# eigenvivek/DiffDRR

Hardware: AMD Instinct MI355X
Metric: DRRs/sec fwd+bwd, 512^3 vol -> 256^2 det, batched poses (higher is better)
Workload: dtype f32; 1 GPU; 512^3 fp32 noise volume -> 256x256 detector, Siddon forward + backward w.r.t. 6-DoF pose (euler ZXY) through NCC, 32 perturbed poses per GPU per step; volume=512x512x512 f32 (512 MiB, replicated per GPU), detector=256x256, batch_per_gpu=32, global_batch=32, parallelism=single GPU, brick_storage_fallbacks=0, bricks=2048, brick_storage=q16p, step=DRR.ncc, fused (at most 32 poses per call): ddrr_pose_ray...

## Files before the change

### diffdrr_amd/_lib.py

```python
from __future__ import annotations

import ctypes
import os
import re
from ctypes import c_char_p, c_double, c_float, c_int, c_long, c_void_p
from typing import NamedTuple

_HERE = os.path.dirname(os.path.abspath(__file__))
_INCLUDE = os.path.join(os.path.dirname(_HERE), "include")
LIB_PATH = os.path.join(_HERE, "csrc", "libdiffdrr_hip.so")
ABI_VERSION = 33
MI_ABI_VERSION = 1
RECON_ABI_VERSION = 1
FBP_ABI_VERSION = 1
LM_ABI_VERSION = 1
WARP_ABI_VERSION = 1
BSPLINE_ABI_VERSION = 1
POLYRIGID_ABI_VERSION = 1
JACOBIAN_ABI_VERSION = 1
PROX_ABI_VERSION = 1

_P, _I, _F, _L, _D = c_void_p, c_int, c_float, c_long, c_double
_ARGTYPES = {"int": c_int, "long": c_long, "float": c_float, "double": c_double}
_RESTYPES_OF = {"int": c_int, "long": c_long, "const char *": c_char_p}
_DECLARATION = re.compile(r"(.*?)\b(ddrr_\w+)\s*\((.*)\)", re.S)
_POINTER = re.compile(r"[\w\s]+\*[\s*]*\w+")
_SCALAR = re.compile(r"(\w+)\s+\w+")


def parse_header(text: str):
    code = re.sub(r"/\*.*?\*/", " ", text, flags=re.S)
    code = re.sub(r"//[^\n]*", "", code)
    defines = {k: int(v) for k, v in re.findall(r"^[ \t]*#[ \t]*define[ \t]+(DDRR_\w+)[ \t]+(\d+)[ \t]*$",
                                                code, re.M)}
    code = re.sub(r"^[ \t]*#[^\n]*", "", code, flags=re.M)
    signatures, restypes = {}, {}
    for stmt in re.split(r"[;{}]", code):
        if not re.search(r"\bddrr_\w+\s*\(", stmt):
            continue
        m = _DECLARATION.fullmatch(" ".join(stmt.split()))
        name = m.group(2) if m else re.search(r"\bddrr_\w+", stmt).group(0)
        ret = re.sub(r"\s*\*\s*", " *", m.group(1)).strip() if m else None
        if ret not in _RESTYPES_OF:
            raise ValueError(f"{name}: cannot bind the declaration {' '.join(stmt.split())!r} "
                             "(return type int, long or const char * expected)")
        params = m.group(3).strip()
        argtypes = []
        for param in ([] if params == "void" else params.split(",")):
            param = param.strip()
            scalar = _SCALAR.fullmatch(param)
            if _POINTER.fullmatch(param):
                argtypes.append(c_void_p)
            elif scalar and scalar.group(1) in _ARGTYPES:
                argtypes.append(_ARGTYPES[scalar.group(1)])
            else:
                raise ValueError(f"{name}: cannot bind the parameter {param!r} (a pointer, int, long, float "
                                 "or double expected)")
        if name in signatures:
            raise ValueError(f"{name}: declared twice")
        signatures[name], restypes[name] = argtypes, _RESTYPES_OF[ret]
    return signatures, restypes, defines


class Header(NamedTuple):
    path: str
    prefix: str
    version: int
    argtypes: dict
    restypes: dict
    defines: dict

    @classmethod
    def read(cls, name: str, prefix: str, version: int) -> "Header":
        path = os.path.join(_INCLUDE, name)
        with open(path) as f:
            argtypes, restypes, defines = parse_header(f.read())
        macro = f"{prefix.upper()}_ABI_VERSION"
        if defines.get(macro) != version:
            raise RuntimeError(f"{path}: {macro} is {defines.get(macro)}, the binding is written against {version}")
        return cls(path, prefix, version, argtypes, restypes, defines)

    def tables(self):
        own = (f"{self.prefix}_abi_version", f"{self.prefix}_last_error")
        signatures = {n: a for n, a in self.argtypes.items() if n not in own}
        return signatures, {n: self.restypes[n] for n in signatures if self.restypes[n] is not c_int}, \
            list(self.argtypes)

    def constants(self, *names):
        return [self.defines[f"{self.prefix.upper()}_{n}"] for n in names]


HEADER = Header.read("diffdrr_hip.h", "ddrr", ABI_VERSION)
_SIGNATURES, _RESTYPES, EXPORTS = HEADER.tables()

REDUCE_SUM, REDUCE_MAX = HEADER.constants("REDUCE_SUM", "REDUCE_MAX")
LOOKUP_STEP, LOOKUP_MID_NEAREST, LOOKUP_MID_TRILINEAR = HEADER.constants(
    "LOOKUP_STEP", "LOOKUP_MID_NEAREST", "LOOKUP_MID_TRILINEAR")
SIDDON_AUX, = HEADER.constants("SIDDON_AUX")
AUX_INTERLEAVED, AUX_BLOCKED, AUX_PACKED = HEADER.constants("AUX_INTERLEAVED", "AUX_BLOCKED", "AUX_PACKED")
REC_BLOCK_RAYS, REC_BLOCK_FLOATS = HEADER.constants("REC_BLOCK_RAYS", "REC_BLOCK_FLOATS")
BRICKS_F32, BRICKS_Q16, BRICKS_Q16_PACKED, BRICKS_CLEARED = HEADER.constants(
    "BRICKS_F32", "BRICKS_Q16", "BRICKS_Q16_PACKED", "BRICKS_CLEARED")
PACKED_AUX_PLANES, TRI_AUX_PLANES = HEADER.constants("PACKED_AUX_PLANES", "TRI_AUX_PLANES")


class DdrrLibrary:

    def __init__(self, path: str, header: Header = HEADER):
        self.path = path
        self.cdll = ctypes.CDLL(path)
        for name in header.argtypes:
            if not hasattr(self.cdll, name):
                raise RuntimeError(f"{path} does not export {name}")
            fn = getattr(self.cdll, name)
            fn.argtypes, fn.restype = header.argtypes[name], header.restypes[name]
        got = getattr(self.cdll, f"{header.prefix}_abi_version")()
        if got != header.version:
            raise RuntimeError(f"{path}: ABI version {got}, expected {header.version}")
        self._last_error = getattr(self.cdll, f"{header.prefix}_last_error")

    def query(self, name: str, *args):
        return getattr(self.cdll, name)(*args)

    def call(self, name: str, *args):
        rc = getattr(self.cdll, name)(*args)
        if rc != 0:
            msg = self._last_error().decode(errors="replace")
            raise RuntimeError(f"{name} failed (code {rc}): {msg}")


_lib: DdrrLibrary | None = None


def get_lib() -> DdrrLibrary:
    global _lib
    if _lib is None:
        import torch

        if not os.path.exists(LIB_PATH):
            raise RuntimeError(
                f"{LIB_PATH} is missing: the MI355X renderers have not been built. Run "
                "`python -c 'import __graft_entry__ as g; g.build()'` (needs hipcc); "
                "diffdrr_amd has no CPU fallback."
            )
        _lib = DdrrLibrary(LIB_PATH)
    return _lib


MI_LIB_PATH = os.path.join(_HERE, "csrc", "libdiffdrr_mi_hip.so")
MI_HEADER = Header.read("diffdrr_mi_hip.h", "ddrr_mi", MI_ABI_VERSION)
_MI_SIGNATURES, _MI_RESTYPES, MI_EXPORTS = MI_HEADER.tables()
MI_MAX_BINS, = MI_HEADER.constants("MAX_BINS")


def mi_library(path: str) -> DdrrLibrary:
    return DdrrLibrary(path, MI_HEADER)


_mi_lib: DdrrLibrary | None = None


def get_mi_lib() -> DdrrLibrary:
    global _mi_lib
    if _mi_lib is None:
        import torch

        if not os.path.exists(MI_LIB_PATH):
            raise RuntimeError(
                f"{MI_LIB_PATH} is missing: the MutualInformation kernels have not been built. Run "
                "`python -c 'import __graft_entry__ as g; g.build()'` (needs hipcc).")
        _mi_lib = mi_library(MI_LIB_PATH)
    return _mi_lib


RECON_LIB_PATH = os.path.join(_HERE, "csrc", "libdiffdrr_recon_hip.so")
RECON_HEADER = Header.read("diffdrr_recon_hip.h", "ddrr_recon", RECON_ABI_VERSION)
_RECON_SIGNATURES, _RECON_RESTYPES, RECON_EXPORTS = RECON_HEADER.tables()
RECON_TV_ISOTROPIC, RECON_TV_ANISOTROPIC, RECON_MAX_DIM = RECON_HEADER.constants(
    "TV_ISOTROPIC", "TV_ANISOTROPIC", "MAX_DIM")


def recon_library(path: str) -> DdrrLibrary:
    return DdrrLibrary(path, RECON_HEADER)


_recon_lib: DdrrLibrary | None = None


def get_recon_lib() -> DdrrLibrary:
    global _recon_lib
    if _recon_lib is None:
        import torch

        if not os.path.exists(RECON_LIB_PATH):
            raise RuntimeError(
                f"{RECON_LIB_PATH} is missing: the reconstruction kernels have not been built. Run "
                "`python -c 'import __graft_entry__ as g; g.build()'` (needs hipcc).")
        _recon_lib = recon_library(RECON_LIB_PATH)
    return _recon_lib


FBP_LIB_PATH = os.path.join(_HERE, "csrc", "libdiffdrr_fbp_hip.so")
FBP_HEADER = Header.read("diffdrr_fbp_hip.h", "ddrr_fbp", FBP_ABI_VERSION)
_FBP_SIGNATURES, _FBP_RESTYPES, FBP_EXPORTS = FBP_HEADER.tables()
FBP_MAX_IMAGE_DIM, FBP_MAX_VIEWS, FBP_MAX_DIM, FBP_VIEW_FLOATS = FBP_HEADER.constants(
    "MAX_IMAGE_DIM", "MAX_VIEWS", "MAX_DIM", "VIEW_FLOATS")


def fbp_library(path: str) -> DdrrLibrary:
    return DdrrLibrary(path, FBP_HEADER)


_fbp_lib: DdrrLibrary | None = None


def get_fbp_lib() -> DdrrLibrary:
    global _fbp_lib
    if _fbp_lib is None:
        import torch

        if not os.path.exists(FBP_LIB_PATH):
            raise RuntimeError(
                f"{FBP_LIB_PATH} is missing: the FDK kernels have not been built. Run "
                "`python -c 'import __graft_entry__ as g; g.build()'` (needs hipcc).")
        _fbp_lib = fbp_library(FBP_LIB_PATH)
    return _fbp_lib


LM_LIB_PATH = os.path.join(_HERE, "csrc", "libdiffdrr_lm_hip.so")
LM_HEADER = Header.read("diffdrr_lm_hip.h", "ddrr_lm", LM_ABI_VERSION)
_LM_SIGNATURES, _LM_RESTYPES, LM_EXPORTS = LM_HEADER.tables()
LM_SUMS, LM_GROUP_RAYS, LM_STATE_DOUBLES, LM_MAX_POSES = LM_HEADER.constants(
    "SUMS", "GROUP_RAYS", "STATE_DOUBLES", "MAX_POSES")


def lm_library(path: str) -> DdrrLibrary:
    return DdrrLibrary(path, LM_HEADER)


_lm_lib: DdrrLibrary | None = None


def get_lm_lib() -> DdrrLibrary:
    global _lm_lib
    if _lm_lib is None:
        import torch

        if not os.path.exists(LM_LIB_PATH):
            raise RuntimeError(
                f"{LM_LIB_PATH} is missing: the Levenberg-Marquardt kernels have not been built. Run "
                "`python -c 'import __graft_entry__ as g; g.build()'` (needs hipcc).")
        _lm_lib = lm_library(LM_LIB_PATH)
    return _lm_lib


# ... 138 lines not shown
```

### diffdrr_amd/csrc/brick_shared.h

```cpp
#pragma once

#include <mutex>

#include "runtime.h"
#include "brick_core.h"
#include "brick_walk.h"
#include "record_layout.h"

namespace ddrr_brick {

using namespace ddrr;

constexpr int kQueueCap = 128;
constexpr int kBuckets = 3;
#if defined(DDRR_EXPERIMENTS) && defined(DDRR_RECORD_GROUP)
constexpr int kRecordGroup = DDRR_RECORD_GROUP;
#else
constexpr int kRecordGroup = 4;
#endif
#if defined(DDRR_EXPERIMENTS) && defined(DDRR_RECORD_ALIGN)
constexpr int kRecordAlign = DDRR_RECORD_ALIGN;
#else
constexpr int kRecordAlign = 4;
#endif
static_assert(kRecordGroup == 8 || kRecordGroup == 4 || kRecordGroup == 2 || kRecordGroup == 1, "DPP maxima");
static_assert(kRecordAlign == 8 || kRecordAlign == 4 || kRecordAlign == 2 || kRecordAlign == 1, "a power of two, at most a run of the record");

struct BrickArgs {
    const float *vol;
    Dims D;
    const float *source;
    const float *target;
    const float *img;
    int B, det_h, det_w;
    float shift, eps;
    BrickLayout lay;
    unsigned aux_plane;
    float rec_q;
    int pix_bits;
    float t1, t2;
    int dbg;
    int *work;
    const float *grad_out;
    float *g_volume;
    int n_points;
    const float *amin, *amax;
    unsigned long long *prof;
    const unsigned char *labels;
    int n_channels;
    const float *ranges;
    const int *fallback;
    int *ws_header;
    int ranges_valid;
    const unsigned char *packed;
    const unsigned *pix_mask;
    const unsigned *fingerprint;
    int vec;
    const int *order;
    int *order_ws;
    int order_cap;
    float *clear;
    long clear_n;
    unsigned *brick_times;
    int split_t, split_s;
};

#if defined(DDRR_BRICK_PROFILE)
struct BrickProf {
    unsigned long long t[16];
    unsigned long long last, born;
    __device__ __forceinline__ void start() {
#pragma unroll
        for (int i = 0; i < 16; ++i) t[i] = 0;
        last = __builtin_amdgcn_s_memtime();
        born = __builtin_amdgcn_s_memrealtime();
    }
    __device__ __forceinline__ void mark(int i) {
        const unsigned long long now = __builtin_amdgcn_s_memtime();
        t[i] += now - last;
        last = now;
    }
    __device__ __forceinline__ void count(int i, unsigned long long n) { t[i] += n; }
};
#if defined(DDRR_TRACE_ONLY)
#define DDRR_PROF(i)
#define DDRR_PROF_COUNT(i, n)
#define DDRR_PROF_WAIT_VMEM()
#else
#define DDRR_PROF(i) prof.mark(i)
#define DDRR_PROF_COUNT(i, n) prof.count(i, n)
#define DDRR_PROF_WAIT_VMEM() asm volatile("s_waitcnt vmcnt(0)" ::: "memory")
#endif
#else
struct BrickProf {};
#define DDRR_PROF(i)
#define DDRR_PROF_COUNT(i, n)
#define DDRR_PROF_WAIT_VMEM()
#endif
enum {
    PROF_STAGE = 0,
    PROF_PULL = 1,
    PROF_PHASE_A = 2,
    PROF_POP = 3,
    PROF_LOADS = 4,
    PROF_SETUP = 5,
    PROF_WALK = 6,
    PROF_DELIVER = 7,
    PROF_BARRIER = 8,
    PROF_N_BATCH = 9, PROF_N_STEPS = 10, PROF_N_UNITS = 11, PROF_N_HITS = 12,
    PROF_CLAIM = 13,
    PROF_ROWS = 14,
    PROF_STORE = 15,
};

constexpr int BRICK_FWD = 0;
constexpr int BRICK_FWD_AUX = 1;
constexpr int BRICK_VOLGRAD = 2;
constexpr int BRICK_TRI_FWD = 3;
constexpr int BRICK_TRI_VOLGRAD = 4;
constexpr int BRICK_TRI_FWD_AUX = 5;
constexpr int BRICK_CHANNELS = 6;
constexpr int BRICK_TRI_CHANNELS = 7;
constexpr int BRICK_CHANNELS_AUX = 8;
constexpr int BRICK_TRI_CHANNELS_AUX = 9;
constexpr int BRICK_CHANNELS_VOLGRAD = 10;
constexpr int BRICK_CHANNELS_WORDS = 12;
constexpr int BRICK_TRI_CHANNELS_VOLGRAD = 11;


#if defined(__HIPCC__)
__device__ __forceinline__ void halfwave_swap(unsigned a, unsigned b, unsigned &x, unsigned &y) {
    const auto s = __builtin_amdgcn_permlane32_swap(a, b, false, false);
    x = s[0];
    y = s[1];
}

__device__ __forceinline__ void deliver_record_blocked(float *__restrict__ aux, bool ok,
                                                       unsigned r, const float v[5]) {
    const unsigned lo = rec_off01(r) | (ok ? 0u : 0x80000000u);
    unsigned xu, yu, x01u, y01u, x23u, y23u;
    halfwave_swap(lo, lo + 8u, xu, yu);
    halfwave_swap(__float_as_uint(v[0]), __float_as_uint(v[1]), x01u, y01u);
    halfwave_swap(__float_as_uint(v[2]), __float_as_uint(v[3]), x23u, y23u);
    const int xo = (int)xu, yo = (int)yu;
    const float x01 = __uint_as_float(x01u), y01 = __uint_as_float(y01u);
    const float x23 = __uint_as_float(x23u), y23 = __uint_as_float(y23u);
    if (xo >= 0) {
        unsafeAtomicAdd(aux + xo, x01);
        unsafeAtomicAdd(aux + xo + 16, x23);
    }
    if (yo >= 0) {
        unsafeAtomicAdd(aux + yo, y01);
        unsafeAtomicAdd(aux + yo + 16, y23);
    }
    if (ok) unsafeAtomicAdd(aux + rec_off4(r), v[4]);
}

typedef unsigned int quad_u32x4 __attribute__((ext_vector_type(4)));
typedef unsigned int quad_u32x4_a4 __attribute__((ext_vector_type(4), aligned(4)));
template <bool LABELS>
__device__ __forceinline__ void quad_load(const float *__restrict__ vol,
                                          const unsigned char *__restrict__ label_map, const Dims &D,
                                          long at, quad_u32x4 &v, unsigned &labels) {
    const long a = quad_clamped_at(D, at);
    v = *reinterpret_cast<const quad_u32x4_a4 *>(vol + a);
    if (LABELS) __builtin_memcpy(&labels, label_map + a, 4);
}
__device__ __forceinline__ void quad_fix(const Dims &D, int x, int y, int z, quad_u32x4 &v,
                                         unsigned &labels) {
    const int shift = quad_shift(D, x, y, z);
    if (shift > 0) {
        if (shift >= 2) v = quad_u32x4{v.z, v.w, 0u, 0u};
        if (shift & 1) v = quad_u32x4{v.y, v.z, v.w, 0u};
        labels = shift < 4 ? labels >> (8 * shift) : 0u;
    }
}

__device__ __forceinline__ int lane_rank(unsigned long long mask) {
    return (int)__builtin_amdgcn_mbcnt_hi((unsigned)(mask >> 32),
                                          __builtin_amdgcn_mbcnt_lo((unsigned)mask, 0u));
}

__device__ __forceinline__ int uni(int v) { return __builtin_amdgcn_readfirstlane(v); }

__device__ __forceinline__ void wave_fence() {
    __builtin_amdgcn_fence(__ATOMIC_SEQ_CST, "wavefront");
    __builtin_amdgcn_wave_barrier();
}

#endif

struct BrickLaunch {
    const float *volume;
    int dx, dy, dz;
    const float *source, *target, *img;
    int B, det_h, det_w;
    float shift, eps;
    hipStream_t st;
    void *launch_ws;
    const char *who;
    const float *grad_out = nullptr;
    float *out = nullptr, *aux = nullptr, *g_volume = nullptr;
    int n_points = 0;
    const float *amin = nullptr, *amax = nullptr;
    float rec_q = 0.f;
    const unsigned char *labels = nullptr;
    int n_channels = 0;
    const unsigned *pix_mask = nullptr;
};

struct FwdStorage {
    int variant, packed;
    float *brick_ranges;
    int ranges_valid;
    float *clear;
    long clear_n;
};

int brick_args(const BrickLaunch &l, BrickArgs &p);

long brick_launch_workspace_bytes(int dx, int dy, int dz);
int brick_launch_resources(const BrickLaunch &l, BrickArgs &p, int &dev, int &n_cu, bool zero_work = true);

constexpr int kMaxDev = 64;
int current_device(int &dev);
struct OncePerDevice {
    std::mutex mu;
    bool done[kMaxDev] = {false};
};
template <class F>
int once_per_device(OncePerDevice &once, int dev, F f) {
    std::lock_guard<std::mutex> lock(once.mu);
    if (once.done[dev]) return 0;
    if (int rc = f()) return rc;
    once.done[dev] = true;
    return 0;
}
template <class K>
int raise_lds_limit(K *kernel, int bytes) {
    const hipError_t e = hipFuncSetAttribute(reinterpret_cast<const void *>(kernel),
                                             hipFuncAttributeMaxDynamicSharedMemorySize, bytes);
    return e == hipSuccess ? 0 : ddrr_rt::fail_hip(e, "hipFuncSetAttribute");
}

bool order_bricks(BrickArgs &q, int BX, int BY, int BZ, int nby, int nbz, int n_bricks, int slots,
                  hipStream_t st, bool zero_counter = false, int min_poses = 8);
int launch_bricks(int mode, const BrickLaunch &l);

long brick_workspace_bytes(int dx, int dy, int dz, int brick_storage);
int launch_fwd_bricks(const BrickLaunch &l, const FwdStorage &s);

#if defined(DDRR_EXPERIMENTS) || defined(DDRR_BRICK_PROFILE)
extern float g_brick_t1, g_brick_t2;
extern int g_brick_dbg;
extern int g_brick_variant;
extern const int *g_brick_order;
extern unsigned *g_brick_times;
extern int g_brick_split_t, g_brick_split_s;
#else
constexpr float g_brick_t1 = 18.f, g_brick_t2 = 40.f;
constexpr int g_brick_dbg = 0;
#endif
#if defined(DDRR_BRICK_PROFILE)
extern unsigned long long *g_brick_prof;
#endif

}
```

### diffdrr_amd/csrc/bricks.hip

```cpp
#include "runtime.h"

#include "siddon_core.h"
#include "brick_core.h"
#include "brick_walk.h"
#include "brick_step.h"
#include "record_pack.h"
#include "record_layout.h"
#include "tri_brick.h"
#include "brick_shared.h"
#include "trilinear_core.h"

using namespace ddrr;
using namespace ddrr_rt;
using namespace ddrr_brick;

namespace {


constexpr int kBrickThreads = 1024;
constexpr int kBrickWaves = kBrickThreads / 64;
constexpr int kPoseChunk = 32;

inline size_t brick_lds_bytes(const BrickLayout &lay) {
    return (size_t)brick_floats(lay) * 4 + (size_t)kBrickWaves * kBuckets * kQueueCap * 4 +
// ... 964 lines not shown
    p.prof = g_brick_prof;
#endif
    return 0;
}

namespace {

struct BrickMode {
    int mode;
    void (*kernel)(BrickArgs, float *, float *);
    bool marcher;
    bool tri_grid;
    int prepare;
    int order_min_poses;
};
template <int MODE>
constexpr BrickMode brick_mode(bool marcher, bool tri_grid, int prepare, int order_min_poses) {
    return {MODE, &siddon_brick_kernel<MODE>, marcher, tri_grid, prepare, order_min_poses};
}
constexpr BrickMode kBrickModes[] = {
    brick_mode<BRICK_CHANNELS_WORDS>(false, false, 0, 8),
    brick_mode<BRICK_TRI_CHANNELS_VOLGRAD>(true, false, 2, 0),
    brick_mode<BRICK_CHANNELS_VOLGRAD>(false, false, 2, 8),
    brick_mode<BRICK_TRI_CHANNELS_AUX>(true, true, 0, 0),
    brick_mode<BRICK_CHANNELS_AUX>(false, false, 0, 8),
    brick_mode<BRICK_TRI_CHANNELS>(true, true, 0, 0),
    brick_mode<BRICK_CHANNELS>(false, false, 0, 8),
    brick_mode<BRICK_TRI_FWD_AUX>(true, true, 0, 0),
    brick_mode<BRICK_FWD>(false, false, 0, 8),
    brick_mode<BRICK_FWD_AUX>(false, false, 0, 8),
    brick_mode<BRICK_VOLGRAD>(false, false, 1, 8),
    brick_mode<BRICK_TRI_FWD>(true, true, 0, 0),
    brick_mode<BRICK_TRI_VOLGRAD>(true, false, 1, 1),
};

}

int launch_bricks(int mode, const BrickLaunch &l) {
    const BrickMode *m = nullptr;
    for (const BrickMode &row : kBrickModes)
        if (row.mode == mode) m = &row;
    if (!m) return fail(-1, "unknown brick mode");
    BrickArgs p;
    if (int rc = brick_args(l, p)) return rc;
    p.lay = g_brick_layout;
    if (m->marcher) {
        p.t1 = g_tri_t1;
        p.t2 = g_tri_t2;
    }
    const size_t lds = brick_lds_bytes(p.lay);
    int dev = 0, n_cu = 0;
    if (int rc = brick_launch_resources(l, p, dev, n_cu)) return rc;
    static OncePerDevice lds_limit;
    if (int rc = once_per_device(lds_limit, dev, [] {
            for (const BrickMode &row : kBrickModes)
                if (int r = raise_lds_limit(row.kernel, 160 * 1024)) return r;
            return 0;
        }))
        return rc;
    if (m->prepare) {
        const int N = l.det_h * l.det_w;
        int bx = (N + kBlock - 1) / kBlock;
        bx = bx > 64 ? 64 : bx;
        hipLaunchKernelGGL(volgrad_prepare_kernel, dim3(bx, l.B), dim3(kBlock), 0, l.st, (int)m->marcher,
                           l.source, l.target, l.img, l.grad_out, N, l.det_w, p.D, l.shift, l.eps,
                           l.n_points, l.amin, l.amax, p.work, m->prepare == 2 ? l.n_channels : 0);
    }
    const BrickGrid bg = m->tri_grid ? tri_brick_grid(p.D) : brick_grid(p.D);
    const int n_bricks = bg.nx * bg.ny * bg.nz;
    if (m->order_min_poses)
        order_bricks(p, BRICK, BRICK, BRICK, bg.ny, bg.nz, n_bricks, n_cu, l.st, false, m->order_min_poses);
    const dim3 grid(n_bricks < n_cu ? n_bricks : n_cu), block(kBrickThreads);
    hipLaunchKernelGGL(m->kernel, grid, block, lds, l.st, p, l.out, l.aux);
    return finish(l.who);
}

}

extern "C" {

#if defined(DDRR_EXPERIMENTS) || defined(DDRR_BRICK_PROFILE)
int ddrr_set_brick_layout(int sy, int sx) {
    if (sy < BRICK || sx < BRICK * sy) return -1;
    BrickLayout lay = {sy, sx};
    if (brick_lds_bytes(lay) > 160 * 1024) return -1;
    g_brick_layout = lay;
    return 0;
}
int ddrr_set_brick_debug(int flags) {
    g_brick_dbg = flags;
    return 0;
}
int ddrr_set_brick_classes(float t1, float t2) {
    g_brick_t1 = t1;
    g_brick_t2 = t2;
    return 0;
}
#endif
#if defined(DDRR_BRICK_PROFILE)
int ddrr_brick_profile_reset() {
    if (!g_brick_prof && hipMalloc(reinterpret_cast<void **>(&g_brick_prof), 20 * 8) != hipSuccess)
        return -1;
    return hipMemset(g_brick_prof, 0, 20 * 8) == hipSuccess ? 0 : -1;
}
int ddrr_brick_profile_read20(unsigned long long *host20) {
    if (!g_brick_prof) return -1;
    return hipMemcpy(host20, g_brick_prof, 20 * 8, hipMemcpyDeviceToHost) == hipSuccess ? 0 : -1;
}
int ddrr_brick_profile_read(unsigned long long *host16) {
    if (!g_brick_prof) return -1;
    return hipMemcpy(host16, g_brick_prof, 16 * 8, hipMemcpyDeviceToHost) == hipSuccess ? 0 : -1;
}
#endif

static int check_detector(int det_h, int det_w) {
    if (det_h < 2 || det_w < 2) return fail(-1, "the brick path needs a detector of at least 2x2");
    return 0;
}
static int check_channel_cap(int B, int C, int N, const char *per_ray_entry) {
    if ((long)B * C * N < (1L << 30) && N < (1 << 22)) return 0;
    char msg[256];
    snprintf(msg, sizeof(msg), "B * C * N must stay below 2^30 (and N below 2^22) for one channel launch "
                               "on the bricks: split the pose batch or use %s", per_ray_entry);
    return fail(-1, msg);
}
static int check_n_points(int n_points) {
    if (n_points < 2) return fail(-1, "n_points must be >= 2");
    return 0;
}
static int check_alpha_range(const float *alphamin, const float *alphamax) {
    if (!alphamin || !alphamax) return fail(-1, "null alphamin / alphamax");
    return 0;
}
static int zero_floats(float *buf, size_t n, hipStream_t st) {
    const hipError_t e = hipMemsetAsync(buf, 0, sizeof(float) * n, st);
    return e == hipSuccess ? 0 : fail_hip(e, "hipMemsetAsync");
}
static int zero_volume_gradient(float *g_volume, int dx, int dy, int dz, hipStream_t st) {
    return zero_floats(g_volume, (size_t)dx * dy * dz, st);
}

static int siddon_forward_bricks_impl(const float *volume, int dx, int dy, int dz, const float *source,
                                      const float *target, const float *img, int B, int det_h,
                                      int det_w, float voxel_shift, float eps, float *out, float *aux,
                                      float record_vmax, int brick_storage, float *brick_ranges,
                                      int ranges_valid, void *launch_ws, const unsigned *pixel_mask,
                                      void *stream) {
    const int N = det_h * det_w;
    if (int rc = check_common(volume, dx, dy, dz, source, 1, target, B, N, nullptr)) return rc;
    if (!out && !aux) return fail(-1, "null out pointer");
    if (int rc = check_detector(det_h, det_w)) return rc;
    if (!(record_vmax >= 0.f)) return fail(-1, "record_vmax must be >= 0");
    if (brick_storage != DDRR_BRICKS_F32 && brick_storage != DDRR_BRICKS_Q16 &&
        brick_storage != DDRR_BRICKS_Q16_PACKED)
        return fail(-1, "brick_storage must be DDRR_BRICKS_F32, DDRR_BRICKS_Q16 or DDRR_BRICKS_Q16_PACKED");
    if (brick_storage != DDRR_BRICKS_F32 && !brick_ranges)
        return fail(-1, "DDRR_BRICKS_Q16 needs the brick_ranges workspace");
    if (B == 0) return 0;
    hipStream_t st = (hipStream_t)stream;
    const long R = (long)B * N;
    const bool cleared = (ranges_valid & DDRR_BRICKS_CLEARED) != 0;
    const bool packed = aux && record_vmax > 0.f;
    const size_t fill = !aux ? (size_t)R : (packed ? (size_t)R * 5 : (size_t)rec_blocked_floats(R));
    BrickLaunch l{volume, dx, dy, dz, source, target, img, B, det_h, det_w, voxel_shift, eps, st, launch_ws,
                  "ddrr_siddon_forward_bricks"};
    l.out = out;
    l.aux = aux;
    l.pix_mask = pixel_mask;
    if (packed) {
        if (!cleared)
            if (int rc = zero_floats(aux, fill, st)) return rc;
        l.rec_q = record_scale(record_vmax, Dims{dx, dy, dz});
        hipLaunchKernelGGL(record_prepare_kernel, dim3((unsigned)((R + kBlock - 1) / kBlock)),
                           dim3(kBlock), 0, st, source, target, R, N, Dims{dx, dy, dz}, voxel_shift,
                           eps, l.rec_q, aux);
    }
    FwdStorage fs;
    fs.packed = brick_storage == DDRR_BRICKS_Q16_PACKED;
    fs.variant = fs.packed ? DDRR_BRICKS_Q16 : brick_storage;
    fs.brick_ranges = brick_ranges;
    fs.ranges_valid = ranges_valid & 1;
    fs.clear = packed || cleared ? nullptr : (aux ? aux : out);
    fs.clear_n = cleared ? -1 : (packed ? 0 : (long)fill);
    if (int rc = launch_fwd_bricks(l, fs)) return rc;
    if (!aux) return 0;
    if (out)
        hipLaunchKernelGGL(siddon_out_from_record_kernel, dim3((unsigned)((R + kBlock - 1) / kBlock)),
                           dim3(kBlock), 0, st, aux + (packed ? 4 * R : 0), packed ? 0 : 1, img, R, out);
    return finish("ddrr_siddon_forward_bricks");
}

int ddrr_siddon_forward_bricks(const float *volume, int dx, int dy, int dz, const float *source,
                               const float *target, const float *img, int B, int det_h,
                               int det_w, float voxel_shift, float eps, float *out, float *aux,
                               float record_vmax, int brick_storage, float *brick_ranges,
                               int ranges_valid, void *launch_ws, void *stream) {
    return siddon_forward_bricks_impl(volume, dx, dy, dz, source, target, img, B, det_h, det_w, voxel_shift,
                                      eps, out, aux, record_vmax, brick_storage, brick_ranges, ranges_valid,
                                      launch_ws, nullptr, stream);
}

int ddrr_siddon_forward_bricks_masked(const float *volume, int dx, int dy, int dz, const float *source,
                                      const float *target, const float *img, int B, int det_h,
                                      int det_w, float voxel_shift, float eps, float *out, float *aux,
                                      float record_vmax, int brick_storage, float *brick_ranges,
                                      int ranges_valid, void *launch_ws, const unsigned *pixel_mask,
                                      void *stream) {
    if (pixel_mask && (reinterpret_cast<uintptr_t>(pixel_mask) & 3) != 0)
        return fail(-1, "pixel_mask must be 4-byte aligned");
    return siddon_forward_bricks_impl(volume, dx, dy, dz, source, target, img, B, det_h, det_w, voxel_shift,
                                      eps, out, aux, record_vmax, brick_storage, brick_ranges, ranges_valid,
                                      launch_ws, pixel_mask, stream);
}

long ddrr_brick_workspace_bytes(int dx, int dy, int dz, int brick_storage) {
    if (dx < 1 || dy < 1 || dz < 1) return 0;
    return brick_workspace_bytes(dx, dy, dz, brick_storage);
}

long ddrr_brick_launch_workspace_bytes(int dx, int dy, int dz) {
    if (dx < 1 || dy < 1 || dz < 1) return 0;
    return brick_launch_workspace_bytes(dx, dy, dz);
}

int ddrr_siddon_forward_channels_bricks(const float *volume, const unsigned char *labels, int dx,
                                        int dy, int dz, const float *source, const float *target,
                                        const float *img, int B, int det_h, int det_w, int C,
                                        float voxel_shift, float eps, float *out, void *launch_ws,
                                        void *stream) {
    const int N = det_h * det_w;
    if (int rc = check_common(volume, dx, dy, dz, source, 1, target, B, N,
                              "ddrr_siddon_forward_channels_bricks (mask_to_channels)"))
        return rc;
    if (!labels || !out || C < 1) return fail(-1, "null labels/out or C < 1");
    if (int rc = check_detector(det_h, det_w)) return rc;
    if (int rc = check_channel_cap(B, C, N, "ddrr_siddon_forward_channels")) return rc;
    if (B == 0) return 0;
    hipStream_t st = (hipStream_t)stream;
    if (int rc = zero_floats(out, (size_t)B * C * N, st)) return rc;
    BrickLaunch l{volume, dx, dy, dz, source, target, img, B, det_h, det_w, voxel_shift, eps, st, launch_ws,
                  "ddrr_siddon_forward_channels_bricks"};
    l.out = out;
    l.labels = labels;
    l.n_channels = C;
    return launch_bricks(BRICK_CHANNELS, l);
}

constexpr int kChannelWordsStateWords = 2 + 2 * kFingerprintWords;

__global__ __launch_bounds__(1024) void channel_words_check_kernel(const float *__restrict__ vol,
                                                                   const unsigned char *__restrict__ labels,
                                                                   long n, int *__restrict__ state, int force) {
    unsigned *fp = reinterpret_cast<unsigned *>(state + 2);
    int bad = force;
    unsigned v = 0u, l = 0u;
    if (threadIdx.x < kFingerprintWords) {
        const long at = fingerprint_index(threadIdx.x, n);
        v = __float_as_uint(vol[at]);
        l = (unsigned)labels[at];
        bad |= (v != fp[threadIdx.x]) | (l != fp[kFingerprintWords + threadIdx.x]);
    }
    const bool stale = __syncthreads_or(bad) != 0;
    if (stale && threadIdx.x < kFingerprintWords) {
        fp[threadIdx.x] = v;
        fp[kFingerprintWords + threadIdx.x] = l;
    }
    if (threadIdx.x == 0) {
        state[0] = stale ? 1 : 0;
        if (stale) state[1] += 1;
    }
}

__global__ __launch_bounds__(1024) void channel_words_kernel(const float *__restrict__ vol,
                                                             const unsigned char *__restrict__ labels, long n,
                                                             unsigned n_channels, float *__restrict__ words,
                                                             const int *__restrict__ state) {
    if (state[0] == 0) return;
    const long stride = (long)gridDim.x * 1024;
    for (long i = (long)blockIdx.x * 1024 + threadIdx.x; i < n; i += stride)
        words[i] = pack_voxel_label_below(vol[i], labels[i], n_channels);
}

long ddrr_channel_words_state_bytes(void) { return (long)kChannelWordsStateWords * 4; }

int ddrr_channel_words(const float *volume, const unsigned char *labels, long n_voxels, int C, float *words,
                       void *state, int force, void *stream) {
    if (!volume || !labels || !words || !state || C < 1 || n_voxels < 0)
        return fail(-1, "null pointer or C < 1");
    if (n_voxels == 0) return 0;
    static_assert(kFingerprintWords <= 1024, "one sample per thread of the check");
    const long blocks = (n_voxels + 4095) / 4096;
    hipLaunchKernelGGL(channel_words_check_kernel, dim3(1), dim3(1024), 0, (hipStream_t)stream, volume, labels,
                       n_voxels, reinterpret_cast<int *>(state), force ? 1 : 0);
    hipLaunchKernelGGL(channel_words_kernel, dim3((unsigned)(blocks > 512 ? 512 : blocks)), dim3(1024), 0,
                       (hipStream_t)stream, volume, labels, n_voxels, (unsigned)C, words,
                       reinterpret_cast<const int *>(state));
    return finish("ddrr_channel_words");
}

int ddrr_siddon_forward_channels_bricks_words(const float *words, int dx, int dy, int dz, const float *source,
                                              const float *target, const float *img, int B, int det_h,
                                              int det_w, int C, float voxel_shift, float eps, float *out,
                                              void *launch_ws, void *stream) {
    const int N = det_h * det_w;
    if (int rc = check_common(words, dx, dy, dz, source, 1, target, B, N,
                              "ddrr_siddon_forward_channels_bricks_words (mask_to_channels)"))
        return rc;
    if (!out || C < 1) return fail(-1, "null out or C < 1");
    if (int rc = check_detector(det_h, det_w)) return rc;
    if (int rc = check_channel_cap(B, C, N, "ddrr_siddon_forward_channels")) return rc;
    if (B == 0) return 0;
    hipStream_t st = (hipStream_t)stream;
    if (int rc = zero_floats(out, (size_t)B * C * N, st)) return rc;
    BrickLaunch l{words, dx, dy, dz, source, target, img, B, det_h, det_w, voxel_shift, eps, st, launch_ws,
                  "ddrr_siddon_forward_channels_bricks_words"};
    l.out = out;
    l.n_channels = C;
    return launch_bricks(BRICK_CHANNELS_WORDS, l);
}

int ddrr_siddon_backward_channels_bricks(const float *volume, const unsigned char *labels, int dx,
                                         int dy, int dz, const float *source, const float *target,
                                         const float *grad_out, int B, int det_h, int det_w, int C,
                                         float voxel_shift, float eps, float *aux, void *launch_ws,
                                         void *stream) {
    const int N = det_h * det_w;
    if (int rc = check_common(volume, dx, dy, dz, source, 1, target, B, N,
                              "ddrr_siddon_backward_channels_bricks (mask_to_channels)"))
        return rc;
    if (!labels || !grad_out || !aux || C < 1) return fail(-1, "null labels/grad_out/aux or C < 1");
    if (int rc = check_detector(det_h, det_w)) return rc;
    if (int rc = check_channel_cap(B, C, N, "ddrr_siddon_backward_channels")) return rc;
// ... 217 lines not shown
```

### diffdrr_amd/csrc/bricks_fwd.hip

```cpp
#include "runtime.h"

#include "siddon_core.h"
#include "brick_core.h"
#include "brick_walk.h"
#include "brick_step.h"
#include "record_pack.h"
#include "record_layout.h"
#include "brick_shared.h"

using namespace ddrr;
using namespace ddrr_rt;
using namespace ddrr_brick;

namespace {

template <int BX_, int BY_, int BZ_, int THREADS_, bool Q16_, int ROWPAD_ = -1>
struct FwdCfg {
    static constexpr int BX = BX_, BY = BY_, BZ = BZ_, THREADS = THREADS_, WAVES = THREADS_ / 64;
    static constexpr bool Q16 = Q16_;
    static constexpr int ES = Q16 ? 2 : 4;
    static constexpr int ROWPAD = ROWPAD_ < 0 ? ES : ROWPAD_;
    static constexpr int SY = BZ * ES + ROWPAD;
    static constexpr int SX = BY * SY + ES;
    static constexpr int BRICK_BYTES = (BX * SX + 15) / 16 * 16;
    static constexpr int WGS_PER_CU = 1024 / THREADS;
    static constexpr int LDS_BUDGET = 160 * 1024 / WGS_PER_CU;
    static constexpr int QUEUE_BYTES = WAVES * kBuckets * kQueueCap * 4;
    static constexpr int HZ = BZ / 2;
    static constexpr int FSY = HZ * 4 + 4, FSX = BY * FSY + 4;
    static constexpr int FALLBACK_BYTES = (BX * FSX + 15) / 16 * 16;
    static constexpr bool MIXED =
        Q16 && HZ % 4 == 0 && (BX * BY * (HZ / 4)) % THREADS == 0 &&
        FALLBACK_BYTES + QUEUE_BYTES + 16 + 8 * 20 * 4 <= LDS_BUDGET;
    using Half = FwdCfg<BX_, BY_, BZ_ / 2, THREADS_, false>;
    static constexpr int LDS_BRICK = MIXED && FALLBACK_BYTES > BRICK_BYTES ? FALLBACK_BYTES : BRICK_BYTES;
    static constexpr int ROW_ROOM = (LDS_BUDGET - LDS_BRICK - QUEUE_BYTES - 48) / (20 * 4);
    static constexpr int CHUNK = ROW_ROOM >= 32 ? 32 : ROW_ROOM;
    static constexpr int LDS_MIN = LDS_BRICK + QUEUE_BYTES + CHUNK * 20 * 4 + 16 + 32;
    static constexpr int POOL_BYTES = WAVES * kBuckets * 4;
    static constexpr bool POOL = LDS_MIN + POOL_BYTES <= LDS_BUDGET && WAVES * kBuckets <= 64;
    static constexpr int LDS = LDS_MIN + (POOL ? POOL_BYTES : 0);
    static constexpr int MAXSTEPS = BX + BY + BZ + 4;
    static_assert(CHUNK >= 8, "no room for the row table");
    static_assert(BZ % 4 == 0 && (BX * BY * (BZ / 4)) % THREADS == 0, "staging");
};

struct FwdRow {
    float D0[3], ei[3], ej[3], P0[3], P1[3];
    float inv_w;
    int i0, j0, w, count;
};
static_assert(sizeof(FwdRow) == 80, "FwdRow");

__device__ __forceinline__ FwdRow fwd_row(const BrickRow &r) {
    FwdRow f;
#pragma unroll
    for (int a = 0; a < 3; ++a) {
        f.D0[a] = r.D0[a];
        f.ei[a] = r.ei[a];
        f.ej[a] = r.ej[a];
        f.P0[a] = r.P0[a];
        f.P1[a] = r.P1[a];
    }
    f.inv_w = r.inv_w;
    f.i0 = r.i0;
    f.j0 = r.j0;
    f.w = r.w;
    f.count = r.count;
    return f;
}

__device__ __forceinline__ BrickRow brick_row_of(const FwdRow &f) {
    BrickRow r;
#pragma unroll
    for (int a = 0; a < 3; ++a) {
        r.D0[a] = f.D0[a];
        r.ei[a] = f.ei[a];
        r.ej[a] = f.ej[a];
        r.P0[a] = f.P0[a];
        r.P1[a] = f.P1[a];
    }
    r.inv_w = f.inv_w;
    r.nscale = 0.f;
    r.i0 = f.i0;
    r.j0 = f.j0;
    r.w = f.w;
    r.count = f.count;
    r.perm_k = 1;
    return r;
}

struct LdsAbsFetch16 {
    __device__ __forceinline__ float operator()(unsigned addr) const {
#if defined(__HIP_DEVICE_COMPILE__)
        const unsigned q =
            *(const __attribute__((address_space(3))) unsigned short *)(unsigned long long)addr;
        return __uint_as_float(q);
#else
        (void)addr;
        return 0.f;
#endif
    }
};

template <class C>
__device__ __forceinline__ Box cfg_brick_box(const Dims D, int nby, int nbz, int id) {
    const int bz = id % nbz, by = (id / nbz) % nby, bx = id / (nbz * nby);
    Box b;
    b.lo[0] = bx * C::BX;
    b.lo[1] = by * C::BY;
    b.lo[2] = bz * C::BZ;
    b.hi[0] = b.lo[0] + C::BX < D.x ? b.lo[0] + C::BX : D.x;
    b.hi[1] = b.lo[1] + C::BY < D.y ? b.lo[1] + C::BY : D.y;
    b.hi[2] = b.lo[2] + C::BZ < D.z ? b.lo[2] + C::BZ : D.z;
    return b;
}

template <bool AUX, class C>
__device__ __forceinline__ void fwd_item(const BrickArgs &p, unsigned lds_base,
                                         const StepGeom &SG, const Q16Range &range, bool active,
                                         unsigned b, unsigned pix, float *__restrict__ out,
                                         float *__restrict__ aux, BrickProf &prof,
                                         const FwdRow *rows = nullptr, int b0 = 0,
                                         bool f32_brick = !C::Q16) {
    const bool q16 = C::Q16 && !f32_brick;
    const unsigned r = b * (unsigned)(p.det_h * p.det_w) + pix;
    float v[5] = {0.f, 0.f, 0.f, 0.f, 0.f};
    bool ok = false;
    if (active) {
        const float *sp = p.source + b * 3u, *tp = p.target + r * 3u;
        float s[3], t[3], L = 1.f;
#if defined(DDRR_EXPERIMENTS) || defined(DDRR_BRICK_PROFILE)
        if ((p.dbg & 256) && rows) {
            const FwdRow &w = rows[b - b0];
            const float fi = floorf(((float)pix + 0.5f) / (float)p.det_w);
            const float fj = (float)pix - fi * (float)p.det_w;
#pragma unroll
            for (int a = 0; a < 3; ++a) {
                s[a] = (float)(a == 0 ? SG.lof[0] : (a == 1 ? SG.lof[1] : SG.lof[2])) - 0.01f - p.shift -
                       w.P0[a];
                t[a] = s[a] + (fmaf(fj, w.ej[a], fmaf(fi, w.ei[a], w.D0[a])) - p.eps);
            }
            L = sqrtf((t[0] - s[0]) * (t[0] - s[0]) + (t[1] - s[1]) * (t[1] - s[1]) +
                      (t[2] - s[2]) * (t[2] - s[2]));
        } else
#endif
        {
#pragma unroll
            for (int a = 0; a < 3; ++a) {
                s[a] = sp[a];
                t[a] = tp[a];
            }
            L = (!AUX && p.img) ? p.img[r] : 1.f;
        }
        DDRR_PROF_WAIT_VMEM();
        DDRR_PROF(PROF_LOADS);
        StepEntry E = step_enter(SG, s, t, p.shift, p.eps, lds_base);
        if (q16) q16_scale_entry(E);
        DDRR_PROF(PROF_SETUP);
        int steps = 0;
        float ex[2] = {0.f, 0.f};
        if (E.hit) {
            if (!AUX) {
                float a_end;
                if (q16) {
                    steps = step_walk_fwd<C::MAXSTEPS>(LdsAbsFetch16{}, SG, E, v[0], a_end);
                    v[0] = q16_finish_fwd(range, E, v[0], a_end);
                } else {
                    steps = step_walk_fwd<C::MAXSTEPS>(LdsAbsFetch{}, SG, E, v[0], a_end);
                }
            } else if (q16) {
                steps = step_walk<AUX, C::MAXSTEPS>(LdsAbsFetch16{}, SG, E, v[0], v + 1, ex);
                q16_finish<AUX>(range, E, ex, v[0], v + 1);
            } else {
                steps = step_walk<AUX, C::MAXSTEPS>(LdsAbsFetch{}, SG, E, v[0], v + 1);
            }
        }
        DDRR_PROF(PROF_WALK);
        DDRR_PROF_COUNT(PROF_N_STEPS, (unsigned long long)__builtin_amdgcn_readfirstlane(steps));
        (void)steps;
        ok = E.hit;
        if (!AUX && ok) unsafeAtomicAdd(out + r, L * v[0]);
    }
    if (AUX) {
        if (p.rec_q > 0.f) {
            if (ok) {
                const float qa = p.rec_q / aux[5u * p.aux_plane + r];
// ... 179 lines not shown
        store1<3>(v3, dst, tid), store1<4>(v4, dst, tid), store1<5>(v5, dst, tid);
        store1<6>(v6, dst, tid), store1<7>(v7, dst, tid), store1<8>(v8, dst, tid);
    }
};

template <class C>
__global__ __launch_bounds__(C::THREADS) void brick_pack_kernel(BrickArgs p, int nby, int nbz,
                                                                unsigned char *__restrict__ packed) {
    extern __shared__ __align__(16) unsigned char smem_raw[];
    __shared__ int counter[4];
    const int tid = threadIdx.x, brick_id = blockIdx.x;
    if (p.fallback && p.fallback[brick_id]) return;
    constexpr int NV = C::BRICK_BYTES / 16;
    uint4 *lds = reinterpret_cast<uint4 *>(smem_raw);
    for (int k = tid; k < NV; k += C::THREADS) lds[k] = make_uint4(0u, 0u, 0u, 0u);
    __syncthreads();
    const Box box = cfg_brick_box<C>(p.D, nby, nbz, brick_id);
    Q16Range range = {0.f, 0.f, 0.f};
    bool empty = false;
    fwd_stage_brick<C>(p, smem_raw, box, brick_id, tid, range, empty, counter);
    __syncthreads();
    uint4 *dst = reinterpret_cast<uint4 *>(packed + (size_t)brick_id * C::BRICK_BYTES);
    for (int k = tid; k < NV; k += C::THREADS) dst[k] = lds[k];
}

#if defined(DDRR_BRICK_PROFILE)
#define DDRR_TRACE(k, how)                                                                      \
    if (p.brick_times && lane == 0) {                                                           \
        const unsigned dt_ = (unsigned)__builtin_amdgcn_s_memrealtime() - (unsigned)ahead[6];   \
        unsigned *slot_ = p.brick_times + n_bricks + 16 * brick_id + (k);                        \
        if (how) atomicMax(slot_, dt_);                                                         \
        else if (wave == 0) *slot_ = dt_;                                                       \
    }
#else
#define DDRR_TRACE(k, how) {}
#endif

template <bool AUX, class C, bool PRE = false, bool SUB = false>
__global__ __launch_bounds__(C::THREADS) __attribute__((amdgpu_waves_per_eu(4, 4))) void
siddon_fwd_brick_kernel(BrickArgs p, float *__restrict__ out, float *__restrict__ aux) {
    extern __shared__ __align__(16) unsigned char smem_raw[];
    unsigned char *brick = smem_raw;
    unsigned *queue = reinterpret_cast<unsigned *>(smem_raw + C::LDS_BRICK);
    FwdRow *rows = reinterpret_cast<FwdRow *>(queue + C::WAVES * kBuckets * kQueueCap);
    int *counter = reinterpret_cast<int *>(rows + C::CHUNK);
    volatile int *ahead = counter + 4;
    int *pool = counter + 12;

    const int tid = threadIdx.x, wave = tid >> 6, lane = tid & 63;
    const int nbx = (p.D.x + C::BX - 1) / C::BX, nby = (p.D.y + C::BY - 1) / C::BY;
    const int nbz = (p.D.z + C::BZ - 1) / C::BZ;
    const int n_bricks = nbx * nby * nbz;
    const int N = p.det_h * p.det_w;
    unsigned *myq = queue + wave * kBuckets * kQueueCap;
    const unsigned pix_mask = (1u << p.pix_bits) - 1u;
    const unsigned lds_base = LdsAbsFetch::base_of(reinterpret_cast<const float *>(brick));
    const bool GROUPED = AUX && p.rec_q == 0.f && !(p.dbg & 8);
    const bool POOLED = C::POOL && !(p.dbg & 2048);

    BrickProf prof;
#if defined(DDRR_BRICK_PROFILE)
    prof.start();
#endif
    int brick_id = 0, sub = 0, n_sub = 1, pose_lo = 0, pose_hi = p.B;
    bool f32_brick = !C::Q16;
    constexpr int kLookRounds = 3;
    constexpr int kLaStage = 1 << 30;
    const bool LOOK = C::Q16 && PackedPrefetch<C>::FITS && p.packed != nullptr && p.B <= C::CHUNK && !(p.dbg & 4096)
#if defined(DDRR_EXPERIMENTS) || defined(DDRR_BRICK_PROFILE)
                      && p.split_t == 0
#endif
        ;
    const int n_wg = (int)gridDim.x;
    PackedPrefetch<C> pf;
    pf.clear();
    int la_item = -1, la_brick = 0, la_after = -1;
    float la_lo = 0.f, la_hi = 0.f;
    bool la_f32 = false;
    bool stale = false;
    if constexpr (C::MIXED) {
        if (p.fingerprint != nullptr && p.ranges_valid) {
            static_assert(kFingerprintWords <= C::THREADS, "one sample per thread");
            int bad = 0;
            if (tid < kFingerprintWords)
                bad = __float_as_uint(p.vol[fingerprint_index(tid, (long)p.D.x * p.D.y * p.D.z)]) != p.fingerprint[tid];
            if constexpr (PRE) {
                if (tid == 0) {
                    const int it = atomicAdd(p.work, 1);
                    int b = 0, fb = 0;
                    float lo = 0.f, hi = 0.f;
                    if (it < n_bricks) {
                        b = p.order ? p.order[it] : it;
                        fb = p.fallback ? p.fallback[b] : 0;
                        lo = p.ranges[2 * b];
                        hi = p.ranges[2 * b + 1];
                    }
                    ahead[0] = it;
                    ahead[1] = b | (fb ? kLaStage : 0);
                    ahead[2] = __float_as_int(lo);
                    ahead[3] = __float_as_int(hi);
                }
            }
            stale = __syncthreads_or(bad) != 0;
            if constexpr (PRE) {
                la_item = uni(ahead[0]);
                const int b = uni(ahead[1]);
                la_brick = b & ~kLaStage;
                la_f32 = stale || (b & kLaStage) != 0;
                la_lo = __int_as_float(uni(ahead[2]));
                la_hi = __int_as_float(uni(ahead[3]));
            }
            if (stale && blockIdx.x == 0 && tid == 0) atomicAdd(p.ws_header + 2, 1);
        }
    }
    int pf_kind = 0;
    int item = 0;
    for (;;) {
        __syncthreads();
        DDRR_PROF(PROF_BARRIER);
        const bool next_half = sub + 1 < n_sub;
        const bool known = !next_half && la_item >= 0;
        const bool loaded = pf_kind != 0;
        if (tid == 0) {
            if (!next_half && !known) counter[1] = atomicAdd(p.work, 1);
            counter[2] = 0;
            counter[3] = 0;
        }
        if (!loaded) __syncthreads();
        float cur_lo = 0.f, cur_hi = 0.f;
        if (next_half) {
            ++sub;
        } else {
            item = known ? la_item : counter[1];
#if defined(DDRR_EXPERIMENTS) || defined(DDRR_BRICK_PROFILE)
            const int n_full = n_bricks - p.split_t;
            if (item >= n_full + p.split_t * p.split_s) break;
            const int kth = item < n_full ? item : n_full + (item - n_full) / p.split_s;
            const int part = item < n_full ? 0 : (item - n_full) % p.split_s;
            const int parts = item < n_full ? 1 : p.split_s;
            pose_lo = (int)((long)p.B * part / parts);
            pose_hi = (int)((long)p.B * (part + 1) / parts);
#else
            if (item >= n_bricks) break;
            const int kth = item;
#endif
            brick_id = known ? la_brick : (p.order ? p.order[kth] : kth);
            cur_lo = la_lo;
            cur_hi = la_hi;
            la_item = -1;
            sub = 0;
            n_sub = 1;
            if (C::MIXED) {
                f32_brick = stale || (known ? la_f32 : (p.fallback && p.fallback[brick_id] != 0));
                const int z0 = (brick_id % nbz) * C::BZ;
                n_sub = f32_brick && p.D.z - z0 > C::HZ ? 2 : 1;
            }
        }
        const bool last_part = sub + 1 >= n_sub;
        const bool look = LOOK && last_part;
#if defined(DDRR_EXPERIMENTS) || defined(DDRR_BRICK_PROFILE)
        const int look_rounds = (p.dbg >> 13) & 3 ? 1 + ((p.dbg >> 13) & 3) : kLookRounds;
#else
        constexpr int look_rounds = kLookRounds;
#endif
        const bool claim = look && item + look_rounds * n_wg < n_bricks;
        int nx_item = la_after;
        int req_item = -1, req_brick = 0, req_fb = 0;
        float req_lo = 0.f, req_hi = 0.f;
        if (tid == 64 && look) {
            if (nx_item < 0 && claim) nx_item = atomicAdd(p.work, 1);
            if (claim) req_item = atomicAdd(p.work, 1);
            if (nx_item >= 0 && nx_item < n_bricks) {
                req_brick = p.order ? p.order[nx_item] : nx_item;
                req_fb = stale ? 1 : (C::MIXED && p.fallback ? p.fallback[req_brick] : 0);
                req_lo = p.ranges[2 * req_brick];
                req_hi = p.ranges[2 * req_brick + 1];
            }
        }
#if defined(DDRR_BRICK_PROFILE)
        const unsigned long long brick_t0 = __builtin_amdgcn_s_memrealtime();
        if (tid == 0) ahead[6] = (int)(unsigned)brick_t0;
#endif
        const int n_chunks = (pose_hi - pose_lo + C::CHUNK - 1) / C::CHUNK;
        const int chunk = n_chunks ? (pose_hi - pose_lo + n_chunks - 1) / n_chunks : 0;
        DDRR_PROF(PROF_CLAIM);
        Box box = cfg_brick_box<C>(p.D, nby, nbz, brick_id);
        if (C::MIXED && f32_brick) {
            box.lo[2] += sub * C::HZ;
            box.hi[2] = box.lo[2] + C::HZ < box.hi[2] ? box.lo[2] + C::HZ : box.hi[2];
        }
        const BoxF cells = boxf(box);
        StepGeom SG;
#pragma unroll
        for (int a = 0; a < 3; ++a) {
            SG.lof[a] = (float)box.lo[a];
            SG.hif[a] = (float)box.hi[a];
        }
        const bool half = C::MIXED && f32_brick;
        SG.strideb[0] = bits_as_float((unsigned)(half ? C::FSX : C::SX));
        SG.strideb[1] = bits_as_float((unsigned)(half ? C::FSY : C::SY));
        SG.strideb[2] = bits_as_float((unsigned)(half ? 4 : C::ES));
        int qn0 = 0, qn1 = 0, qn2 = 0;
        bool brick_empty = false, pool_open = false;
        Q16Range range = {0.f, 0.f, 0.f};
        int tid_pf = tid;
        asm volatile("" : "+v"(tid_pf));
        if (pf_kind == 1) {
            range = q16_range(cur_lo, cur_hi);
            brick_empty = cur_lo == 0.f && cur_hi == 0.f;
            if (!brick_empty) pf.store(brick, tid_pf);
        }
        if constexpr (C::MIXED) {
            if (pf_kind == 2) pf.template half<typename C::Half>(p, brick, box, tid_pf, false);
        }
        DDRR_TRACE(8, 0)
        DDRR_TRACE(10, 1)

        for (int ch = 0; ch < n_chunks; ++ch) {
            const int b0 = pose_lo + ch * chunk;
            const int nb = pose_hi - b0 < chunk ? pose_hi - b0 : chunk;
            const bool last_chunk = ch == n_chunks - 1;
            if (ch > 0) __syncthreads();
            int det_h = p.det_h, det_w = p.det_w, tid_here = tid;
            asm volatile("" : "+s"(det_h), "+s"(det_w), "+v"(tid_here));
            if (tid < nb) {
                const PoseGrid pg = pose_grid(p.source + (long)(b0 + tid) * 3,
                                              p.target + (long)(b0 + tid) * N * 3, det_h, det_w);
                PixBox pb = project_brick_grid(pg, det_h, det_w, cells, p.shift);
                if (GROUPED && kRecordAlign > 1 && !(p.dbg & 1024)) pb = align_pixbox_rows(pb, det_w, kRecordAlign);
                rows[tid] = fwd_row(brick_row(pg, pb, cells, p.shift, p.eps, 0.f));
            }
            if (tid == 0) counter[0] = 0;
            DDRR_PROF(PROF_ROWS);
            if (ch == 0) DDRR_TRACE(9, 0)
            if (ch == 0 && !loaded) {
                if constexpr (C::MIXED) {
                    if (f32_brick)
                        fwd_stage_brick<typename C::Half>(p, brick, box, brick_id, tid_here, range,
                                                          brick_empty, counter);
                    else if (p.packed)
                        fwd_stage_packed<C>(p, brick, brick_id, tid_here, range, brick_empty);
                    else
                        fwd_stage_brick<C>(p, brick, box, brick_id, tid_here, range, brick_empty, counter);
                } else if (C::Q16 && p.packed) {
                    fwd_stage_packed<C>(p, brick, brick_id, tid_here, range, brick_empty);
                } else {
                    fwd_stage_brick<C>(p, brick, box, brick_id, tid_here, range, brick_empty, counter);
                }
            }
            if (ch == 0 && look && tid == 64) {
                ahead[0] = nx_item;
                ahead[1] = req_brick | (req_fb ? kLaStage : 0);
                ahead[2] = __float_as_int(req_lo);
                ahead[3] = __float_as_int(req_hi);
                ahead[4] = req_item;
            }
            DDRR_PROF(PROF_STORE);
            if (ch == 0) DDRR_TRACE(4, 0)
            if (ch == 0) DDRR_TRACE(7, 1)
            __syncthreads();
            if (ch == 0) DDRR_TRACE(0, 0)
            if ((!C::Q16 || f32_brick) && ch == 0 && !loaded) brick_empty = counter[2] == 0;
            int incl = lane < nb ? (rows[lane].count + 63) >> 6 : 0;
#pragma unroll
            for (int o = 1; o < 32; o <<= 1) {
                const int up = __shfl_up(incl, o, 64);
                incl += lane >= o ? up : 0;
            }
            const int units = brick_empty ? 0 : __builtin_amdgcn_readlane(incl, 31);
            int cur = 0, cur_lo = 0, cur_hi = __builtin_amdgcn_readlane(incl, 0);
            DDRR_PROF(PROF_STAGE);
            for (;;) {
                int u = 0;
                if (lane == 0) u = atomicAdd(&counter[0], 1);
                u = uni(u);
                const bool drain = u >= units;
                if (drain && !last_chunk) break;
                if (!drain) {
                    while (u >= cur_hi) {
                        ++cur;
                        cur_lo = cur_hi;
                        cur_hi = __builtin_amdgcn_readlane(incl, uni(cur));
                    }
                    const BrickRow r = brick_row_of(rows[cur]);
                    DDRR_PROF(PROF_PULL);
                    DDRR_PROF_COUNT(PROF_N_UNITS, 1);
                    const int local = (u - cur_lo) * 64 + lane;
                    const bool valid = local < uni(r.count);
                    int pix = 0;
                    float n_est = 0.f;
                    bool hit = valid && brick_candidate(r, local, p.det_w, pix, n_est);
                    if constexpr (SUB) hit = hit && ((p.pix_mask[pix >> 5] >> (pix & 31)) & 1u) != 0u;
                    float n_grp = hit ? n_est : 0.f;
                    if (GROUPED) {
                        if constexpr (kRecordGroup >= 2)
                            n_grp = fmaxf(n_grp, __builtin_bit_cast(float, __builtin_amdgcn_update_dpp(
                                0, __builtin_bit_cast(int, n_grp), 0xB1, 0xf, 0xf, true)));
                        if constexpr (kRecordGroup >= 4)
                            n_grp = fmaxf(n_grp, __builtin_bit_cast(float, __builtin_amdgcn_update_dpp(
                                0, __builtin_bit_cast(int, n_grp), 0x4E, 0xf, 0xf, true)));
                        if constexpr (kRecordGroup >= 8)
                            n_grp = fmaxf(n_grp, __builtin_bit_cast(float, __builtin_amdgcn_update_dpp(
                                0, __builtin_bit_cast(int, n_grp), 0x141, 0xf, 0xf, true)));
                    }
                    const bool c0 = n_grp < p.t1, c1 = !c0 && n_grp < p.t2;
                    const unsigned long long m0 = __ballot(hit && c0);
                    const unsigned long long m1 = __ballot(hit && c1);
                    const unsigned long long m2 = __ballot(hit && !c0 && !c1);
                    if (hit) {
                        const int r0 = lane_rank(m0), r1 = lane_rank(m1), r2 = lane_rank(m2);
                        const int slot = c0 ? qn0 + r0 : (c1 ? kQueueCap + qn1 + r1
                                                             : 2 * kQueueCap + qn2 + r2);
                        myq[slot] = ((unsigned)(b0 + cur) << p.pix_bits) | (unsigned)pix;
                    }
                    qn0 = uni(qn0 + (int)__popcll(m0));
                    qn1 = uni(qn1 + (int)__popcll(m1));
                    qn2 = uni(qn2 + (int)__popcll(m2));
                    wave_fence();
                    DDRR_PROF_COUNT(PROF_N_HITS, __popcll(m0) + __popcll(m1) + __popcll(m2));
                    DDRR_PROF(PROF_PHASE_A);
                }
                for (;;) {
                    int n = 0;
                    unsigned e = 0;
                    if (!pool_open) {
                        int k = -1;
                        if (qn0 >= 64) k = 0;
                        else if (qn1 >= 64) k = 1;
                        else if (qn2 >= 64) k = 2;
                        if (k >= 0) {
                            const int base = (k == 0 ? qn0 : (k == 1 ? qn1 : qn2)) - 64;
                            qn0 -= k == 0 ? 64 : 0;
                            qn1 -= k == 1 ? 64 : 0;
                            qn2 -= k == 2 ? 64 : 0;
                            e = myq[k * kQueueCap + base + lane];
                            n = 64;
                        } else if (drain && POOLED) {
                            if (lane < kBuckets)
                                pool[wave * kBuckets + lane] = lane == 0 ? qn0 : (lane == 1 ? qn1 : qn2);
                            DDRR_TRACE(1, 0)
                            __syncthreads();
                            DDRR_TRACE(2, 0)
                            DDRR_PROF(PROF_BARRIER);
                            pool_open = true;
                            continue;
                        } else if (drain && qn0 + qn1 + qn2 > 0) {
                            const int tot = qn0 + qn1 + qn2;
                            n = tot < 64 ? tot : 64;
                            const int i2 = lane, i1 = lane - qn2, i0 = lane - qn2 - qn1;
                            if (lane < n)
                                e = i2 < qn2 ? myq[2 * kQueueCap + qn2 - 1 - i2]
                                             : (i1 < qn1 ? myq[kQueueCap + qn1 - 1 - i1]
                                                         : myq[qn0 - 1 - i0]);
                            const int t2 = qn2 < n ? qn2 : n;
                            const int t1 = qn1 < n - t2 ? qn1 : n - t2;
                            qn2 -= t2;
                            qn1 -= t1;
                            qn0 -= n - t2 - t1;
                        } else {
                            break;
                        }
                    } else {
                        constexpr int NSEG = C::WAVES * kBuckets;
                        int j = 0;
                        if (lane == 0) j = atomicAdd(&counter[3], 1);
                        j = uni(j) * 64;
                        int end = lane < NSEG ? pool[(lane % C::WAVES) * kBuckets + kBuckets - 1 - lane / C::WAVES] : 0;
#pragma unroll
                        for (int o = 1; o < 64; o <<= 1) {
                            const int up = __shfl_up(end, o, 64);
                            end += lane >= o ? up : 0;
                        }
                        const int total = __builtin_amdgcn_readlane(end, 63);
                        if (j >= total) break;
                        const int kf = (int)__popcll(__ballot(lane < NSEG && end <= j));
                        const int kl = (int)__popcll(__ballot(lane < NSEG && end <= j + 63));
                        const int g = j + lane;
                        int seg = kf, base = kf ? __builtin_amdgcn_readlane(end, uni(kf - 1)) : 0;
                        for (int k = kf; k < kl; ++k) {
                            const int ek = __builtin_amdgcn_readlane(end, uni(k));
                            if (ek <= g) seg = k + 1, base = ek;
                        }
                        n = total - j < 64 ? total - j : 64;
                        if (lane < n)
                            e = queue[((seg % C::WAVES) * kBuckets + kBuckets - 1 - seg / C::WAVES) * kQueueCap + (g - base)];
                    }
                    DDRR_PROF(PROF_POP);
                    DDRR_PROF_COUNT(PROF_N_BATCH, 1);
                    fwd_item<AUX, C>(p, lds_base, SG, range, lane < n, e >> p.pix_bits,
                                     e & pix_mask, out, aux, prof, rows, b0, f32_brick);
                    wave_fence();
                }
                if (drain) break;
            }
        }
        DDRR_TRACE(3, 0)
        DDRR_TRACE(6, 1)
        pf_kind = 0;
        int half_of = -1, half_sub = 0;
        if (C::MIXED && LOOK && !last_part) {
            half_of = brick_id;
            half_sub = sub + 1;
        } else if (look) {
            la_item = uni(ahead[0]);
            la_after = uni(ahead[4]);
            const int b = uni(ahead[1]);
            la_brick = b & ~kLaStage;
            la_lo = __int_as_float(uni(ahead[2]));
            la_hi = __int_as_float(uni(ahead[3]));
            la_f32 = (b & kLaStage) != 0;
            if (la_item >= 0 && la_item < n_bricks) {
                if (la_f32) half_of = la_brick;
                else pf_kind = 1;
            }
        }
        int tid_ld = tid;
        asm volatile("" : "+v"(tid_ld));
        if (pf_kind == 1 && !(la_lo == 0.f && la_hi == 0.f)) {
            pf.load(p, la_brick, tid_ld);
        } else if (C::MIXED && half_of >= 0) {
            if constexpr (C::MIXED) {
                Box nbox = cfg_brick_box<C>(p.D, nby, nbz, half_of);
                nbox.lo[2] += half_sub * C::HZ;
                nbox.hi[2] = nbox.lo[2] + C::HZ < nbox.hi[2] ? nbox.lo[2] + C::HZ : nbox.hi[2];
                pf.clear();
                pf.template half<typename C::Half>(p, brick, nbox, tid_ld, true);
                pf_kind = 2;
            }
        } else {
            pf.clear();
        }
        DDRR_TRACE(5, 1)
#if defined(DDRR_BRICK_PROFILE)
        __syncthreads();
        if (tid == 0 && p.brick_times)
            p.brick_times[brick_id] = (unsigned)(__builtin_amdgcn_s_memrealtime() - brick_t0);
#endif
    }
#if defined(DDRR_BRICK_PROFILE)
    DDRR_PROF(PROF_BARRIER);
    if (lane == 0 && p.prof) {
        for (int i = 0; i < 16; ++i) atomicAdd(p.prof + i, prof.t[i]);
        const unsigned long long died = __builtin_amdgcn_s_memrealtime();
        atomicAdd(p.prof + 16, prof.born);
        atomicAdd(p.prof + 17, died);
        atomicMax(p.prof + 18, ~prof.born);
        atomicMax(p.prof + 19, died);
    }
#endif
}

constexpr int kSubBlocks = 1024;
__global__ __launch_bounds__(256) void brick_range_kernel(const float *__restrict__ vol, Dims D,
                                                          int BX, int BY, int BZ, int nby, int nbz,
                                                          float *__restrict__ ranges,
                                                          int *__restrict__ fallback, int vec) {
    __shared__ float red[3][4];
    __shared__ float sub_sum[kSubBlocks];
    __shared__ int sub_nnz[kSubBlocks];
    const int id = blockIdx.x;
    const int bz = id % nbz, by = (id / nbz) % nby, bx = id / (nbz * nby);
    const int x0 = bx * BX, y0 = by * BY, z0 = bz * BZ;
    const int nx = min(BX, D.x - x0), ny = min(BY, D.y - y0), nz = min(BZ, D.z - z0);
    const int QZ = BZ / 4, quads = nx * ny * QZ;
    const int SBY = (BY + 3) / 4, n_sub = ((BX + 3) / 4) * SBY * QZ;
    for (int k = threadIdx.x; k < kSubBlocks; k += 256) {
        sub_sum[k] = 0.f;
        sub_nnz[k] = 0;
    }
    __syncthreads();
    float tmin = INFINITY, tmax = -INFINITY;
    bool bad = false;
    for (int k = threadIdx.x; k < quads; k += 256) {
        const int qz = k % QZ, row = k / QZ, ly = row % ny, lx = row / ny;
        if (qz * 4 >= nz) continue;
        const float *g = vol + ((long)(x0 + lx) * D.y + (y0 + ly)) * D.z + z0 + qz * 4;
        const int nv = nz - qz * 4;
        float4 v;
        if (vec) {
            v = *reinterpret_cast<const float4 *>(g);
        } else {
            v.x = g[0];
            v.y = nv > 1 ? g[1] : v.x;
            v.z = nv > 2 ? g[2] : v.x;
            v.w = nv > 3 ? g[3] : v.x;
        }
        tmin = fminf(fminf(fminf(tmin, v.x), fminf(v.y, v.z)), v.w);
        tmax = fmaxf(fmaxf(fmaxf(tmax, v.x), fmaxf(v.y, v.z)), v.w);
        const float sum = (fabsf(v.x) + (nv > 1 ? fabsf(v.y) : 0.f)) +
                          ((nv > 2 ? fabsf(v.z) : 0.f) + (nv > 3 ? fabsf(v.w) : 0.f));
        bad = bad || !(sum < INFINITY);
        const int sb = ((lx >> 2) * SBY + (ly >> 2)) * QZ + qz;
        if (n_sub <= kSubBlocks) {
            atomicAdd(&sub_sum[sb], sum);
            atomicAdd(&sub_nnz[sb], (v.x != 0.f) + (nv > 1 && v.y != 0.f) + (nv > 2 && v.z != 0.f) +
                                        (nv > 3 && v.w != 0.f));
        }
    }
#pragma unroll
    for (int o = 32; o > 0; o >>= 1) {
        tmin = fminf(tmin, __shfl_xor(tmin, o, 64));
        tmax = fmaxf(tmax, __shfl_xor(tmax, o, 64));
    }
    bad = __ballot(bad) != 0ull;
    const int wave = threadIdx.x >> 6;
    if ((threadIdx.x & 63) == 0) {
        red[0][wave] = tmin;
        red[1][wave] = bad ? NAN : tmax;
    }
    __syncthreads();
    float lo = INFINITY, hi = -INFINITY;
    bool nan = false;
    for (int w = 0; w < 4; ++w) {
        lo = fminf(lo, red[0][w]);
        hi = fmaxf(hi, red[1][w]);
        nan = nan || red[1][w] != red[1][w];
    }
    if (!(lo <= hi)) lo = hi = 0.f;
    float level = INFINITY;
    for (int k = threadIdx.x; k < n_sub && n_sub <= kSubBlocks; k += 256) {
        const int qz = k % QZ, sy = (k / QZ) % SBY, sx = k / (QZ * SBY);
        const int cx = min(4, nx - 4 * sx), cy = min(4, ny - 4 * sy), cz = min(4, nz - 4 * qz);
        if (cx <= 0 || cy <= 0 || cz <= 0) continue;
        const int n_eff = lo == 0.f ? sub_nnz[k] : cx * cy * cz;
        if (n_eff > 0) level = fminf(level, sub_sum[k] / (float)n_eff);
    }
#pragma unroll
    for (int o = 32; o > 0; o >>= 1) level = fminf(level, __shfl_xor(level, o, 64));
    if ((threadIdx.x & 63) == 0) red[2][wave] = level;
    __syncthreads();
    if (threadIdx.x == 0) {
        level = fminf(fminf(red[2][0], red[2][1]), fminf(red[2][2], red[2][3]));
        if (n_sub > kSubBlocks) level = 0.f;
        const float vmax = nan ? NAN : hi;
        ranges[2 * id] = lo;
        ranges[2 * id + 1] = vmax;
        fallback[id] = q16_usable(lo, vmax, level) ? 0 : 1;
    }
}

__global__ __launch_bounds__(256) void brick_fallback_count_kernel(const int *__restrict__ fallback,
                                                                   int n_bricks, int *__restrict__ header) {
    __shared__ int total;
    if (threadIdx.x == 0) total = 0;
    __syncthreads();
    int n = 0;
    for (int k = threadIdx.x; k < n_bricks; k += 256) n += fallback[k] != 0;
    atomicAdd(&total, n);
    __syncthreads();
    if (threadIdx.x == 0) {
        header[0] = total;
        header[1] = n_bricks;
        header[2] = 0;
    }
}

__global__ __launch_bounds__(1024) void brick_fingerprint_kernel(const float *__restrict__ vol, long n_vox,
                                                                 unsigned *__restrict__ fp) {
    const int i = blockIdx.x * 1024 + threadIdx.x;
    if (i < kFingerprintWords) fp[i] = __float_as_uint(vol[fingerprint_index(i, n_vox)]);
}

__global__ __launch_bounds__(256) void brick_weight_kernel(BrickArgs p, int BX, int BY, int BZ,
                                                           int nby, int nbz, int n_bricks,
                                                           float *__restrict__ weight) {
    const int brick = blockIdx.x * 4 + (threadIdx.x >> 6), lane = threadIdx.x & 63;
    if (brick >= n_bricks) return;
    const int bz = brick % nbz, by = (brick / nbz) % nby, bx = brick / (nbz * nby);
    BoxF cells;
    cells.lo[0] = (float)(bx * BX), cells.lo[1] = (float)(by * BY), cells.lo[2] = (float)(bz * BZ);
    cells.hi[0] = (float)min(bx * BX + BX, p.D.x), cells.hi[1] = (float)min(by * BY + BY, p.D.y);
    cells.hi[2] = (float)min(bz * BZ + BZ, p.D.z);
    const int N = p.det_h * p.det_w;
    float w = 0.f;
    for (int b = lane; b < p.B; b += 64) {
        const PoseGrid pg = pose_grid(p.source + (long)b * 3, p.target + (long)b * N * 3, p.det_h, p.det_w);
        w += (float)pixbox_count(project_brick_grid(pg, p.det_h, p.det_w, cells, p.shift));
    }
#pragma unroll
    for (int o = 32; o > 0; o >>= 1) w += __shfl_xor(w, o, 64);
    if (lane == 0) weight[brick] = p.fallback && p.fallback[brick] ? 2.f * w : w;
}

constexpr int kOrderClasses = 1024;
__global__ __launch_bounds__(1024) void brick_order_kernel(const float *__restrict__ weight,
                                                           int n_bricks, int *__restrict__ order,
                                                           int *__restrict__ zero4) {
    if (zero4 && threadIdx.x < 4) zero4[threadIdx.x] = 0;
    __shared__ int hist[kOrderClasses];
    __shared__ float wmax_s[16];
    const int tid = threadIdx.x;
    float wmax = 0.f;
    for (int i = tid; i < n_bricks; i += 1024) wmax = fmaxf(wmax, weight[i]);
#pragma unroll
    for (int o = 32; o > 0; o >>= 1) wmax = fmaxf(wmax, __shfl_xor(wmax, o, 64));
    if ((tid & 63) == 0) wmax_s[tid >> 6] = wmax;
    hist[tid] = 0;
    __syncthreads();
    wmax = 0.f;
    for (int k = 0; k < 16; ++k) wmax = fmaxf(wmax, wmax_s[k]);
    const float scale = wmax > 0.f ? (float)(kOrderClasses - 1) / wmax : 0.f;
    for (int i = tid; i < n_bricks; i += 1024)
        atomicAdd(&hist[kOrderClasses - 1 - (int)(weight[i] * scale)], 1);
    __syncthreads();
    int v = hist[tid];
    for (int o = 1; o < kOrderClasses; o <<= 1) {
        __syncthreads();
        const int add = tid >= o ? hist[tid - o] : 0;
        __syncthreads();
        hist[tid] += add;
    }
    __syncthreads();
    const int excl = hist[tid] - v;
    __syncthreads();
    hist[tid] = excl;
    __syncthreads();
    for (int i = tid; i < n_bricks; i += 1024)
        order[atomicAdd(&hist[kOrderClasses - 1 - (int)(weight[i] * scale)], 1)] = i;
}

__global__ __launch_bounds__(256) void brick_clear_kernel(float *__restrict__ buf, long n, int *__restrict__ work) {
    if (work && blockIdx.x == 0 && threadIdx.x < 4) work[threadIdx.x] = 0;
    const long stride = (long)gridDim.x * 256, n4 = n >> 2;
    float4 *b4 = reinterpret_cast<float4 *>(buf);
    for (long i = (long)blockIdx.x * 256 + threadIdx.x; i < n4; i += stride) b4[i] = make_float4(0.f, 0.f, 0.f, 0.f);
    if (blockIdx.x == 0 && threadIdx.x < (n & 3)) buf[(n4 << 2) + threadIdx.x] = 0.f;
}

template <bool AUX, class C, bool PRE = false, bool SUB = false>
int launch_cfg(const BrickArgs &p, int dev, int n_cu, float *out, float *aux, hipStream_t st) {
    static_assert(C::LDS <= C::LDS_BUDGET, "LDS budget");
    static OncePerDevice lds_limit;
    if (int rc = once_per_device(lds_limit, dev, [] {
            return raise_lds_limit(&siddon_fwd_brick_kernel<AUX, C, PRE, SUB>, C::LDS);
        }))
        return rc;
    hipError_t e;
    const int nbx = (p.D.x + C::BX - 1) / C::BX, nby = (p.D.y + C::BY - 1) / C::BY;
    const int nbz = (p.D.z + C::BZ - 1) / C::BZ;
    const int n_bricks = nbx * nby * nbz, slots = n_cu * C::WGS_PER_CU;
    if constexpr (C::Q16) {
        if (!p.ranges) return fail(-1, "DDRR_BRICKS_Q16 needs the brick_ranges workspace");
        if (!p.ranges_valid) {
            hipLaunchKernelGGL(brick_range_kernel, dim3(n_bricks), dim3(256), 0, st, p.vol, p.D, C::BX,
                               C::BY, C::BZ, nby, nbz, const_cast<float *>(p.ranges),
                               const_cast<int *>(p.fallback), p.vec);
            hipLaunchKernelGGL(brick_fallback_count_kernel, dim3(1), dim3(256), 0, st, p.fallback,
                               n_bricks, p.ws_header);
            hipLaunchKernelGGL(brick_fingerprint_kernel, dim3((kFingerprintWords + 1023) / 1024), dim3(1024), 0, st,
                               p.vol, (long)p.D.x * p.D.y * p.D.z, const_cast<unsigned *>(p.fingerprint));
            if (p.packed) {
                static OncePerDevice pack_lds_limit;
                if (int rc = once_per_device(pack_lds_limit, dev, [] {
                        return raise_lds_limit(&brick_pack_kernel<C>, C::BRICK_BYTES);
                    }))
                    return rc;
                hipLaunchKernelGGL(brick_pack_kernel<C>, dim3(n_bricks), dim3(C::THREADS),
                                   C::BRICK_BYTES, st, p, nby, nbz,
                                   const_cast<unsigned char *>(p.packed));
            }
        }
    } else if (p.packed) {
        return fail(-1, "packed bricks are 16-bit bricks");
    }
    BrickArgs q = p;
    const bool ordered = order_bricks(q, C::BX, C::BY, C::BZ, nby, nbz, n_bricks, slots, st, true);
    const bool clear_here = p.clear && p.clear_n > 0;
    if (p.clear_n < 0) {
    } else if (clear_here && (reinterpret_cast<uintptr_t>(p.clear) & 15) == 0) {
        const long blocks = (p.clear_n / 4 + 255) / 256;
        hipLaunchKernelGGL(brick_clear_kernel, dim3((unsigned)(blocks < 1 ? 1 : (blocks > 4096 ? 4096 : blocks))),
                           dim3(256), 0, st, p.clear, p.clear_n, ordered ? nullptr : q.work);
    } else {
        if (clear_here && (e = hipMemsetAsync(p.clear, 0, sizeof(float) * (size_t)p.clear_n, st)) != hipSuccess)
            return fail_hip(e, "hipMemsetAsync");
        if (!ordered && (e = hipMemsetAsync(q.work, 0, 4 * sizeof(int), st)) != hipSuccess)
            return fail_hip(e, "hipMemsetAsync");
    }
    const dim3 grid(n_bricks < slots ? n_bricks : slots), block(C::THREADS);
    hipLaunchKernelGGL((siddon_fwd_brick_kernel<AUX, C, PRE, SUB>), grid, block, C::LDS, st, q, out, aux);
    return 0;
}

using CfgF32 = FwdCfg<32, 32, 32, 1024, false>;
using CfgQ16Z64 = FwdCfg<32, 32, 64, 1024, true>;
#if defined(DDRR_EXPERIMENTS) || defined(DDRR_BRICK_PROFILE)
using CfgQ16x2 = FwdCfg<32, 32, 32, 512, true>;
using CfgQ16x1 = FwdCfg<32, 32, 32, 1024, true>;
using CfgF32Half = FwdCfg<32, 32, 16, 512, false, 0>;
using CfgQ16X64 = FwdCfg<64, 32, 32, 1024, true>;
using CfgQ16Y64 = FwdCfg<32, 64, 32, 1024, true>;
using CfgF32Y64 = FwdCfg<16, 64, 32, 1024, false>;
using CfgF32X64 = FwdCfg<64, 16, 32, 1024, false>;
using CfgF32Z64 = FwdCfg<16, 32, 64, 1024, false>;
#endif

}

namespace ddrr_brick {

bool order_bricks(BrickArgs &q, int BX, int BY, int BZ, int nby, int nbz, int n_bricks, int slots,
                  hipStream_t st, bool zero_counter, int min_poses) {
    if (!(q.order_ws && n_bricks <= q.order_cap && n_bricks > slots && !q.order && q.B >= min_poses)) return false;
    float *weight = reinterpret_cast<float *>(q.order_ws);
    int *order = q.order_ws + q.order_cap;
    hipLaunchKernelGGL(brick_weight_kernel, dim3((n_bricks + 3) / 4), dim3(256), 0, st, q, BX, BY,
                       BZ, nby, nbz, n_bricks, weight);
    hipLaunchKernelGGL(brick_order_kernel, dim3(1), dim3(1024), 0, st, weight, n_bricks, order,
                       zero_counter ? q.work : nullptr);
    q.order = order;
    return true;
}

constexpr long kWsHeaderBytes = 256;
static long n32_bricks(int dx, int dy, int dz) {
    return (long)((dx + 31) / 32) * ((dy + 31) / 32) * ((dz + 31) / 32);
}
constexpr long kFingerprintBytes = kFingerprintWords * (long)sizeof(unsigned);
static long ranges_bytes(int dx, int dy, int dz) {
    return kWsHeaderBytes + (n32_bricks(dx, dy, dz) * 3 * (long)sizeof(float) + 255) / 256 * 256 + kFingerprintBytes;
}

long brick_workspace_bytes(int dx, int dy, int dz, int brick_storage) {
    if (brick_storage == DDRR_BRICKS_F32) return 0;
    long n = ranges_bytes(dx, dy, dz);
    if (brick_storage == DDRR_BRICKS_Q16_PACKED)
        n += (long)((dx + CfgQ16Z64::BX - 1) / CfgQ16Z64::BX) * ((dy + CfgQ16Z64::BY - 1) / CfgQ16Z64::BY) *
             ((dz + CfgQ16Z64::BZ - 1) / CfgQ16Z64::BZ) * CfgQ16Z64::BRICK_BYTES;
    return n;
}

template <class C, bool PRE = false>
static int launch_variant(const BrickLaunch &l, const BrickArgs &p, int dev, int n_cu) {
    if (p.pix_mask)
        return l.aux ? launch_cfg<true, C, PRE, true>(p, dev, n_cu, l.out, l.aux, l.st)
                     : launch_cfg<false, C, PRE, true>(p, dev, n_cu, l.out, l.aux, l.st);
    return l.aux ? launch_cfg<true, C, PRE, false>(p, dev, n_cu, l.out, l.aux, l.st)
                 : launch_cfg<false, C, PRE, false>(p, dev, n_cu, l.out, l.aux, l.st);
}

int launch_fwd_bricks(const BrickLaunch &l, const FwdStorage &s) {
    int variant = s.variant, ranges_valid = s.ranges_valid;
    const bool vec_ok = (l.dz & 3) == 0 && (reinterpret_cast<uintptr_t>(l.volume) & 15) == 0;
    const bool quads_ok = l.dz >= 4 && (long)l.dx * l.dy * l.dz >= 4 && (reinterpret_cast<uintptr_t>(l.volume) & 3) == 0;
    bool few_f32 = variant == DDRR_BRICKS_F32 && l.B < 8;
#if defined(DDRR_EXPERIMENTS) || defined(DDRR_BRICK_PROFILE)
    if (g_brick_variant != -2) {
        static int last_variant = -100;
        variant = g_brick_variant;
        if (variant != last_variant) ranges_valid = 0;
        last_variant = variant;
        few_f32 = false;
    }
#endif
    if (!quads_ok || variant < 0 || few_f32) {
        if (s.clear && s.clear_n > 0 &&
            hipMemsetAsync(s.clear, 0, sizeof(float) * (size_t)s.clear_n, l.st) != hipSuccess)
            return fail(-1, "hipMemsetAsync");
        return launch_bricks(l.aux ? BRICK_FWD_AUX : BRICK_FWD, l);
    }
    BrickArgs p;
    if (int rc = brick_args(l, p)) return rc;
    p.vec = vec_ok ? 1 : 0;
    float *const ws = s.brick_ranges;
    p.ws_header = reinterpret_cast<int *>(ws);
    p.ranges = ws ? ws + kWsHeaderBytes / sizeof(float) : nullptr;
    p.fallback = ws ? reinterpret_cast<const int *>(p.ranges + 2 * n32_bricks(l.dx, l.dy, l.dz)) : nullptr;
    p.ranges_valid = ranges_valid;
    p.packed = s.packed && ws ? reinterpret_cast<const unsigned char *>(ws) + ranges_bytes(l.dx, l.dy, l.dz)
                              : nullptr;
    p.fingerprint = ws ? reinterpret_cast<const unsigned *>(reinterpret_cast<const unsigned char *>(ws) +
                                                            ranges_bytes(l.dx, l.dy, l.dz) - kFingerprintBytes)
                       : nullptr;
    p.clear = s.clear;
    p.clear_n = s.clear_n;
#if defined(DDRR_EXPERIMENTS) || defined(DDRR_BRICK_PROFILE)
    p.order = g_brick_order;
    p.split_t = g_brick_split_t;
    p.split_s = g_brick_split_s;
#endif
    if (variant == DDRR_BRICKS_Q16 || variant == 5) {
        p.t1 = g_brick_t1 * (22.f / 18.f);
        p.t2 = g_brick_t2 * (48.f / 40.f);
    }
    int dev = 0, n_cu = 0;
    if (int rc = brick_launch_resources(l, p, dev, n_cu, false)) return rc;
    int rc = 0;
    switch (variant) {
        case DDRR_BRICKS_F32: rc = launch_variant<CfgF32>(l, p, dev, n_cu); break;
        case DDRR_BRICKS_Q16:
            rc = l.B <= 8 ? launch_variant<CfgQ16Z64, true>(l, p, dev, n_cu)
                          : launch_variant<CfgQ16Z64>(l, p, dev, n_cu);
            break;
#if defined(DDRR_EXPERIMENTS) || defined(DDRR_BRICK_PROFILE)
        case 2: rc = launch_variant<CfgQ16x1>(l, p, dev, n_cu); break;
        case 10: rc = launch_variant<CfgQ16x2>(l, p, dev, n_cu); break;
        case 3: rc = launch_variant<CfgF32Half>(l, p, dev, n_cu); break;
        case 4: rc = launch_variant<CfgQ16X64>(l, p, dev, n_cu); break;
        case 5: rc = launch_variant<CfgQ16Z64>(l, p, dev, n_cu); break;
        case 6: rc = launch_variant<CfgQ16Y64>(l, p, dev, n_cu); break;
        case 7: rc = launch_variant<CfgF32Y64>(l, p, dev, n_cu); break;
        case 8: rc = launch_variant<CfgF32X64>(l, p, dev, n_cu); break;
        case 9: rc = launch_variant<CfgF32Z64>(l, p, dev, n_cu); break;
#endif
        default: return fail(-1, "unknown brick variant");
    }
    if (rc) return rc;
    return finish(l.who);
}

}

#if defined(DDRR_EXPERIMENTS) || defined(DDRR_BRICK_PROFILE)
extern "C" int ddrr_set_brick_variant(int v) {
    ddrr_brick::g_brick_variant = v;
    return 0;
}
extern "C" int ddrr_set_brick_times(unsigned *device_times) {
    ddrr_brick::g_brick_times = device_times;
    return 0;
}
extern "C" int ddrr_set_brick_order(const int *device_order) {
    ddrr_brick::g_brick_order = device_order;
    return 0;
}
extern "C" int ddrr_set_brick_split(int t, int s) {
    ddrr_brick::g_brick_split_t = t;
    ddrr_brick::g_brick_split_s = s < 1 ? 1 : s;
    return 0;
}
#endif
```

### diffdrr_amd/drr.py

```python
from __future__ import annotations

import math

import torch
import torch.nn as nn
from torch.utils.checkpoint import checkpoint

from . import ops
from .detector import Detector
from .pose import RigidTransform, convert, euler_world_pose
from .renderers import Siddon, Trilinear


class DRR(nn.Module):

    def __init__(
        self,
        subject,
        sdd: float,
        height: int,
        delx: float,
        width: int | None = None,
        dely: float | None = None,
        x0: float = 0.0,
        y0: float = 0.0,
        p_subsample: float | None = None,
        reshape: bool = True,
        reverse_x_axis: bool = True,
        patch_size: int | None = None,
        renderer: str = "siddon",
        voxel_shift: float = 0.5,
        persistent: bool = True,
        compile_renderer: bool = False,
        checkpoint_gradients: bool = False,
        **renderer_kwargs,
    ):
        super().__init__()
        width = height if width is None else width
        dely = delx if dely is None else dely
        n_subsample = int(height * width * p_subsample) if p_subsample is not None else None
        self.detector = Detector(sdd, height, width, delx, dely, x0, y0, subject.reorient,
                                 reverse_x_axis=reverse_x_axis, n_subsample=n_subsample)

        self.subject = subject
        affine = torch.as_tensor(subject.volume.affine, dtype=torch.float32).unsqueeze(0)
        self.register_buffer("_affine", affine, persistent=persistent)
        self.register_buffer("_affine_inverse", torch.linalg.inv(affine).contiguous(),
                             persistent=persistent)
        density = subject.density.data.squeeze().to(torch.float32).contiguous()
        self.register_buffer("density", density, persistent=persistent)
        if subject.mask is not None:
            self.register_buffer("mask", subject.mask.data.to(torch.float32).squeeze(),
                                 persistent=persistent)

        if renderer == "siddon":
            self.renderer = Siddon(voxel_shift, **renderer_kwargs)
        elif renderer == "trilinear":
            self.renderer = Trilinear(voxel_shift, **renderer_kwargs)
        else:
            raise ValueError(f"renderer must be 'siddon' or 'trilinear', not {renderer}")
        self.compile_renderer = compile_renderer
        self.reshape = reshape
        self.patch_size = patch_size
        self.checkpoint_gradients = checkpoint_gradients

    @property
    def affine(self):
        return RigidTransform(self._affine)

    @property
    def affine_inverse(self):
        return RigidTransform(self._affine_inverse)

    @property
    def n_patches(self):
        return (self.detector.height * self.detector.width) // (self.patch_size**2)

    @property
    def device(self):
        return self.density.device

    @property
    def dtype(self):
        return self.density.dtype

    def reshape_transform(self, img, batch_size):
        if self.reshape:
            if self.detector.n_subsample is None:
                img = img.view(batch_size, -1, self.detector.height, self.detector.width)
            else:
                img = reshape_subsampled_drr(img, self.detector, batch_size)
        return img

    def volume_changed(self):
        ops.invalidate_brick_workspace(self.density)

    def forward(self, *args, parameterization: str = None, convention: str = None,
                calibration: RigidTransform = None, mask_to_channels: bool = False,
                degrees: bool = False, **kwargs):
        fused = self._fused_ok(mask_to_channels, kwargs, calibration)
        if (fused and parameterization == "euler_angles" and len(args) == 2
                and all(torch.is_tensor(a) and a.dim() == 2 and a.shape[-1] == 3
                        and a.dtype == torch.float32 and ops.on_device(a) for a in args)):
            if (not mask_to_channels and calibration is None and not kwargs
                    and not (torch.is_grad_enabled() and (args[0].requires_grad or args[1].requires_grad
                                                          or self.density.requires_grad))):
                img = self._render_euler_inference(args[0], args[1], convention, degrees)
                if img is not None:
                    return self._reshape_fused(img, len(args[0]))
            if not mask_to_channels and calibration is None and not kwargs:
                img = self._render_euler_differentiable(args[0], args[1], convention, degrees)
                if img is not None:
                    return self._reshape_fused(img, len(args[0]))
            Mw = euler_world_pose(args[0], args[1], convention, self.detector._reorient,
                                  degrees=degrees)
            return self._reshape_fused(self._render_fused_Mw(Mw, calibration, mask_to_channels, **kwargs),
                                       len(Mw))
        if parameterization is None:
            pose = args[0]
        else:
            pose = convert(*args, parameterization=parameterization, convention=convention,
                           degrees=degrees)
        if fused:
            return self._reshape_fused(self._render_fused(pose, calibration, mask_to_channels, **kwargs),
                                       len(pose))
        source, target = self.detector(pose, calibration)
        self._rays_from_detector = True
        try:
            if self.checkpoint_gradients:
                img = checkpoint(self.render, self.density, source, target, mask_to_channels,
                                 **kwargs, use_reentrant=False)
            else:
                img = self.render(self.density, source, target, mask_to_channels, **kwargs)
        finally:
            self._rays_from_detector = False
        return self.reshape_transform(img, batch_size=len(pose))

    def _reshape_fused(self, img, batch_size):
        if isinstance(img, _ScatteredGrid):
            det = self.detector
            if self.reshape:
                return img.dense.view(batch_size, -1, det.height, det.width)
            return img.dense.index_select(-1, det.subsample_index())
        return self.reshape_transform(img, batch_size=batch_size)

    fuse_ray_generation = True
    _rays_from_detector = False

    def _fused_ok(self, mask_to_channels, kwargs, cal=None, dense_only=False):
        r = self.renderer
        if dense_only and self.detector.n_subsample is not None:
            return False
        if cal is not None and getattr(getattr(cal, "matrix", None), "requires_grad", False):
            return False
        kw_ok = not kwargs or (isinstance(r, Trilinear)
                               and set(kwargs) <= {"n_points", "alphamin", "alphamax"})
        return (self.fuse_ray_generation and isinstance(r, (Siddon, Trilinear))
                and r.supports_pose_entry()
                and ops.on_device(self.density) and self.density.dtype == torch.float32
                and (not mask_to_channels or getattr(self, "mask", None) is not None)
                and kw_ok and not self.checkpoint_gradients
                and (self.patch_size is None or self.n_patches >= 1)
                and min(self.detector.height, self.detector.width) >= 2)

    def _render_fused(self, pose, calibration, mask_to_channels=False, **kwargs):
        Mw = (pose.matrix @ self.detector._reorient)[:, :3, :]
        return self._render_fused_Mw(Mw, calibration, mask_to_channels, **kwargs)

    def _calibrated_points(self, calibration=None):
        det = self.detector
        grid = det.full_target()
        if calibration is not None:
            return calibration(grid)[0].detach()
        key = getattr(self, "_P_key", None)
        if key is None or key[0] is not det._calibration or key[1] != det._calibration._version \
                or key[2] is not grid or key[3] != grid._version:
            self._P_cache = det.calibration(grid)[0].detach()
            self._P_key = (det._calibration, det._calibration._version, grid, grid._version)
        return self._P_cache

    def _render_fused_Mw(self, Mw, calibration, mask_to_channels=False, **kwargs):
        det = self.detector
        P = self._calibrated_points(calibration)
        Ainv = self._affine_inverse[0, :3, :] if self._affine_inverse.dim() == 3 \
            else self._affine_inverse[:3, :]
        if self.patch_size is not None or det.n_subsample is not None:
            return self._render_sparse(Mw, P, Ainv, self.mask if mask_to_channels else None, **kwargs)
        self.renderer.detector_shape = (det.height, det.width)
        self.renderer.trust_detector_shape = True
        try:
            return self.renderer.render_poses(self.density, Mw, P, Ainv,
                                              mask=self.mask if mask_to_channels else None,
                                              **kwargs)
        finally:
            self.renderer.trust_detector_shape = False

    def _sparse_plan(self):
        det = self.detector
        H, W = det.height, det.width
        key = (H, W, self.patch_size, None if det.n_subsample is None else len(det.subsamples))
        plan = getattr(det, "_sparse_plan_cache", None)
        if plan is not None and plan[0] == key and plan[2] == det.target.device:
            return plan[1]
        idx = det.subsample_index()
        n = H * W if idx is None else int(idx.numel())
        if self.patch_size is not None:
            k = self.n_patches
            size = -(-n // k)
            bounds = [(a, min(a + size, n)) for a in range(0, n, size)]
        else:
            bounds = [(0, n)]
        host = None if idx is None else idx.cpu()
        chunks = []
        for a, b in bounds:
            if host is None:
                r0, r1 = a // W, (b - 1) // W
            else:
                r0, r1 = int(host[a:b].min()) // W, int(host[a:b].max()) // W
            if r1 == r0:
                r0, r1 = (r0, r0 + 1) if r0 + 1 < H else (r0 - 1, r0)
            whole = host is None and a == r0 * W and b == (r1 + 1) * W
            local = None if whole else (
                torch.arange(a - r0 * W, b - r0 * W, device=det.target.device) if host is None
                else idx[a:b] - r0 * W)
            chunks.append((r0, r1 - r0 + 1, local, None if host is None else idx[a:b], (a, b)))
        det._sparse_plan_cache = (key, chunks, det.target.device)
        return chunks

    def _render_sparse(self, Mw, P, Ainv, mask, **kwargs):
        from .renderers import _RaygenFn, get_alpha_minmax

        det, r = self.detector, self.renderer
        H, W = det.height, det.width
        idx = det.subsample_index()
        if isinstance(r, Siddon):
            pm = det.subsample_mask() if (idx is not None and mask is None and r.grid_path == "bricks") else None
            r.detector_shape, r.trust_detector_shape = (H, W), True
            try:
                dense = r.render_poses(self.density, Mw, P, Ainv, mask=mask, pixel_mask=pm)
            finally:
                r.trust_detector_shape = False
            if pm is not None:
                return _ScatteredGrid(dense)
            return dense if idx is None else dense.index_select(-1, idx)
        source, target, img = _RaygenFn.apply(Mw, P, Ainv)
        given = kwargs.get("alphamin") is not None and kwargs.get("alphamax") is not None
        need_grad = torch.is_grad_enabled() and (source.requires_grad or target.requires_grad)
        outs = []
        for r0, rows, local, pix, (a, b) in self._sparse_plan():
            kw = dict(kwargs)
            t_rows = target[:, r0 * W:(r0 + rows) * W]
            i_rows = img[:, r0 * W:(r0 + rows) * W]
            if not given:
                t_c = t_rows if local is None else t_rows.index_select(1, local)
                if need_grad:
                    lo, hi = get_alpha_minmax(source, t_c, r.dims(self.density), r.voxel_shift, r.eps)
                    kw["alphamin"], kw["alphamax"] = lo.min(), hi.max()
                else:
                    kw["alphamin"], kw["alphamax"] = ops.trilinear_alpha_range(
                        source.detach(), t_c.detach().contiguous(), self.density.shape,
                        voxel_shift=r.voxel_shift, eps=r.eps)
            r.detector_shape, r.trust_detector_shape = (rows, W), True
            try:
                out = r(self.density, source, t_rows.contiguous(), i_rows.contiguous(), mask=mask, **kw)
            finally:
                r.trust_detector_shape = False
            outs.append(out if local is None else out.index_select(-1, local))
        return outs[0] if len(outs) == 1 else torch.cat(outs, dim=-1)

    def _render_euler_inference(self, rot, xyz, convention, degrees):
        from .pose import _AXIS, _check_convention
        from .renderers import _brick_storage

        r, det = self.renderer, self.detector
        B = rot.shape[0]
        if not (isinstance(r, Siddon) and r.grid_path == "bricks" and not r.packed_record and B > 0
                and rot.shape == xyz.shape and rot.device == self.density.device == xyz.device):
            return None
        _check_convention(convention)
        if degrees:
            rot = rot / 180 * math.pi
        axes = tuple(_AXIS[c] for c in convention)
        P = self._calibrated_points()
        Ainv = self._affine_inverse[0, :3, :] if self._affine_inverse.dim() == 3 \
            else self._affine_inverse[:3, :]
        cfg = r._cfg(False, det=(det.height, det.width))
        with torch.no_grad():
            out = torch.empty(B, P.shape[0], dtype=torch.float32, device=rot.device)
            launch_ws = ops.launch_workspace(self.density.shape, self.density.device)
            _, source, target, img = ops.pose_raygen_forward(
                rot.detach(), xyz.detach(), axes, det._reorient[:3, :].contiguous(), Ainv, P, clear=out,
                clear_launch_ws=launch_ws)
            ops.siddon_forward_bricks(self.density, source, target, img, cfg["det"],
                                      voxel_shift=cfg["voxel_shift"], eps=cfg["eps"],
                                      storage=_brick_storage(self.density, cfg, B), out=out, launch_ws=launch_ws,
                                      cleared=True, pixel_mask=det.subsample_mask())
        if det.n_subsample is not None:
            return _ScatteredGrid(out.unsqueeze(1))
        return out.unsqueeze(1)

    def _render_euler_differentiable(self, rot, xyz, convention, degrees):
        from .pose import _AXIS, _check_convention
        from .renderers import _EulerSiddonImageFn

        r, det = self.renderer, self.detector
        B = rot.shape[0]
        if not (torch.is_grad_enabled() and (rot.requires_grad or xyz.requires_grad)
                and not self.density.requires_grad and isinstance(r, Siddon) and r.grid_path == "bricks"
                and not r.packed_record and 0 < B <= self.FUSED_NCC_MAX_POSES and rot.shape == xyz.shape
                and rot.device == self.density.device == xyz.device
                and self.patch_size is None and det.n_subsample is None and self.fuse_ray_generation):
            return None
        _check_convention(convention)
        if degrees:
            rot = rot / 180 * math.pi
        axes = tuple(_AXIS[c] for c in convention)
        P = self._calibrated_points()
        Ainv = self._affine_inverse[0, :3, :] if self._affine_inverse.dim() == 3 \
            else self._affine_inverse[:3, :]
        cfg = r._cfg(False, det=(det.height, det.width))
        out = _EulerSiddonImageFn.apply(rot, xyz, self.density, det._reorient[:3, :].contiguous(), P, Ainv,
                                        axes, cfg)
        return out.unsqueeze(1)

    FUSED_NCC_MAX_POSES = 32

    def ncc(self, fixed: torch.Tensor, rot: torch.Tensor, xyz: torch.Tensor, *,
            convention: str = "ZXY", degrees: bool = False, eps: float = 1e-5,
            reduction: str = "none") -> torch.Tensor:
        from .metrics import NormalizedCrossCorrelation2d
        from .pose import _AXIS, _check_convention
        from .renderers import _EulerSiddonNccFn

        B = rot.shape[0]
        r, det = self.renderer, self.detector
        ok = (torch.is_grad_enabled() and (rot.requires_grad or xyz.requires_grad)
              and B <= self.FUSED_NCC_MAX_POSES
              and self._fused_ok(False, {}, None, dense_only=True) and isinstance(r, Siddon)
              and r.grid_path == "bricks" and not r.packed_record and not self.density.requires_grad
              and all(torch.is_tensor(a) and a.dim() == 2 and a.shape == (B, 3)
                      and a.dtype == torch.float32 and ops.on_device(a) for a in (rot, xyz))
              and torch.is_tensor(fixed) and fixed.dim() == 4 and fixed.shape[0] in (1, B)
              and fixed.shape[1:] == (1, det.height, det.width) and fixed.dtype == torch.float32
              and fixed.device == rot.device and not fixed.requires_grad and B > 0)
        if reduction not in ("none", "sum"):
            raise ValueError(f"reduction must be 'none' or 'sum', not {reduction}")
        if not ok:
            img = self(rot, xyz, parameterization="euler_angles", convention=convention, degrees=degrees)
            if img.dim() == 3 and det.n_subsample is None:
                img = img.view(B, -1, det.height, det.width)
            vals = NormalizedCrossCorrelation2d(eps=eps)(fixed.expand(B, -1, -1, -1), img)
            if reduction == "sum":
                self.ncc_per_pose = vals.detach()
                return vals.sum()
            return vals
        _check_convention(convention)
        if degrees:
            rot = rot / 180 * math.pi
        axes = tuple(_AXIS[c] for c in convention)
        self._calibrated_points()
        Ainv = self._affine_inverse[0, :3, :] if self._affine_inverse.dim() == 3 \
            else self._affine_inverse[:3, :]
        cfg = r._cfg(False, det=(det.height, det.width))
        x1 = fixed.reshape(fixed.shape[0], det.height * det.width)
        res = _EulerSiddonNccFn.apply(rot, xyz, self.density, det._reorient[:3, :].contiguous(),
                                      self._P_cache, Ainv, x1, axes, cfg, float(eps), reduction == "sum")
        if reduction == "sum":
            total, self.ncc_per_pose = res
            return total
        return res

    @torch.no_grad()
    def marching_range(self, *args, parameterization: str = None, convention: str = None,
                       calibration: RigidTransform = None, degrees: bool = False):
        pose = args[0] if parameterization is None else convert(
            *args, parameterization=parameterization, convention=convention, degrees=degrees)
        source, target = self.detector(pose, calibration)
        source, target = self.affine_inverse(source), self.affine_inverse(target)
        r = self.renderer
        if ops.on_device(target) and target.dtype == torch.float32:
            return ops.trilinear_alpha_range(source, target, self.density.shape,
                                             voxel_shift=r.voxel_shift, eps=r.eps)
        from .renderers import get_alpha_minmax
        lo, hi = get_alpha_minmax(source, target, r.dims(self.density), r.voxel_shift, r.eps)
        return lo.min(), hi.max()

    def render(self, density: torch.Tensor, source: torch.Tensor, target: torch.Tensor,
               mask_to_channels: bool = False, **kwargs):
        img = (target - source).norm(dim=-1).unsqueeze(1)
        source = self.affine_inverse(source)
        target = self.affine_inverse(target)

        kwargs["mask"] = self.mask if mask_to_channels else None
        r = self.renderer
        unpatched = self.patch_size is None or (
            isinstance(r, Siddon) and r.supports_pose_entry() and r.grid_path == "bricks"
            and ops.on_device(density) and density.dtype == torch.float32
            and not kwargs.get("align_corners", False) and self.n_patches >= 1)
        full_grid = (self.detector.n_subsample is None and unpatched and
                     target.shape[1] == self.detector.height * self.detector.width)
        if full_grid and not self._rays_from_detector and ops.on_device(target):
            full_grid = ops.rays_form_detector_grid(source, target, self.detector.height,
                                                    self.detector.width)
        self.renderer.detector_shape = \
            (self.detector.height, self.detector.width) if full_grid else None
        self.renderer.trust_detector_shape = True
        try:
            if unpatched and (self.patch_size is None or full_grid):
                return self.renderer(density, source, target, img, **kwargs)
            partials = [
                self.renderer(density, source, t, i, **kwargs)
                for t, i in zip(target.chunk(self.n_patches, dim=1),
                                img.chunk(self.n_patches, dim=-1))
            ]
            return torch.cat(partials, dim=-1)
        finally:
            self.renderer.trust_detector_shape = False

    def set_intrinsics_(self, sdd: float = None, height: int = None, width: int = None,
                        delx: float = None, dely: float = None, x0: float = None,
                        y0: float = None, n_subsample: int = None, reverse_x_axis: bool = None):
        d = self.detector
        self.detector = Detector(
            sdd if sdd is not None else d.sdd,
            height if height is not None else d.height,
            width if width is not None else d.width,
            delx if delx is not None else d.delx,
            dely if dely is not None else d.dely,
            x0 if x0 is not None else -d.x0,
            y0 if y0 is not None else -d.y0,
            self.subject.reorient,
            n_subsample if n_subsample is not None else d.n_subsample,
            reverse_x_axis if reverse_x_axis is not None else d.reverse_x_axis,
        ).to(self.density)

    def rescale_detector_(self, scale: float):
        self.set_intrinsics_(
            height=int(self.detector.height * scale),
            width=int(self.detector.width * scale),
            delx=float(self.detector.delx / scale),
            dely=float(self.detector.dely / scale),
        )

    def perspective_projection(self, pose: RigidTransform, pts: torch.Tensor):
        extrinsic = (self.detector.reorient.compose(pose)).inverse()
        x = extrinsic(pts)
        x = torch.einsum("ij,bnj->bni", self.detector.intrinsic, x)
        x = x / x[..., -1:].clone()
# ... 29 lines not shown
```

### diffdrr_amd/ops.py

```python
from __future__ import annotations

import ctypes
import os
import weakref

import torch

from . import _lib
from ._lib import REDUCE_MAX, REDUCE_SUM, SIDDON_AUX, TRI_AUX_PLANES

_REDUCE = {"sum": REDUCE_SUM, "max": REDUCE_MAX}
_LOOKUP = {"step": _lib.LOOKUP_STEP, "mid_nearest": _lib.LOOKUP_MID_NEAREST,
           "mid_trilinear": _lib.LOOKUP_MID_TRILINEAR}


def reduce_code(reducefn) -> int:
    if isinstance(reducefn, str) and reducefn in _REDUCE:
        return _REDUCE[reducefn]
    if callable(reducefn):
        raise NotImplementedError(
            "the fused kernels reduce with 'sum' or 'max'; a callable reducefn is served by the "
            "renderer modules through the materialised per-segment / per-sample tensors "
            "(ops.siddon_segments, ops.trilinear_samples)")
    raise ValueError(f"Only supports reducefn 'sum' or 'max', not {reducefn}")
# ... 77 lines not shown

    def __init__(self, source, target, img):
        self.B, self.N, _ = target.shape
        self.source, self.target = source.contiguous(), target.contiguous()
        self.img = None if img is None else img.contiguous()
        self._held = []

    def ptr(self, t):
        if t is None:
            return None
        t = t.contiguous()
        self._held.append(t)
        return t.data_ptr()

    def vol(self, volume):
        return (self.ptr(volume), *volume.shape)

    def rays(self):
        return self.source.data_ptr(), self.source.shape[1], self.target.data_ptr(), _ptr(self.img)

    def grid(self):
        return self.source.data_ptr(), self.target.data_ptr(), _ptr(self.img)


def _rays(volume, source, target, img, dtype=torch.float32) -> _Rays:
    _check_rays(volume, source, target, img, dtype)
    return _Rays(source, target, img)


def _grid(det, N, source):
    H, W = int(det[0]), int(det[1])
    if H * W != N or source.shape[1] != 1 or min(H, W) < 2:
        raise ValueError("the brick path needs one source per pose and an H*W >= 2x2 ray grid")
    return H, W


def _channels(grad_out, B, N):
    C = grad_out.shape[1]
    if grad_out.shape != (B, C, N):
        raise ValueError(f"grad_out must be (B, C, N) = ({B}, C, {N}), got {tuple(grad_out.shape)}")
    return C


def _check_labels(labels_u8, volume=None):
    if volume is None:
        if labels_u8.dtype != torch.uint8 or labels_u8.dim() != 3:
            raise ValueError("labels must be a 3-D uint8 tensor")
    elif labels_u8.dtype != torch.uint8 or labels_u8.shape != volume.shape:
        raise ValueError("labels must be a uint8 tensor of the volume's shape")


def _grad_buffers(B, N, dtype, device, *, rays, img, alpha=None, volume_shape=None, new=torch.empty):
    def buf(want, *shape):
        return new(*shape, dtype=dtype, device=device) if want else None

    g = {"g_source": buf(rays, B, N, 3), "g_target": buf(rays, B, N, 3), "g_img": buf(img, B, N)}
    if alpha is not None:
        g["g_alpha"] = buf(alpha, B, N, 2)
    g["g_volume"] = None if volume_shape is None else \
        torch.zeros(tuple(volume_shape), dtype=dtype, device=device)
    return g


def _batch_grad(g_out, B):
    if g_out.dim() == 0 or (g_out.dim() == 1 and B > 1 and g_out.stride(0) == 0):
        return g_out, 0
    return g_out.contiguous(), 1


def _empty(B, N):
    return B == 0 or N == 0


def rays_form_detector_grid(source, target, det_h, det_w, tol=2e-3) -> bool:
    B, N, _ = target.shape
    if N != det_h * det_w or min(det_h, det_w) < 2 or source.shape[1] != 1:
        return False
    if target.numel() == 0:
        return False
    t = target.detach().reshape(B, det_h, det_w, 3)
    t00 = t[:, :1, :1]
    ei = (t[:, -1:, :1] - t00) / (det_h - 1)
    ej = (t[:, :1, -1:] - t00) / (det_w - 1)
    i = torch.arange(det_h, device=t.device, dtype=t.dtype).view(1, det_h, 1, 1)
    j = torch.arange(det_w, device=t.device, dtype=t.dtype).view(1, 1, det_w, 1)
    dev = (t00 + i * ei + j * ej - t).abs().amax()
    area = torch.linalg.cross(ei.reshape(B, 3), ej.reshape(B, 3)).norm(dim=-1).amin()
    return bool(((dev <= tol) & (area > tol * tol)).item())


def _hints(det, tile, N):
    if det is None or det[0] * det[1] != N:
        return 0, 0, 1, 64
    th, tw = default_tile() if tile is None else tile
    return int(det[0]), int(det[1]), int(th), int(tw)


def siddon_forward(volume, source, target, img, *, voxel_shift=0.5, eps=1e-8, reducefn="sum",
                   lookup="step", align_corners=False, want_aux=False, count_voxels=False,
                   det=None, tile=None):
    r = _rays(volume, source, target, img)
    B, N = r.B, r.N
    out = torch.empty(B, N, dtype=torch.float32, device=volume.device)
    aux = torch.empty(B, N, SIDDON_AUX, dtype=torch.float32, device=volume.device) \
        if want_aux else None
    nvox = torch.empty(B, N, dtype=torch.int32, device=volume.device) if count_voxels else None
    hints = _hints(det, tile, N)
    if _empty(B, N):
        return out, aux, nvox
    _launch(
        "ddrr_siddon_forward", volume.device, *r.vol(volume), *r.rays(), B, N, float(voxel_shift), float(eps),
        reduce_code(reducefn), _LOOKUP[lookup], int(bool(align_corners)), *hints,
        out.data_ptr(), _ptr(aux), _ptr(nvox))
    return out, aux, nvox


_vmax_cache = {}


def volume_absmax(volume) -> float:
    ent = _vmax_cache.get(id(volume))
    if ent is not None and ent[0]() is volume and ent[1] == volume._version:
        return ent[2]
    value = float(volume.detach().abs().max().item())
    key = id(volume)
    _vmax_cache[key] = (weakref.ref(volume, lambda _, k=key: _vmax_cache.pop(k, None)),
                        volume._version, value)
    return value


def record_blocks(B, N) -> int:
    return -(-(B * N) // _lib.REC_BLOCK_RAYS)


def _aux_layout(aux, B, N):
    if aux.shape == (B, N, SIDDON_AUX):
        return _lib.AUX_INTERLEAVED
    if aux.shape == (record_blocks(B, N), _lib.REC_BLOCK_FLOATS):
        return _lib.AUX_BLOCKED
    if aux.shape == (_lib.PACKED_AUX_PLANES, B, N):
        return _lib.AUX_PACKED
    raise ValueError(f"aux has shape {tuple(aux.shape)}: neither (B,N,8), the blocked record "
                     f"(ceil(B N / 16), 80) nor the packed one (7,B,N)")


def record_planes(aux, B, N):
    R = B * N
    blk = aux.reshape(-1, 5, 16)
    pairs = blk[:, :4].reshape(-1, 2, 2, 2, 8)
    p03 = pairs.permute(2, 3, 0, 1, 4).reshape(4, -1)
    return torch.cat([p03, blk[:, 4].reshape(1, -1)])[:, :R].reshape(5, B, N)


_BRICK_STORAGE = {"f32": _lib.BRICKS_F32, "q16": _lib.BRICKS_Q16, "q16p": _lib.BRICKS_Q16_PACKED}
_range_cache = {}


class _Workspace:
    __slots__ = ("ref", "buf", "built_version", "built_ptr", "churn", "event", "stream")

    def __init__(self, ref, buf):
        self.ref, self.buf = ref, buf
        self.built_version = None
        self.built_ptr = None
        self.churn = 0
        self.event = self.stream = None


def _workspace_entry(volume, storage):
    ent = _range_cache.get((id(volume), storage))
    if ent is not None and ent.ref() is volume and ent.buf.device == volume.device:
        return ent
    return None


def brick_workspace(volume, storage="q16"):
    key = (id(volume), storage)
    ent = _workspace_entry(volume, storage)
    n = (int(_query("ddrr_brick_workspace_bytes", *(int(d) for d in volume.shape),
                    _BRICK_STORAGE[storage])) + 3) // 4
    if ent is None or ent.buf.numel() != n:
        ent = _Workspace(weakref.ref(volume, lambda _, k=key: _range_cache.pop(k, None)),
                         torch.empty(n, dtype=torch.float32, device=volume.device))
        _range_cache[key] = ent
    valid = int(ent.built_version is not None and ent.built_version == volume._version
                and ent.built_ptr == volume.data_ptr())
    if valid and ent.event is not None and not torch.cuda.is_current_stream_capturing():
        if ent.event.query():
            ent.event = ent.stream = None
        elif torch.cuda.current_stream(volume.device) != ent.stream:
            torch.cuda.current_stream(volume.device).wait_event(ent.event)
    return ent.buf, valid


def brick_workspace_commit(volume, storage):
    ent = _workspace_entry(volume, storage)
    if ent is None or (ent.built_version == volume._version and ent.built_ptr == volume.data_ptr()):
        return
    if volume.device.type == "cuda" and torch.cuda.is_current_stream_capturing():
        return
    if ent.built_version is not None:
        ent.churn += 1
    ent.built_version = volume._version
    ent.built_ptr = volume.data_ptr()
    ent.event = ent.stream = None
    if volume.device.type == "cuda":
        ent.stream = torch.cuda.current_stream(volume.device)
        ent.event = torch.cuda.Event()
        ent.event.record(ent.stream)


def invalidate_brick_workspace(volume):
    for storage in ("q16", "q16p"):
        ent = _workspace_entry(volume, storage)
        if ent is not None:
            ent.built_version = ent.built_ptr = None


def brick_workspace_stale(volume, storage):
    ent = _workspace_entry(volume, storage)
    if ent is None or ent.built_version is None:
        return None
    return int(ent.buf[2:3].view(torch.int32).item())


def workspace_churn(volume, storage):
    ent = _workspace_entry(volume, storage)
    return ent.churn if ent is not None else 0


def brick_fallbacks(volume, storage):
    ent = _workspace_entry(volume, storage)
    if ent is None or ent.built_version is None:
        return None
    head = ent.buf[:2].view(torch.int32).tolist()
    return head[0], head[1]


def brick_storage_applies(volume) -> bool:
    return volume.dim() == 3 and volume.is_contiguous() and volume.numel() >= 4


def brick_ranges(volume):
    return brick_workspace(volume, "q16")


def brick_record_buffer(B, N, device):
    return torch.empty(record_blocks(B, N), _lib.REC_BLOCK_FLOATS, dtype=torch.float32, device=device)


def siddon_forward_bricks(volume, source, target, img, det, *, voxel_shift=0.5, eps=1e-8,
                          want_aux=False, record_vmax=0.0, storage="f32", want_image=True,
                          aux=None, out=None, launch_ws=None, cleared=False, pixel_mask=None):
    r = _rays(volume, source, target, img)
    B, N = r.B, r.N
    H, W = _grid(det, N, source)
    if storage != "f32" and not brick_storage_applies(volume):
        storage = "f32"
    need_out = want_image or not want_aux
    if out is not None and (not need_out or out.shape != (B, N) or out.dtype != torch.float32
                            or not out.is_contiguous() or out.device != volume.device):
        raise ValueError("out: a contiguous float32 (B, N) image on the volume's device, where one is written")
    if need_out and out is None:
        out = torch.empty(B, N, dtype=torch.float32, device=volume.device)
    ranges, valid = brick_workspace(volume, storage) if storage != "f32" else (None, 0)
    packed = bool(want_aux and record_vmax and record_vmax > 0.0)
    if cleared and (launch_ws is None or packed or (want_aux and aux is None)):
        raise ValueError("cleared=True: the float record (an image with it is formed from the record afterwards) "
                         "or the image, and the launch workspace, as the caller cleared them")
    if want_aux and aux is None:
        shape = (_lib.PACKED_AUX_PLANES, B, N) if packed else \
            (record_blocks(B, N), _lib.REC_BLOCK_FLOATS)
        aux = torch.empty(*shape, dtype=torch.float32, device=volume.device)
    elif not want_aux:
        aux = None
    if _empty(B, N):
        return out, aux
    if launch_ws is None:
        launch_ws = launch_workspace(volume.shape, volume.device)
    if pixel_mask is not None and (pixel_mask.dtype != torch.int32 or pixel_mask.numel() != (N + 31) // 32
                                   or not pixel_mask.is_contiguous() or pixel_mask.device != volume.device):
        raise ValueError("pixel_mask: a contiguous int32 tensor of ceil(N / 32) words on the volume's device")
    _launch(
        "ddrr_siddon_forward_bricks" if pixel_mask is None else "ddrr_siddon_forward_bricks_masked",
        volume.device, *r.vol(volume), *r.grid(), B, H, W, float(voxel_shift), float(eps),
        _ptr(out), _ptr(aux), float(record_vmax) if packed else 0.0,
        _BRICK_STORAGE[storage], _ptr(ranges), int(valid) | (_lib.BRICKS_CLEARED if cleared else 0),
        launch_ws.data_ptr(), *(() if pixel_mask is None else (pixel_mask.data_ptr(),)))
    if storage != "f32" and not valid:
        brick_workspace_commit(volume, storage)
    return out, aux


def pixel_mask_of(index, n_pixels):
    words = torch.zeros((n_pixels + 31) // 32 * 32, dtype=torch.bool, device=index.device)
    words[index] = True
    weights = (1 << torch.arange(32, dtype=torch.int64, device=index.device))
    packed = (words.view(-1, 32).to(torch.int64) * weights).sum(dim=1)
    return (packed - ((packed >> 31) << 32)).to(torch.int32).contiguous()


def siddon_backward_rays(aux, grad_out, source, target, img, *, eps=1e-8, reducefn="sum",
                         want_img_grad=True):
    B, N, _ = target.shape
    layout = _aux_layout(aux, B, N)
    g_source = torch.empty(B, N, 3, dtype=torch.float32, device=target.device)
    g_target = torch.empty(B, N, 3, dtype=torch.float32, device=target.device)
    g_img = torch.empty(B, N, dtype=torch.float32, device=target.device) if want_img_grad else None
    if not _empty(B, N):
        r = _Rays(source, target, img)
        _launch(
            "ddrr_siddon_backward_rays", target.device, aux.data_ptr(), layout, r.ptr(grad_out), *r.rays(), B, N,
            float(eps), reduce_code(reducefn), g_source.data_ptr(), g_target.data_ptr(), _ptr(g_img))
    return g_source, g_target, g_img


def pose_euler_forward(rot, xyz, axes, reorient34):
    _require_gpu(rot)
    B = rot.shape[0]
    rot, xyz, reorient34 = rot.contiguous(), xyz.contiguous(), reorient34.contiguous()
    Mw = torch.empty(B, 3, 4, dtype=torch.float32, device=rot.device)
    if B:
        _launch("ddrr_pose_euler_forward", rot.device, rot.data_ptr(), xyz.data_ptr(), *axes,
                reorient34.data_ptr(), B, Mw.data_ptr())
    return Mw


def pose_euler_backward(rot, xyz, axes, reorient34, gMw):
    B = rot.shape[0]
    rot, xyz, reorient34, gMw = (t.contiguous() for t in (rot, xyz, reorient34, gMw))
    g_rot, g_xyz = torch.empty_like(rot), torch.empty_like(xyz)
    if B:
        _launch("ddrr_pose_euler_backward", rot.device, rot.data_ptr(), xyz.data_ptr(), *axes,
                reorient34.data_ptr(), gMw.data_ptr(), B, g_rot.data_ptr(), g_xyz.data_ptr())
    return g_rot, g_xyz


def ncc_forward(x1, x2, eps):
    _require_gpu(x2)
    B, N = x2.shape
    shared = x1.shape[0] == 1 and B != 1
    x1, x2 = x1.contiguous(), x2.contiguous()
    out = torch.empty(B, dtype=torch.float32, device=x2.device)
    stats = torch.empty(B, 5, dtype=torch.float32, device=x2.device)
    if B:
        _launch("ddrr_ncc_forward", x2.device, x1.data_ptr(), 0 if shared else N, x2.data_ptr(), B,
                N, float(eps), out.data_ptr(), stats.data_ptr())
    return out, stats


def ncc_backward(x1, x2, stats, g_out, want_x1, want_x2):
    B, N = x2.shape
    shared = x1.shape[0] == 1 and B != 1
    x1, x2 = x1.contiguous(), x2.contiguous()
    g_out, g_stride = _batch_grad(g_out, B)
    g_x2 = torch.empty_like(x2) if want_x2 else None
    g_x1 = torch.empty_like(x2) if (want_x1 and not shared) else None
    if B:
        _launch("ddrr_ncc_backward", x2.device, x1.data_ptr(), 0 if shared else N, x2.data_ptr(),
                stats.data_ptr(), g_out.data_ptr(), g_stride, B, N, _ptr(g_x1), _ptr(g_x2))
    return g_x1, g_x2


def ncc_patch_forward(x1, x2, p, eps, want_coef=True):
    _require_gpu(x2)
    B, H, W = x2.shape
    shared = x1.shape[0] == 1 and B != 1
    x1, x2 = x1.contiguous(), x2.contiguous()
    out = torch.empty(B, dtype=torch.float32, device=x2.device)
    coef = torch.empty(B, H - p + 1, W - p + 1, 4, dtype=torch.float32, device=x2.device) if want_coef else None
    if B:
        _launch("ddrr_ncc_patch_forward", x2.device, x1.data_ptr(), 0 if shared else H * W, x2.data_ptr(), B,
                H, W, int(p), float(eps), out.data_ptr(), _ptr(coef))
    return out, coef


def ncc_patch_backward(x1, x2, coef, g_out, p):
    B, H, W = x2.shape
    shared = x1.shape[0] == 1 and B != 1
    x1, x2 = x1.contiguous(), x2.contiguous()
    g_out, g_stride = _batch_grad(g_out, B)
    g_x2 = torch.empty_like(x2)
    if B:
        _launch("ddrr_ncc_patch_backward", x2.device, x1.data_ptr(), 0 if shared else H * W, x2.data_ptr(),
                coef.data_ptr(), g_out.data_ptr(), g_stride, B, H, W, int(p), g_x2.data_ptr())
    return g_x2


def sobel_forward(img):
    _require_gpu(img)
    B, H, W = img.shape
    img = img.contiguous()
    out = torch.empty(B, 2, H, W, dtype=torch.float32, device=img.device)
    if B:
        _launch("ddrr_sobel_forward", img.device, img.data_ptr(), B, H, W, out.data_ptr())
    return out


def sobel_backward(g_out):
    B, _, H, W = g_out.shape
    g_out = g_out.contiguous()
    g_img = torch.empty(B, H, W, dtype=torch.float32, device=g_out.device)
    if B:
        _launch("ddrr_sobel_backward", g_out.device, g_out.data_ptr(), B, H, W, g_img.data_ptr())
    return g_img


def blur_sobel_forward(img, taps):
    _require_gpu(img)
    B, H, W = img.shape
    shared = B > 1 and img.stride(0) == 0
    if shared:
        img = img[:1]
    img = img.contiguous()
    out = torch.empty(B, 2, H, W, dtype=torch.float32, device=img.device)
    if B:
        _launch("ddrr_blur_sobel_forward", img.device, img.data_ptr(), 0 if shared else H * W, B, H, W,
                taps.data_ptr(), int(taps.numel()), out.data_ptr())
    return out


def blur_sobel_backward(g_out, taps):
    B, _, H, W = g_out.shape
    g_out = g_out.contiguous()
    g_img = torch.empty(B, H, W, dtype=torch.float32, device=g_out.device)
    if B:
        _launch("ddrr_blur_sobel_backward", g_out.device, g_out.data_ptr(), B, H, W, taps.data_ptr(),
                int(taps.numel()), g_img.data_ptr())
    return g_img


def raygen_forward(Mw, Ainv, P):
    _require_gpu(Mw)
    B, N = Mw.shape[0], P.shape[0]
    if Mw.shape[1:] != (3, 4) or Ainv.shape != (3, 4) or P.shape != (N, 3):
        raise ValueError("raygen_forward: Mw (B,3,4), Ainv (3,4), P (N,3) expected")
    for t in (Mw, Ainv, P):
        if t.dtype != torch.float32 or t.device != Mw.device:
            raise NotImplementedError("raygen_forward needs float32 tensors on one device")
    Mw, Ainv, P = Mw.contiguous(), Ainv.contiguous(), P.contiguous()
    dev = Mw.device
    source = torch.empty(B, 1, 3, dtype=torch.float32, device=dev)
    target = torch.empty(B, N, 3, dtype=torch.float32, device=dev)
# ... 1251 lines not shown
```

### diffdrr_amd/registration.py

```python
from __future__ import annotations

import torch
import torch.nn as nn

from .pose import convert


class Registration(nn.Module):
    def __init__(self, drr, rotation: torch.Tensor, translation: torch.Tensor,
                 parameterization: str, convention: str | None = None):
        super().__init__()
        self.drr = drr
        self._rotation = nn.Parameter(rotation)
        self._translation = nn.Parameter(translation)
        self.parameterization = parameterization
        self.convention = convention

    def forward(self, **kwargs):
        return self.drr(self._rotation, self._translation,
                        parameterization=self.parameterization, convention=self.convention,
                        **kwargs)

    @property
    def pose(self):
# ... 75 lines not shown

        from .metrics import NormalizedCrossCorrelation2d
        fused = (type(criterion) is NormalizedCrossCorrelation2d and criterion.patch_size is None
                 and reg.parameterization == "euler_angles" and not render_kwargs
                 and hasattr(reg.drr, "ncc") and fused_similarity)
        self.fused_similarity = bool(fused)

        one = torch.ones((), dtype=reg._rotation.dtype, device=reg._rotation.device)

        def iteration():
            optimizer.zero_grad(set_to_none=True)
            if fused:
                values = reg.drr.ncc(target, reg._rotation, reg._translation, convention=reg.convention,
                                     eps=criterion.eps)
            else:
                values = criterion(target, reg(**render_kwargs))
            loss = values.reshape(()) if values.numel() == 1 else values.sum()
            loss.backward(gradient=one)
            optimizer.step()
            return loss.detach()

        try:
            side = torch.cuda.Stream()
            side.wait_stream(torch.cuda.current_stream())
            with torch.cuda.stream(side):
                for _ in range(warmup):
                    iteration()
            torch.cuda.current_stream().wait_stream(side)
            self.graph = torch.cuda.CUDAGraph()
            cap = torch.cuda.Stream()
            cap.wait_stream(torch.cuda.current_stream())
            if fused:
                from . import ops
                with torch.cuda.stream(cap):
                    ops.siddon_ncc_workspace(reg._rotation.shape[0], reg._rotation.device)
                cap.synchronize()
            with torch.cuda.graph(self.graph, stream=cap):
                self.loss = iteration()
        finally:
            if had_static is not None:
                renderer.static_volume = had_static
        with torch.no_grad():
            for p, v in zip(params, saved_params):
                p.copy_(v)
                p.grad = None
                for name, val in optimizer.state.get(p, {}).items():
                    if torch.is_tensor(val):
                        old = saved_state[p].get(name)
                        val.copy_(old) if old is not None else val.zero_()

        self._captured_hyper = self._host_hyper()

    def _host_hyper(self):
        return [tuple(sorted((k, v) for k, v in g.items()
                             if k != "params" and isinstance(v, (bool, int, float, tuple, type(None)))))
                for g in self.optimizer.param_groups]

    def __call__(self) -> torch.Tensor:
        if self._host_hyper() != self._captured_hyper:
            raise RuntimeError(
                "GraphedIteration: the optimizer's hyper-parameters changed after capture "
                f"({self._captured_hyper} -> {self._host_hyper()}); they are baked into the graph -- "
                "build a new GraphedIteration (or use tensor-valued learning rates)")
        self.graph.replay()
        self.iterations_done += 1
        return self.loss


def normal_equations_reference(J: torch.Tensor, x: torch.Tensor, f: torch.Tensor, eps: float = 1e-5):
    J, x, f = J.double(), x.double(), f.double()
    N = x.shape[-1]
    mx, mf = x.mean(-1, keepdim=True), f.mean(-1, keepdim=True)
    vx, vf = ((x - mx) ** 2).mean(-1, keepdim=True), ((f - mf) ** 2).mean(-1, keepdim=True)
    sx, sf = (vx + eps).sqrt(), (vf + eps).sqrt()
    zx, zf = (x - mx) / sx, (f - mf) / sf
    Jc = J - J.mean(-2, keepdim=True)
    zJ = (zx.unsqueeze(-1) * J).sum(-2, keepdim=True)
    Jr = Jc / sx.unsqueeze(-1) - zx.unsqueeze(-1) * zJ / (N * sx.unsqueeze(-1))
    r = zx - zf
    return (zx * zf).mean(-1), Jr.transpose(-1, -2) @ Jr, (Jr * r.unsqueeze(-1)).sum(-2)


class LevenbergMarquardt:

    def __init__(self, reg: Registration, fixed: torch.Tensor, damping: float = 1.0, up: float = 4.0,
                 down: float = 1.0 / 3.0, damping_min: float = 1e-7, damping_max: float = 1e6, eps: float = 1e-5,
                 graph: bool = False):
        from . import ops
        from .pose import _AXIS, _check_convention
        from .renderers import Siddon

        if graph:
            raise NotImplementedError("LevenbergMarquardt: graph=True (the step as one captured HIP graph) is not "
                                      "built; run the eager step, which does not synchronise with the host either")
        self.reg = reg
        self.up, self.down, self.damping_min, self.damping_max, self.eps = (
            float(up), float(down), float(damping_min), float(damping_max), float(eps))
        if not (self.up > 1.0 and 0.0 < self.down < 1.0 and 0.0 < self.damping_min <= self.damping_max < float("inf")
                and self.damping_min <= float(damping) <= self.damping_max and self.eps >= 0.0):
            raise ValueError("LevenbergMarquardt: up > 1, 0 < down < 1, 0 < damping_min <= damping <= damping_max "
                             "< inf and eps >= 0 expected")
        drr = reg.drr
        r, det = getattr(drr, "renderer", None), getattr(drr, "detector", None)
        rot, xyz = reg._rotation, reg._translation

        def refuse(what):
            raise ValueError(f"LevenbergMarquardt: {what}")

        if reg.parameterization != "euler_angles":
            refuse(f"parameterization must be 'euler_angles', not {reg.parameterization!r}")
        _check_convention(reg.convention)
        if not isinstance(r, Siddon):
            refuse("the renderer must be Siddon")
        if r.grid_path != "bricks":
            refuse("the Siddon renderer must take the brick kernel (grid_path == 'bricks')")
        if r.packed_record:
            refuse("the packed backward record (packed_record=True) is not read; use the float record")
        if drr.density.requires_grad:
            refuse("the volume must not require a gradient")
        if drr.patch_size is not None:
            refuse("patch_size must be None")
        if det.n_subsample is not None:
            refuse("p_subsample must be None (a dense detector)")
        if not drr.fuse_ray_generation:
            refuse("fuse_ray_generation must be on")
        for name, t in (("rotation", rot), ("translation", xyz)):
            if t.dim() != 2 or t.shape[1] != 3 or t.dtype != torch.float32 or not t.is_contiguous():
                refuse(f"{name} must be a contiguous float32 (B, 3) parameter, got {tuple(t.shape)} {t.dtype}")
            if t.device != drr.density.device or not ops.on_device(t):
                refuse(f"{name} must live on the volume's device ({drr.density.device}), got {t.device}")
        B = rot.shape[0]
        if rot.shape != xyz.shape:
            refuse(f"rotation {tuple(rot.shape)} and translation {tuple(xyz.shape)} must have one shape")
        if not 0 < B <= drr.FUSED_NCC_MAX_POSES:
            refuse(f"1 ... {drr.FUSED_NCC_MAX_POSES} poses expected, got {B}")
        H, W = det.height, det.width
        if not (torch.is_tensor(fixed) and fixed.dim() == 4 and fixed.shape[0] in (1, B)
                and tuple(fixed.shape[1:]) == (1, H, W) and fixed.dtype == torch.float32):
            refuse(f"fixed must be a float32 ((1 | {B}), 1, {H}, {W}) tensor")
        if fixed.device != rot.device:
            refuse(f"fixed must live on the parameters' device ({rot.device}), got {fixed.device}")
        self.B, self.N = B, H * W
        self.axes = tuple(_AXIS[c] for c in reg.convention)
        self.fixed = fixed.detach().reshape(fixed.shape[0], H * W).contiguous()
        dev = rot.device
        self._state = ops.lm_state(B, damping, dev)
        self._ws = ops.lm_workspace(B, self.N, dev)
        self._aux = ops.brick_record_buffer(B, self.N, dev)
        self._ncc = torch.zeros(B, dtype=torch.float32, device=dev)
        self.steps_done = 0

    def _render(self):
        from . import ops
        from .renderers import _brick_storage

        drr, reg = self.reg.drr, self.reg
        r, det = drr.renderer, drr.detector
        P = drr._calibrated_points()
        Ainv = drr._affine_inverse[0, :3, :] if drr._affine_inverse.dim() == 3 else drr._affine_inverse[:3, :]
        cfg = r._cfg(False, det=(det.height, det.width))
        reorient34 = det._reorient[:3, :].contiguous()
        rot, xyz = reg._rotation.detach(), reg._translation.detach()
        launch_ws = ops.launch_workspace(drr.density.shape, drr.density.device)
        Mw, source, target, img = ops.pose_raygen_forward(rot, xyz, self.axes, reorient34, Ainv, P, clear=self._aux,
                                                          clear_launch_ws=launch_ws)
        ops.siddon_forward_bricks(drr.density, source, target, img, cfg["det"], voxel_shift=cfg["voxel_shift"],
                                  eps=cfg["eps"], want_aux=True, storage=_brick_storage(drr.density, cfg, self.B),
                                  want_image=False, aux=self._aux, launch_ws=launch_ws, cleared=True)
        return dict(aux=self._aux, source=source, Mw=Mw, Ainv=Ainv, P=P, rot=rot, xyz=xyz, axes=self.axes,
                    reorient34=reorient34), dict(eps=cfg["eps"], with_img_path=not cfg["stop_gradients"])

    @torch.no_grad()
    def _step(self, out):
        from . import ops

        args, kw = self._render()
        ops.lm_normal_sums(args.pop("aux"), self.fixed, **args, **kw, ws=self._ws)
        return ops.lm_step(self._ws, self._state, args["rot"], args["xyz"], self.N, ncc_eps=self.eps, up=self.up,
                           down=self.down, damping_min=self.damping_min, damping_max=self.damping_max, out=out)

    def step(self) -> torch.Tensor:
        out = self._step(None)
        self.steps_done += 1
        return out

    @torch.no_grad()
    def commit(self):
        valid = self._state[:, 35:36] != 0
        best = self._state[:, :6].to(torch.float32)
        self.reg._rotation.copy_(torch.where(valid, best[:, :3], self.reg._rotation))
        self.reg._translation.copy_(torch.where(valid, best[:, 3:], self.reg._translation))

    @torch.no_grad()
    def jacobian(self) -> torch.Tensor:
        from . import ops

        args, kw = self._render()
        return ops.lm_normal_sums(args.pop("aux"), self.fixed, **args, **kw, want_jacobian=True)[1]

    @property
    def damping(self) -> torch.Tensor:
        view = self._state[:, 34].detach()
        return view

    @property
    def best_parameters(self):
        best = self._state[:, :6].to(torch.float32)
        return best[:, :3], best[:, 3:]

    @property
    def best_ncc(self) -> torch.Tensor:
        return self._state[:, 6].detach()

    @property
    def accepted(self) -> torch.Tensor:
        return self._state[:, 36] != 0
```

### diffdrr_amd/renderers.py

```python
from __future__ import annotations

import weakref

import torch

from . import ops


def _grid_or_none(renderer, source, target):
    det = renderer.detector_shape
    if det is None or renderer.trust_detector_shape:
        return det
    return det if ops.rays_form_detector_grid(source, target, int(det[0]), int(det[1])) else None


_label_cache = {}


def _labels_u8(mask: torch.Tensor):
    ent = _label_cache.get(id(mask))
    if ent is not None and ent[0]() is mask and ent[1] == mask._version:
        return ent[2]
    C = int(mask.max().item()) + 1
    if C <= 256:
        chunks = [(mask.to(torch.uint8).contiguous(), C, 0)]
    else:
        lab = mask.to(torch.int64)
        chunks = [(torch.where(lab < 255, lab, torch.full_like(lab, 255)).to(torch.uint8).contiguous(),
                   255, 0)]
        for c0 in range(255, C, 254):
            n = min(254, C - c0)
            inside = (lab >= c0) & (lab < c0 + n)
            chunks.append((torch.where(inside, lab - c0 + 1, torch.zeros_like(lab))
                           .to(torch.uint8).contiguous(), n + 1, 1))
    key = id(mask)
    _label_cache[key] = (weakref.ref(mask, lambda _, k=key: _label_cache.pop(k, None)),
                         mask._version, chunks)
    return chunks


def _volume_gradient(volume, source, target, img, grad_out, cfg):
    N = target.shape[1]
    grid = (cfg["lookup"] == "step" and cfg["reducefn"] == "sum" and cfg["det"] is not None
            and cfg["det"][0] * cfg["det"][1] == N and source.shape[1] == 1
            and min(cfg["det"]) >= 2)
    if grid and cfg["path"] == "bricks":
        return ops.siddon_backward_volume_bricks(
            volume.shape, source, target, img, grad_out, cfg["det"],
            voxel_shift=cfg["voxel_shift"], eps=cfg["eps"])
    return ops.siddon_backward_volume(
        volume, source, target, img, grad_out, voxel_shift=cfg["voxel_shift"], eps=cfg["eps"],
        reducefn=cfg["reducefn"], det=cfg["det"], tile=cfg["tile"])


def _record_vmax(volume, want_aux, cfg):
    if not want_aux or not cfg.get("packed_record", False) or volume.requires_grad:
        return 0.0
    return ops.volume_absmax(volume)


_cu_count = {}


_FEW_BRICKS_POLICY = ((1.5, 1, 5), (2.5, 1, 1 << 30), (4.0, 8, 12))


def _few_bricks_take_q16(per_cu: float, poses) -> bool:
    if poses is None:
        return False
    lo, hi = next((a, b) for r, a, b in _FEW_BRICKS_POLICY if per_cu < r)
    return lo <= int(poses) <= hi


def _brick_storage(volume, cfg, poses=None):
    storage = cfg.get("storage", "f32")
    if storage not in ("q16", "q16p") or volume.requires_grad:
        return "f32"
    if not ops.brick_storage_applies(volume):
        return "f32"
    dev = volume.device
    if (dev.type == "cuda" and torch.cuda.is_current_stream_capturing()
            and not cfg.get("static_volume", False)):
        return "f32"
    if dev.type == "cuda":
        if dev not in _cu_count:
            _cu_count[dev] = torch.cuda.get_device_properties(dev).multi_processor_count
        dx, dy, dz = volume.shape
        per_cu = (-(-dx // 32)) * (-(-dy // 32)) * (-(-dz // 64)) / _cu_count[dev]
        if per_cu < 4 and not _few_bricks_take_q16(per_cu, poses):
            return "f32"
    if ops.workspace_churn(volume, storage) >= 3:
        return "f32"
    return storage


class _SiddonFn(torch.autograd.Function):

    @staticmethod
    def forward(ctx, volume, source, target, img, cfg):
        need_rays = any(ctx.needs_input_grad[1:4])
        want_aux = bool(need_rays and cfg["lookup"] == "step")
        N = target.shape[1]
        grid = (cfg["lookup"] == "step" and cfg["reducefn"] == "sum" and cfg["det"] is not None
                and cfg["det"][0] * cfg["det"][1] == N and source.shape[1] == 1
                and min(cfg["det"]) >= 2)
        if grid and cfg["path"] == "bricks":
            out, aux = ops.siddon_forward_bricks(
                volume, source, target, img, cfg["det"], voxel_shift=cfg["voxel_shift"],
                eps=cfg["eps"], want_aux=want_aux, record_vmax=_record_vmax(volume, want_aux, cfg),
                storage=_brick_storage(volume, cfg, source.shape[0]))
        else:
            out, aux, _ = ops.siddon_forward(
                volume, source, target, img, voxel_shift=cfg["voxel_shift"], eps=cfg["eps"],
                reducefn=cfg["reducefn"], lookup=cfg["lookup"],
                align_corners=cfg["align_corners"], want_aux=want_aux, det=cfg["det"],
                tile=cfg["tile"])
        ctx.cfg = cfg
        ctx.has_aux = want_aux
        ctx.save_for_backward(volume, source, target, img, aux if want_aux else None)
        return out

    @staticmethod
    def backward(ctx, grad_out):
        volume, source, target, img, aux = ctx.saved_tensors
        cfg = ctx.cfg
        need_vol, need_s, need_t, need_i = ctx.needs_input_grad[:4]
        stop = cfg["stop_gradients"]
        if cfg["lookup"] != "step":
            if cfg["reducefn"] != "sum":
                raise NotImplementedError("gradients of the midpoint lookups need reducefn='sum'")
            if stop:
                raise NotImplementedError("stop_gradients_through_grid_sample is implemented for "
                                          "mode='nearest', align_corners=False")
            gs, gt, gi, gv = ops.siddon_backward_midpoint(
                volume, source, target, img, grad_out, voxel_shift=cfg["voxel_shift"],
                eps=cfg["eps"], lookup=cfg["lookup"], align_corners=cfg["align_corners"],
                want_rays=bool(need_s or need_t), want_img=bool(need_i),
                want_volume=bool(need_vol))
            g_s = None
            if need_s:
                g_s = gs.sum(dim=1, keepdim=True) if source.shape[1] == 1 else gs
            return gv, g_s, (gt if need_t else None), \
                (gi.view_as(img) if need_i else None), None
        g_vol = g_s = g_t = g_i = None
        grad_out = grad_out.contiguous()
        if need_s or need_t or need_i:
            gs, gt, gi = ops.siddon_backward_rays(
                aux, grad_out, source, target, img, eps=cfg["eps"], reducefn=cfg["reducefn"],
                want_img_grad=bool(need_i and not stop))
            if need_s:
                g_s = gs.sum(dim=1, keepdim=True) if source.shape[1] == 1 else gs
            if need_t:
                g_t = gt
            if need_i and not stop:
                g_i = gi.view_as(img)
        if need_vol and not stop:
            g_vol = _volume_gradient(volume, source, target, img, grad_out, cfg)
        return g_vol, g_s, g_t, g_i, None


class _SiddonF64Fn(torch.autograd.Function):

    @staticmethod
    def forward(ctx, volume, source, target, img, cfg):
        need_rays = any(ctx.needs_input_grad[1:4])
        out, aux = ops.siddon_forward_f64(
            volume, source, target, img, voxel_shift=cfg["voxel_shift"], eps=cfg["eps"],
            reducefn=cfg["reducefn"], want_aux=bool(need_rays and cfg["reducefn"] == "sum"))
        ctx.cfg = cfg
        ctx.save_for_backward(volume, source, target, img, aux)
        return out

    @staticmethod
    def backward(ctx, grad_out):
        volume, source, target, img, aux = ctx.saved_tensors
        cfg = ctx.cfg
        if cfg["reducefn"] != "sum":
            raise NotImplementedError("float64 gradients are implemented for reducefn='sum'")
        need_vol, need_s, need_t, need_i = ctx.needs_input_grad[:4]
        stop = cfg["stop_gradients"]
        gs, gt, gi, gv = ops.siddon_backward_f64(
            volume.shape, source, target, img, grad_out.contiguous(), aux,
            voxel_shift=cfg["voxel_shift"], eps=cfg["eps"], want_rays=bool(need_s or need_t),
            want_img=bool(need_i and not stop), want_volume=bool(need_vol and not stop))
        g_s = None
        if need_s:
            g_s = gs.sum(dim=1, keepdim=True) if source.shape[1] == 1 else gs
        return gv, g_s, (gt if need_t else None), (gi.view_as(img) if gi is not None else None), None


class _TrilinearF64Fn(torch.autograd.Function):

    @staticmethod
    def forward(ctx, volume, source, target, img, alphamin, alphamax, cfg):
        out = ops.trilinear_forward_f64(volume, source, target, img, alphamin, alphamax,
                                        n_points=cfg["n_points"], voxel_shift=cfg["voxel_shift"],
                                        eps=cfg["eps"])
        ctx.cfg = cfg
        ctx.save_for_backward(volume, source, target, img, alphamin, alphamax)
        return out

    @staticmethod
    def backward(ctx, grad_out):
        volume, source, target, img, alphamin, alphamax = ctx.saved_tensors
        cfg = ctx.cfg
        need_vol, need_s, need_t, need_i, need_a0, need_a1 = ctx.needs_input_grad[:6]
        r = ops.trilinear_backward_f64(
            volume, source, target, img, grad_out, alphamin, alphamax, n_points=cfg["n_points"],
            voxel_shift=cfg["voxel_shift"], eps=cfg["eps"], want_rays=bool(need_s or need_t),
            want_img=bool(need_i), want_alpha=bool(need_a0 or need_a1), want_volume=bool(need_vol))
        g_s = g_t = g_a0 = g_a1 = g_i = None
        if need_s:
            g_s = r["g_source"].sum(dim=1, keepdim=True) if source.shape[1] == 1 \
                else r["g_source"]
        if need_t:
            g_t = r["g_target"]
        if need_i:
            g_i = r["g_img"].view_as(img)
        if need_a0 or need_a1:
            ga = r["g_alpha"].sum(dim=(0, 1))
            g_a0 = ga[0].reshape(alphamin.shape) if need_a0 else None
            g_a1 = ga[1].reshape(alphamax.shape) if need_a1 else None
        return r["g_volume"], g_s, g_t, g_i, g_a0, g_a1, None


class _SiddonChannelsFn(torch.autograd.Function):

    @staticmethod
    def forward(ctx, volume, source, target, img, labels, C, cfg):
        out = _channels_forward(volume, labels, C, source, target, img, cfg)
        ctx.cfg = cfg
        ctx.save_for_backward(volume, source, target, img, labels)
        return out

    @staticmethod
    def backward(ctx, grad_out):
        volume, source, target, img, labels = ctx.saved_tensors
        cfg = ctx.cfg
        need_vol, need_s, need_t, need_i = ctx.needs_input_grad[:4]
        stop = cfg["stop_gradients"]
        want_vol = bool(need_vol and not stop)
        B, C, N = grad_out.shape
        if _channels_use_bricks(cfg, source, N) and ops.channels_fit_bricks(B, C, N):
            gs = gt = gi = gv = None
            if need_s or need_t or (need_i and not stop):
                gs, gt, gi = ops.siddon_backward_channels_bricks(
                    volume, labels, source, target, img, grad_out, cfg["det"],
                    voxel_shift=cfg["voxel_shift"], eps=cfg["eps"], want_img=bool(need_i and not stop))
            if want_vol:
                gv = ops.siddon_backward_channels_volume_bricks(
                    labels, source, target, img, grad_out, cfg["det"],
                    voxel_shift=cfg["voxel_shift"], eps=cfg["eps"]).to(volume.dtype)
        else:
            gs, gt, gi, gv = ops.siddon_backward_channels(
                volume, labels, source, target, img, grad_out, voxel_shift=cfg["voxel_shift"],
                eps=cfg["eps"], want_rays=bool(need_s or need_t), want_img=bool(need_i and not stop),
                want_volume=want_vol, det=cfg["det"], tile=cfg["tile"])
        g_s = g_t = None
        if need_s:
            g_s = gs.sum(dim=1, keepdim=True) if source.shape[1] == 1 else gs
        if need_t:
            g_t = gt
        g_i = gi.view_as(img) if gi is not None else None
        return gv, g_s, g_t, g_i, None, None, None


class _SiddonSegmentsFn(torch.autograd.Function):

    @staticmethod
    def forward(ctx, volume, source, target, img, cfg):
        terms = ops.siddon_segments(volume, source, target, img, voxel_shift=cfg["voxel_shift"],
                                    eps=cfg["eps"])
        ctx.cfg = cfg
        ctx.save_for_backward(volume, source, target, img)
        return terms.transpose(1, 2)

    @staticmethod
    def backward(ctx, grad):
        volume, source, target, img = ctx.saved_tensors
        cfg = ctx.cfg
        need_vol, need_s, need_t, need_i = ctx.needs_input_grad[:4]
        stop = cfg["stop_gradients"]
        gs, gt, gi, gv = ops.siddon_segments_backward(
            volume, source, target, img, grad.transpose(1, 2), voxel_shift=cfg["voxel_shift"],
            eps=cfg["eps"], want_rays=bool(need_s or need_t), want_img=bool(need_i and not stop),
            want_volume=bool(need_vol and not stop))
        g_s = g_t = None
        if need_s:
            g_s = gs.sum(dim=1, keepdim=True) if source.shape[1] == 1 else gs
        if need_t:
            g_t = gt
        g_i = gi.view_as(img) if gi is not None else None
        return gv, g_s, g_t, g_i, None


class _SiddonTermsFn(torch.autograd.Function):

    @staticmethod
    def forward(ctx, volume, source, target, img, cfg):
        terms = ops.siddon_segments_general(
            volume, source, target, img, voxel_shift=cfg["voxel_shift"], eps=cfg["eps"],
            lookup=cfg["lookup"], align_corners=cfg["align_corners"])
        ctx.cfg = cfg
        ctx.save_for_backward(volume, source, target, img)
        return terms.transpose(1, 2)

    @staticmethod
    def backward(ctx, grad):
        volume, source, target, img = ctx.saved_tensors
        cfg = ctx.cfg
        need_vol, need_s, need_t, need_i = ctx.needs_input_grad[:4]
        through = not cfg["stop_gradients"]
        gs, gt, gi, gv = ops.siddon_segments_general_backward(
            volume, source, target, img, grad.transpose(1, 2), voxel_shift=cfg["voxel_shift"],
            eps=cfg["eps"], lookup=cfg["lookup"], align_corners=cfg["align_corners"],
            through_lookup=through, want_rays=bool(need_s or need_t), want_img=bool(need_i),
            want_volume=bool(need_vol))
        g_s = None
        if need_s:
            g_s = gs.sum(dim=1, keepdim=True) if source.shape[1] == 1 else gs
        return gv, g_s, (gt if need_t else None), \
            (gi.view_as(img) if gi is not None and need_i else None), None


def _scatter_channels(terms, labels, mask):
    B, _, N = terms.shape
    C = int(mask.max().item()) + 1
    return torch.zeros(B, C, N, dtype=terms.dtype, device=terms.device).scatter_add_(1, labels, terms)


def _reduce_terms(terms, reducefn):
    if reducefn == "sum":
        return terms.sum(dim=-1)
    if reducefn == "max":
        return terms.max(dim=-1).values
    if callable(reducefn):
        return reducefn(terms)
    raise ValueError(f"Only supports reducefn 'sum' or 'max', not {reducefn}")


class _SiddonPoseFn(torch.autograd.Function):

    @staticmethod
    def forward(ctx, volume, Mw, P, Ainv, cfg):
        source, target, img = ops.raygen_forward(Mw, Ainv, P)
        want_aux = bool(ctx.needs_input_grad[1])
        if cfg["path"] == "bricks":
            out, aux = ops.siddon_forward_bricks(
                volume, source, target, img, cfg["det"], voxel_shift=cfg["voxel_shift"],
                eps=cfg["eps"], want_aux=want_aux, record_vmax=_record_vmax(volume, want_aux, cfg),
                storage=_brick_storage(volume, cfg, source.shape[0]), pixel_mask=cfg.get("pixel_mask"))
        else:
            out, aux, _ = ops.siddon_forward(
                volume, source, target, img, voxel_shift=cfg["voxel_shift"], eps=cfg["eps"],
                want_aux=want_aux, det=cfg["det"], tile=cfg["tile"])
        ctx.cfg = cfg
        ctx.save_for_backward(volume, Mw, P, Ainv, source, target, img, aux)
        return out

    @staticmethod
    def backward(ctx, grad_out):
        volume, Mw, P, Ainv, source, target, img, aux = ctx.saved_tensors
        cfg = ctx.cfg
        need_vol, need_M = ctx.needs_input_grad[:2]
        stop = cfg["stop_gradients"]
        g_vol = g_M = None
        grad_out = grad_out.contiguous()
        if need_M:
            g_M = ops.siddon_backward_pose(aux, grad_out, source, target, img, Mw, Ainv, P,
                                           eps=cfg["eps"], with_img_path=not stop)
        if need_vol and not stop:
            pm = cfg.get("pixel_mask")
            if pm is not None:
                grad_out = grad_out * _pixel_mask_bits(pm, grad_out.shape[-1]).to(grad_out.dtype)
            g_vol = _volume_gradient(volume, source, target, img, grad_out, cfg)
        return g_vol, g_M, None, None, None


def _pixel_mask_bits(pixel_mask, n_pixels):
    shifts = torch.arange(32, dtype=torch.int32, device=pixel_mask.device)
    return ((pixel_mask.unsqueeze(-1) >> shifts) & 1).view(-1)[:n_pixels].bool()


class _EulerSiddonNccFn(torch.autograd.Function):

    @staticmethod
    def forward(ctx, rot, xyz, volume, reorient34, P, Ainv, fixed, axes, cfg, ncc_eps, reduce_sum=False):
        B, N = rot.shape[0], P.shape[0]
        aux = ops.brick_record_buffer(B, N, rot.device)
        launch_ws = ops.launch_workspace(volume.shape, volume.device)
        some = B > 0 and N > 0
        Mw, source, target, img = ops.pose_raygen_forward(rot, xyz, axes, reorient34, Ainv, P,
                                                          clear=aux if some else None,
                                                          clear_launch_ws=launch_ws if some else None)
        ops.siddon_forward_bricks(
            volume, source, target, img, cfg["det"], voxel_shift=cfg["voxel_shift"], eps=cfg["eps"],
            want_aux=True, storage=_brick_storage(volume, cfg, B), want_image=False, aux=aux,
            launch_ws=launch_ws, cleared=some)
        ncc, stats, _, total = ops.siddon_ncc_forward(aux, img, fixed, ncc_eps, want_sum=True) if reduce_sum \
            else (*ops.siddon_ncc_forward(aux, img, fixed, ncc_eps), None)
        ctx.axes, ctx.cfg = axes, cfg
        ctx.save_for_backward(rot, xyz, reorient34, P, Ainv, fixed, Mw, source, target, img, aux, stats)
        if reduce_sum:
            ctx.mark_non_differentiable(ncc)
            ctx.set_materialize_grads(False)
            return total, ncc
        return ncc

    @staticmethod
    def backward(ctx, g, _g_values=None):
        if g is None:
            return (None,) * 11
        rot, xyz, reorient34, P, Ainv, fixed, Mw, source, target, img, aux, stats = ctx.saved_tensors
        g_rot, g_xyz = ops.siddon_ncc_backward_pose(
            aux, img, fixed, stats, g, source, target, Mw, Ainv, P, rot, xyz, ctx.axes, reorient34,
            eps=ctx.cfg["eps"], with_img_path=not ctx.cfg["stop_gradients"])
        return g_rot, g_xyz, None, None, None, None, None, None, None, None, None


class _EulerSiddonImageFn(torch.autograd.Function):

    @staticmethod
    def forward(ctx, rot, xyz, volume, reorient34, P, Ainv, axes, cfg):
        B, N = rot.shape[0], P.shape[0]
        aux = ops.brick_record_buffer(B, N, rot.device)
        launch_ws = ops.launch_workspace(volume.shape, volume.device)
        Mw, source, target, img = ops.pose_raygen_forward(rot, xyz, axes, reorient34, Ainv, P,
                                                          clear=aux, clear_launch_ws=launch_ws)
        out, _ = ops.siddon_forward_bricks(
            volume, source, target, img, cfg["det"], voxel_shift=cfg["voxel_shift"], eps=cfg["eps"],
            want_aux=True, storage=_brick_storage(volume, cfg, B), aux=aux, launch_ws=launch_ws, cleared=True)
        ctx.axes, ctx.cfg = axes, cfg
        ctx.save_for_backward(rot, xyz, reorient34, P, Ainv, Mw, source, aux)
        return out

    @staticmethod
    def backward(ctx, g):
        rot, xyz, reorient34, P, Ainv, Mw, source, aux = ctx.saved_tensors
        g_rot, g_xyz = ops.siddon_backward_pose_euler(
            aux, g, source, Mw, Ainv, P, rot, xyz, ctx.axes, reorient34, eps=ctx.cfg["eps"],
            with_img_path=not ctx.cfg["stop_gradients"])
        return g_rot, g_xyz, None, None, None, None, None, None


def _cat_channels(blocks):
    blocks = list(blocks)
    return blocks[0] if len(blocks) == 1 else torch.cat(blocks, dim=1)


def _chunk(block, k0):
    return block if k0 == 0 else block[:, k0:]


def _channels_use_bricks(cfg, source, N):
    grid = (cfg["det"] is not None and cfg["det"][0] * cfg["det"][1] == N
            and source.shape[1] == 1 and min(cfg["det"]) >= 2)
    return bool(grid and cfg["path"] == "bricks" and cfg.get("channels_on_bricks", True))


def _channels_forward(volume, labels, C, source, target, img, cfg):
    B, N = target.shape[:2]
    if _channels_use_bricks(cfg, source, N) and ops.channels_fit_bricks(B, C, N):
        words = None
        if (cfg.get("channel_words", True) and not volume.requires_grad and volume.is_contiguous()
                and labels.is_contiguous() and B > 0
                and not (volume.device.type == "cuda" and torch.cuda.is_current_stream_capturing())):
            words = ops.channel_words(volume, labels, C, build=False)
        return ops.siddon_forward_channels_bricks(
            volume, labels, C, source, target, img, cfg["det"],
            voxel_shift=cfg["voxel_shift"], eps=cfg["eps"], words=words)
    return ops.siddon_forward_channels(
        volume, labels, C, source.contiguous(), target.contiguous(), img.contiguous(),
        voxel_shift=cfg["voxel_shift"], eps=cfg["eps"], det=cfg["det"], tile=cfg["tile"])


class _RaygenFn(torch.autograd.Function):

    @staticmethod
    def forward(ctx, Mw, P, Ainv):
        source, target, img = ops.raygen_forward(Mw, Ainv, P)
        ctx.save_for_backward(Mw, P, Ainv, img)
        ctx.set_materialize_grads(False)
        return source, target, img

    @staticmethod
    def backward(ctx, gs, gt, gi):
        Mw, P, Ainv, img = ctx.saved_tensors
        if not ctx.needs_input_grad[0]:
            return None, None, None
        A, R = Ainv[:, :3], Mw[:, :, :3]
        B, N = img.shape
        g_tw = gt @ A if gt is not None else Mw.new_zeros(B, N, 3)
        g_sw = gs.sum(dim=1) @ A if gs is not None else Mw.new_zeros(B, 3)
        if gi is not None:
            ku = (gi / img.clamp_min(1e-30)).unsqueeze(-1) * (P @ R.transpose(1, 2))
            g_tw = g_tw + ku
            g_sw = g_sw - ku.sum(dim=1)
        g_R = torch.einsum("bna,nj->baj", g_tw, P)
        g_T = g_tw.sum(dim=1) + g_sw
        return torch.cat([g_R, g_T.unsqueeze(-1)], dim=-1), None, None


class Siddon(torch.nn.Module):

    def __init__(
        self,
        voxel_shift: float = 0.5,
        mode: str = "nearest",
        stop_gradients_through_grid_sample: bool = False,
        filter_intersections_outside_volume: bool = False,
        reducefn: str = "sum",
        eps: float = 1e-8,
    ):
        super().__init__()
        if mode not in ("nearest", "bilinear"):
            raise ValueError(f"mode must be 'nearest' or 'bilinear', not {mode}")
        self.mode = mode
        self.stop_gradients_through_grid_sample = stop_gradients_through_grid_sample
        self.filter_intersections_outside_volume = filter_intersections_outside_volume
        self.reducefn = reducefn
        self.voxel_shift = voxel_shift
        self.eps = eps
        self.detector_shape = None
        self.trust_detector_shape = False
        self.tile = None
        self.grid_path = "bricks"
        self.packed_record = False
        self.brick_storage = "q16p"
        self.static_volume = False
        self.channels_on_bricks = True
        self.channel_words = True

    def dims(self, volume):
        return torch.tensor(volume.shape).to(volume)

    @staticmethod
    def volume_changed(volume):
        ops.invalidate_brick_workspace(volume)

    def _cfg(self, align_corners, det="unchecked", reducefn=None):
        if self.mode == "bilinear":
            lookup = "mid_trilinear"
        elif align_corners:
            lookup = "mid_nearest"
        else:
            lookup = "step"
        reducefn = self.reducefn if reducefn is None else reducefn
        ops.reduce_code(reducefn)
        return {"voxel_shift": self.voxel_shift, "eps": self.eps, "reducefn": reducefn,
                "lookup": lookup, "align_corners": bool(align_corners),
                "stop_gradients": self.stop_gradients_through_grid_sample,
                "det": self.detector_shape if det == "unchecked" else det, "tile": self.tile,
                "path": self.grid_path,
                "packed_record": self.packed_record, "storage": self.brick_storage,
                "static_volume": self.static_volume,
                "channels_on_bricks": self.channels_on_bricks, "channel_words": self.channel_words}

    def supports_pose_entry(self):
        return self.mode == "nearest" and self.reducefn == "sum"

    def render_poses(self, volume, Mw, P, Ainv, mask=None, pixel_mask=None):
        cfg = self._cfg(False)
        if pixel_mask is not None and mask is None and cfg["path"] == "bricks":
            cfg["pixel_mask"] = pixel_mask
        if mask is not None:
            source, target, img = _RaygenFn.apply(Mw, P, Ainv)
            return _cat_channels(_chunk(_SiddonChannelsFn.apply(volume, source, target, img, labels, C, cfg), k0)
                                 for labels, C, k0 in _labels_u8(mask))
        return _SiddonPoseFn.apply(volume, Mw, P, Ainv, cfg).unsqueeze(1)

    def _general(self, volume, source, target, img, lookup, align_corners, mask):
        B, N, _ = target.shape
        dt = volume.dtype
        source, target = source.to(dt), target.to(dt)
        gcfg = {"voxel_shift": self.voxel_shift, "eps": self.eps, "lookup": lookup,
                "align_corners": bool(align_corners),
                "stop_gradients": self.stop_gradients_through_grid_sample}
        terms = _SiddonTermsFn.apply(volume, source, target, img.reshape(B, N).to(dt), gcfg)
        if mask is None:
            return _reduce_terms(terms, self.reducefn).unsqueeze(1)
        labels = ops.siddon_segments_general(
            mask.to(dt), source.detach(), target.detach(), None, voxel_shift=self.voxel_shift,
            eps=self.eps, lookup=lookup, align_corners=align_corners, raw=True).long()
        return _scatter_channels(terms.transpose(1, 2), labels, mask)

    def forward(self, volume, source, target, img, align_corners=False, mask=None):
        B, N, _ = target.shape
        user_reduce = callable(self.reducefn) and not isinstance(self.reducefn, str)
        f64 = volume.dtype == torch.float64
        if self.mode == "bilinear":
            lookup = "mid_trilinear"
        else:
            lookup = "mid_nearest" if align_corners else "step"
        if mask is not None:
            if f64 or lookup != "step":
                return self._general(volume, source, target, img, lookup, align_corners, mask)
            cfg = self._cfg(align_corners, _grid_or_none(self, source, target), reducefn="sum")
            return _cat_channels(_chunk(_SiddonChannelsFn.apply(volume, source, target, img.reshape(B, N),
                                                                labels, C, cfg), k0)
                                 for labels, C, k0 in _labels_u8(mask))
        if user_reduce:
            if f64 or lookup != "step":
                return self._general(volume, source, target, img, lookup, align_corners, None)
            cfg = {"voxel_shift": self.voxel_shift, "eps": self.eps,
                   "stop_gradients": self.stop_gradients_through_grid_sample}
            terms = _SiddonSegmentsFn.apply(volume, source, target, img.reshape(B, N), cfg)
            return self.reducefn(terms).unsqueeze(1)
        cfg = self._cfg(align_corners, _grid_or_none(self, source, target))
        wants_grad = torch.is_grad_enabled() and any(
            t.requires_grad for t in (volume, source, target, img))
        if f64:
            if lookup != "step" or (wants_grad and self.reducefn != "sum"):
                return self._general(volume, source, target, img, lookup, align_corners, None)
            out = _SiddonF64Fn.apply(volume, source.to(volume), target.to(volume),
                                     img.reshape(B, N).to(volume), cfg)
            return out.unsqueeze(1)
        if lookup != "step" and wants_grad and (
                self.reducefn != "sum" or self.stop_gradients_through_grid_sample):
            return self._general(volume, source, target, img, lookup, align_corners, None)
        out = _SiddonFn.apply(volume, source, target, img.reshape(B, N), cfg)
        return out.unsqueeze(1)


def get_alpha_minmax(source, target, dims, voxel_shift, eps):
    sdd = target - source + eps
    lo_plane = -voxel_shift
    hi_plane = dims.to(source) + 1 - voxel_shift
    a0 = (lo_plane - source) / sdd
    a1 = (hi_plane - source) / sdd
    alphamin = torch.minimum(a0, a1).amax(dim=-1, keepdim=True).clamp_min(0.0)
    alphamax = torch.maximum(a0, a1).amin(dim=-1, keepdim=True).clamp_max(1.0)
    return alphamin, alphamax


class _TrilinearFn(torch.autograd.Function):

    @staticmethod
    def _grid(cfg, source, target):
        N = target.shape[1]
        return (cfg["bricks"] and cfg["mode"] == "bilinear" and cfg["reducefn"] == "sum"
                and not cfg["align_corners"] and cfg["det"] is not None
                and cfg["det"][0] * cfg["det"][1] == N and source.shape[1] == 1
                and min(cfg["det"]) >= 2)

    @staticmethod
    def forward(ctx, volume, source, target, img, alphamin, alphamax, cfg):
        aux = None
        if _TrilinearFn._grid(cfg, source, target):
            want_aux = any(ctx.needs_input_grad[1:6])
            res = ops.trilinear_forward_bricks(
                volume, source, target, img, alphamin, alphamax, cfg["det"],
                n_points=cfg["n_points"], voxel_shift=cfg["voxel_shift"], eps=cfg["eps"],
                want_aux=want_aux)
            out, aux = res if want_aux else (res, None)
        else:
            out = ops.trilinear_forward(
                volume, source.contiguous(), target.contiguous(), img.contiguous(), alphamin,
                alphamax, n_points=cfg["n_points"], voxel_shift=cfg["voxel_shift"],
                eps=cfg["eps"], reducefn=cfg["reducefn"], mode=cfg["mode"],
                align_corners=cfg["align_corners"], det=cfg["det"], tile=cfg["tile"])
        ctx.cfg = cfg
        ctx.save_for_backward(volume, source, target, img, alphamin, alphamax, aux)
        return out

    @staticmethod
    def backward(ctx, grad_out):
        volume, source, target, img, alphamin, alphamax, aux = ctx.saved_tensors
        cfg = ctx.cfg
        need_vol, need_s, need_t, need_i, need_a0, need_a1 = ctx.needs_input_grad[:6]
        need_rays = need_s or need_t or need_i or need_a0 or need_a1
        g_vol_bricks = None
        if need_vol and _TrilinearFn._grid(cfg, source, target):
            g_vol_bricks = ops.trilinear_backward_volume_bricks(
                volume.shape, source, target, img, grad_out, alphamin, alphamax, cfg["det"],
                n_points=cfg["n_points"], voxel_shift=cfg["voxel_shift"], eps=cfg["eps"])
            need_vol = False
            if not need_rays:
                return g_vol_bricks, None, None, None, None, None, None
        if aux is not None and not need_vol:
            r = ops.trilinear_backward_rays(
                aux, grad_out, source, target, img, alphamin, alphamax, n_points=cfg["n_points"],
                eps=cfg["eps"], want_rays=bool(need_s or need_t), want_img=bool(need_i),
                want_alpha=bool(need_a0 or need_a1))
        else:
            r = ops.trilinear_backward(
                volume, source.contiguous(), target.contiguous(), img.contiguous(), grad_out,
                alphamin, alphamax, n_points=cfg["n_points"], voxel_shift=cfg["voxel_shift"],
                eps=cfg["eps"], mode=cfg["mode"], align_corners=cfg["align_corners"],
                want_rays=bool(need_s or need_t), want_img=bool(need_i),
                want_alpha=bool(need_a0 or need_a1), want_volume=bool(need_vol), det=cfg["det"],
                tile=cfg["tile"], reducefn=cfg["reducefn"])
        g_s = g_t = g_a0 = g_a1 = g_i = None
        if need_s:
            g_s = r["g_source"].sum(dim=1, keepdim=True) if source.shape[1] == 1 \
                else r["g_source"]
        if need_t:
            g_t = r["g_target"]
        if need_i:
            g_i = r["g_img"].view_as(img)
        if need_a0 or need_a1:
            ga = r["g_alpha"].sum(dim=(0, 1))
            g_a0 = ga[0].reshape(alphamin.shape) if need_a0 else None
            g_a1 = ga[1].reshape(alphamax.shape) if need_a1 else None
        return (g_vol_bricks if g_vol_bricks is not None else r["g_volume"]), g_s, g_t, g_i, \
            g_a0, g_a1, None


# ... 237 lines not shown
```

### include/diffdrr_hip.h

```cpp
#ifndef DIFFDRR_HIP_H
#define DIFFDRR_HIP_H

#ifdef __cplusplus
extern "C" {
#endif

#define DDRR_ABI_VERSION 33

#define DDRR_REDUCE_SUM 0
#define DDRR_REDUCE_MAX 1

#define DDRR_LOOKUP_STEP 0
#define DDRR_LOOKUP_MID_NEAREST 1
#define DDRR_LOOKUP_MID_TRILINEAR 2

#define DDRR_SIDDON_AUX 8

#define DDRR_AUX_INTERLEAVED 0
#define DDRR_AUX_BLOCKED 1
#define DDRR_REC_BLOCK_RAYS 16
#define DDRR_REC_BLOCK_FLOATS 80
#define DDRR_AUX_PACKED 2
#define DDRR_PACKED_AUX_PLANES 7
#define DDRR_TRI_AUX_PLANES 7

int ddrr_abi_version(void);
const char *ddrr_last_error(void);

int ddrr_siddon_forward(const float *volume, int dx, int dy, int dz, const float *source,
                        int src_n, const float *target, const float *img, int B, int N,
                        float voxel_shift, float eps, int reduce_mode, int lookup_mode,
                        int align_corners, int det_h, int det_w, int tile_h, int tile_w,
                        float *out, float *aux, int *n_vox, void *stream);

#define DDRR_BRICKS_F32 0
#define DDRR_BRICKS_Q16 1
#define DDRR_BRICKS_Q16_PACKED 2
#define DDRR_BRICKS_CLEARED 2
long ddrr_brick_workspace_bytes(int dx, int dy, int dz, int brick_storage);
long ddrr_brick_launch_workspace_bytes(int dx, int dy, int dz);
int ddrr_siddon_forward_bricks(const float *volume, int dx, int dy, int dz, const float *source,
                               const float *target, const float *img, int B, int det_h,
                               int det_w, float voxel_shift, float eps, float *out, float *aux,
                               float record_vmax, int brick_storage, float *brick_ranges,
                               int ranges_valid, void *launch_ws, void *stream);
int ddrr_siddon_forward_bricks_masked(const float *volume, int dx, int dy, int dz, const float *source,
                                      const float *target, const float *img, int B, int det_h,
                                      int det_w, float voxel_shift, float eps, float *out, float *aux,
                                      float record_vmax, int brick_storage, float *brick_ranges,
                                      int ranges_valid, void *launch_ws, const unsigned *pixel_mask,
                                      void *stream);

int ddrr_siddon_backward_volume_bricks(int dx, int dy, int dz, const float *source,
                                       const float *target, const float *img,
                                       const float *grad_out, int B, int det_h, int det_w,
                                       float voxel_shift, float eps, float *g_volume,
                                       void *launch_ws, void *stream);

int ddrr_siddon_backward_rays(const float *aux, int aux_layout, const float *grad_out,
                              const float *source, int src_n, const float *target,
                              const float *img, int B, int N, float eps, int reduce_mode,
                              float *g_source, float *g_target, float *g_img, void *stream);

int ddrr_siddon_backward_volume(const float *volume, int dx, int dy, int dz, const float *source,
                                int src_n, const float *target, const float *img,
                                const float *grad_out, int B, int N, float voxel_shift, float eps,
                                int reduce_mode, int det_h, int det_w, int tile_h, int tile_w,
                                float *g_volume, void *stream);

int ddrr_siddon_backward_midpoint(const float *volume, int dx, int dy, int dz, const float *source,
                                  int src_n, const float *target, const float *img,
                                  const float *grad_out, int B, int N, float voxel_shift,
                                  float eps, int lookup_mode, int align_corners, float *g_source,
                                  float *g_target, float *g_img, float *g_volume, void *stream);

int ddrr_siddon_forward_channels(const float *volume, const unsigned char *labels, int dx, int dy,
                                 int dz, const float *source, int src_n, const float *target,
                                 const float *img, int B, int N, int C, float voxel_shift,
                                 float eps, int det_h, int det_w, int tile_h, int tile_w,
                                 float *out, void *stream);

int ddrr_siddon_forward_channels_bricks(const float *volume, const unsigned char *labels, int dx,
                                        int dy, int dz, const float *source, const float *target,
                                        const float *img, int B, int det_h, int det_w, int C,
                                        float voxel_shift, float eps, float *out, void *launch_ws,
                                        void *stream);
long ddrr_channel_words_state_bytes(void);
int ddrr_channel_words(const float *volume, const unsigned char *labels, long n_voxels, int C, float *words,
                       void *state, int force, void *stream);
int ddrr_siddon_forward_channels_bricks_words(const float *words, int dx, int dy, int dz, const float *source,
                                              const float *target, const float *img, int B, int det_h,
                                              int det_w, int C, float voxel_shift, float eps, float *out,
                                              void *launch_ws, void *stream);

int ddrr_siddon_backward_channels_bricks(const float *volume, const unsigned char *labels, int dx,
                                         int dy, int dz, const float *source, const float *target,
                                         const float *grad_out, int B, int det_h, int det_w, int C,
                                         float voxel_shift, float eps, float *aux, void *launch_ws,
                                         void *stream);

int ddrr_trilinear_backward_channels_bricks(const float *volume, const unsigned char *labels,
                                            int dx, int dy, int dz, const float *source,
                                            const float *target, const float *grad_out, int B,
                                            int det_h, int det_w, int C, float voxel_shift,
                                            float eps, int n_points, const float *alphamin,
                                            const float *alphamax, float *aux, void *launch_ws,
                                            void *stream);

int ddrr_siddon_backward_channels_volume_bricks(const unsigned char *labels, int dx, int dy, int dz,
                                                const float *source, const float *target,
                                                const float *img, const float *grad_out, int B,
                                                int det_h, int det_w, int C, float voxel_shift,
                                                float eps, float *g_volume, void *launch_ws,
                                                void *stream);

int ddrr_trilinear_backward_channels_volume_bricks(const unsigned char *labels, int dx, int dy,
                                                   int dz, const float *source, const float *target,
                                                   const float *img, const float *grad_out, int B,
                                                   int det_h, int det_w, int C, float voxel_shift,
                                                   float eps, int n_points, const float *alphamin,
                                                   const float *alphamax, float *g_volume,
                                                   void *launch_ws, void *stream);

int ddrr_siddon_backward_channels(const float *volume, const unsigned char *labels, int dx,
                                  int dy, int dz, const float *source, int src_n,
                                  const float *target, const float *img, const float *grad_out,
                                  int B, int N, int C, float voxel_shift, float eps, int det_h,
                                  int det_w, int tile_h, int tile_w, float *g_source,
                                  float *g_target, float *g_img, float *g_volume, void *stream);

int ddrr_siddon_segments(const float *volume, int dx, int dy, int dz, const float *source,
                         int src_n, const float *target, const float *img, int B, int N,
                         float voxel_shift, float eps, float *terms, void *stream);
int ddrr_siddon_segments_backward(const float *volume, int dx, int dy, int dz, const float *source,
                                  int src_n, const float *target, const float *img,
                                  const float *grad_terms, int B, int N, float voxel_shift,
                                  float eps, float *g_source, float *g_target, float *g_img,
                                  float *g_volume, void *stream);

int ddrr_trilinear_alpha_range(const float *source, int src_n, const float *target, int B, int N,
                               int dx, int dy, int dz, float voxel_shift, float eps,
                               float *range2, void *stream);

int ddrr_trilinear_forward(const float *volume, int dx, int dy, int dz, const float *source,
                           int src_n, const float *target, const float *img, int B, int N,
                           float voxel_shift, float eps, int n_points, const float *alphamin,
                           const float *alphamax, int mode_nearest, int reduce_mode,
                           int align_corners, int det_h, int det_w, int tile_h, int tile_w,
                           float *out, void *stream);

int ddrr_trilinear_forward_channels(const float *volume, const unsigned char *labels, int dx,
                                    int dy, int dz, const float *source, int src_n,
                                    const float *target, const float *img, int B, int N, int C,
                                    float voxel_shift, float eps, int n_points,
                                    const float *alphamin, const float *alphamax,
                                    int align_corners, int det_h, int det_w, int tile_h,
                                    int tile_w, float *out, void *stream);

int ddrr_trilinear_forward_bricks(const float *volume, int dx, int dy, int dz,
                                  const float *source, const float *target, const float *img,
                                  int B, int det_h, int det_w, float voxel_shift, float eps,
                                  int n_points, const float *alphamin, const float *alphamax,
                                  float *out, float *aux, void *launch_ws, void *stream);

int ddrr_trilinear_forward_channels_bricks(const float *volume, const unsigned char *labels,
                                           int dx, int dy, int dz, const float *source,
                                           const float *target, const float *img, int B,
                                           int det_h, int det_w, int C, float voxel_shift,
                                           float eps, int n_points, const float *alphamin,
                                           const float *alphamax, float *out, void *launch_ws,
                                           void *stream);
int ddrr_trilinear_backward_rays(const float *aux, const float *grad_out, const float *source,
                                 const float *target, const float *img, int B, int N, float eps,
                                 int n_points, const float *alphamin, const float *alphamax,
                                 float *g_source, float *g_target, float *g_img, float *g_alpha,
                                 void *stream);
int ddrr_trilinear_backward_volume_bricks(int dx, int dy, int dz, const float *source,
                                          const float *target, const float *img,
                                          const float *grad_out, int B, int det_h, int det_w,
                                          float voxel_shift, float eps, int n_points,
                                          const float *alphamin, const float *alphamax,
                                          float *g_volume, void *launch_ws, void *stream);

int ddrr_trilinear_backward(const float *volume, int dx, int dy, int dz, const float *source,
                            int src_n, const float *target, const float *img,
                            const float *grad_out, int B, int N, float voxel_shift, float eps,
                            int n_points, const float *alphamin, const float *alphamax,
                            int mode_nearest, int align_corners, int det_h, int det_w, int tile_h,
                            int tile_w, float *g_source, float *g_target, float *g_img,
                            float *g_alpha, float *g_volume, void *stream);
// ... 149 lines not shown
```

Before: 22510 DRRs/s.

## Add Y-elongated Q16 brick variant chosen automatically from the detector view axis

Adds a 32x64x32 Q16 brick configuration whose fp32 fallback halves split along Y instead of Z, with its own packed workspace and walk thresholds. The Python side derives the dominant view axis from the detector orientation and picks the Y-long bricks when the view runs along Y, the batch is large enough and the brick count covers the CUs. The aim is to make brick shapes line up better with the ray direction, so rays cross fewer bricks and brick loads are reused more. It adds another kernel instantiation and a second workspace layout, and it only takes effect when the view axis comes out as Y.

```diff
diff --git a/diffdrr_amd/_lib.py b/diffdrr_amd/_lib.py
--- a/diffdrr_amd/_lib.py
+++ b/diffdrr_amd/_lib.py
@@ -101,6 +101,7 @@
 REC_BLOCK_RAYS, REC_BLOCK_FLOATS = HEADER.constants("REC_BLOCK_RAYS", "REC_BLOCK_FLOATS")
 BRICKS_F32, BRICKS_Q16, BRICKS_Q16_PACKED, BRICKS_CLEARED = HEADER.constants(
     "BRICKS_F32", "BRICKS_Q16", "BRICKS_Q16_PACKED", "BRICKS_CLEARED")
+BRICKS_Q16_Y, BRICKS_Q16_PACKED_Y = HEADER.constants("BRICKS_Q16_Y", "BRICKS_Q16_PACKED_Y")
 PACKED_AUX_PLANES, TRI_AUX_PLANES = HEADER.constants("PACKED_AUX_PLANES", "TRI_AUX_PLANES")
 
 
diff --git a/diffdrr_amd/csrc/brick_shared.h b/diffdrr_amd/csrc/brick_shared.h
--- a/diffdrr_amd/csrc/brick_shared.h
+++ b/diffdrr_amd/csrc/brick_shared.h
@@ -14,17 +14,19 @@
 constexpr int kQueueCap = 128;
 constexpr int kBuckets = 3;
 #if defined(DDRR_EXPERIMENTS) && defined(DDRR_RECORD_GROUP)
-constexpr int kRecordGroup = DDRR_RECORD_GROUP;
-#else
-constexpr int kRecordGroup = 4;
+constexpr int kRecordGroup = DDRR_RECORD_GROUP, kRecordGroupY = DDRR_RECORD_GROUP;
+#else
+constexpr int kRecordGroup = 4, kRecordGroupY = 4;
 #endif
 #if defined(DDRR_EXPERIMENTS) && defined(DDRR_RECORD_ALIGN)
-constexpr int kRecordAlign = DDRR_RECORD_ALIGN;
-#else
-constexpr int kRecordAlign = 4;
-#endif
-static_assert(kRecordGroup == 8 || kRecordGroup == 4 || kRecordGroup == 2 || kRecordGroup == 1, "DPP maxima");
-static_assert(kRecordAlign == 8 || kRecordAlign == 4 || kRecordAlign == 2 || kRecordAlign == 1, "a power of two, at most a run of the record");
+constexpr int kRecordAlign = DDRR_RECORD_ALIGN, kRecordAlignY = DDRR_RECORD_ALIGN;
+#else
+constexpr int kRecordAlign = 4, kRecordAlignY = 4;
+#endif
+constexpr float kBrickT1Y = 26.f, kBrickT2Y = 56.f;
+constexpr bool record_width_ok(int n) { return n == 8 || n == 4 || n == 2 || n == 1; }
+static_assert(record_width_ok(kRecordGroup) && record_width_ok(kRecordGroupY), "DPP maxima");
+static_assert(record_width_ok(kRecordAlign) && record_width_ok(kRecordAlignY), "a power of two, at most a run of the record");
 
 struct BrickArgs {
     const float *vol;
@@ -210,7 +212,7 @@
 };
 
 struct FwdStorage {
-    int variant, packed;
+    int variant, packed, y_long;
     float *brick_ranges;
     int ranges_valid;
     float *clear;
diff --git a/diffdrr_amd/csrc/bricks.hip b/diffdrr_amd/csrc/bricks.hip
--- a/diffdrr_amd/csrc/bricks.hip
+++ b/diffdrr_amd/csrc/bricks.hip
@@ -1140,8 +1140,9 @@
     if (int rc = check_detector(det_h, det_w)) return rc;
     if (!(record_vmax >= 0.f)) return fail(-1, "record_vmax must be >= 0");
     if (brick_storage != DDRR_BRICKS_F32 && brick_storage != DDRR_BRICKS_Q16 &&
-        brick_storage != DDRR_BRICKS_Q16_PACKED)
-        return fail(-1, "brick_storage must be DDRR_BRICKS_F32, DDRR_BRICKS_Q16 or DDRR_BRICKS_Q16_PACKED");
+        brick_storage != DDRR_BRICKS_Q16_PACKED && brick_storage != DDRR_BRICKS_Q16_Y &&
+        brick_storage != DDRR_BRICKS_Q16_PACKED_Y)
+        return fail(-1, "brick_storage must be DDRR_BRICKS_F32, DDRR_BRICKS_Q16[_Y] or DDRR_BRICKS_Q16_PACKED[_Y]");
     if (brick_storage != DDRR_BRICKS_F32 && !brick_ranges)
         return fail(-1, "DDRR_BRICKS_Q16 needs the brick_ranges workspace");
     if (B == 0) return 0;
@@ -1164,8 +1165,9 @@
                            eps, l.rec_q, aux);
     }
     FwdStorage fs;
-    fs.packed = brick_storage == DDRR_BRICKS_Q16_PACKED;
-    fs.variant = fs.packed ? DDRR_BRICKS_Q16 : brick_storage;
+    fs.packed = brick_storage == DDRR_BRICKS_Q16_PACKED || brick_storage == DDRR_BRICKS_Q16_PACKED_Y;
+    fs.y_long = brick_storage == DDRR_BRICKS_Q16_Y || brick_storage == DDRR_BRICKS_Q16_PACKED_Y;
+    fs.variant = brick_storage == DDRR_BRICKS_F32 ? DDRR_BRICKS_F32 : DDRR_BRICKS_Q16;
     fs.brick_ranges = brick_ranges;
     fs.ranges_valid = ranges_valid & 1;
     fs.clear = packed || cleared ? nullptr : (aux ? aux : out);
diff --git a/diffdrr_amd/csrc/bricks_fwd.hip b/diffdrr_amd/csrc/bricks_fwd.hip
--- a/diffdrr_amd/csrc/bricks_fwd.hip
+++ b/diffdrr_amd/csrc/bricks_fwd.hip
@@ -26,13 +26,20 @@
     static constexpr int WGS_PER_CU = 1024 / THREADS;
     static constexpr int LDS_BUDGET = 160 * 1024 / WGS_PER_CU;
     static constexpr int QUEUE_BYTES = WAVES * kBuckets * kQueueCap * 4;
-    static constexpr int HZ = BZ / 2;
-    static constexpr int FSY = HZ * 4 + 4, FSX = BY * FSY + 4;
+    static constexpr int HAXIS = BY_ > BZ_ ? 1 : 2;
+    static constexpr int HLEN = (HAXIS == 1 ? BY : BZ) / 2;
+    static constexpr int HY = HAXIS == 1 ? BY / 2 : BY, HZ = HAXIS == 2 ? BZ / 2 : BZ;
+    static constexpr int FSY = HZ * 4 + 4, FSX = HY * FSY + 4;
     static constexpr int FALLBACK_BYTES = (BX * FSX + 15) / 16 * 16;
     static constexpr bool MIXED =
-        Q16 && HZ % 4 == 0 && (BX * BY * (HZ / 4)) % THREADS == 0 &&
+        Q16 && HZ % 4 == 0 && (BX * HY * (HZ / 4)) % THREADS == 0 &&
         FALLBACK_BYTES + QUEUE_BYTES + 16 + 8 * 20 * 4 <= LDS_BUDGET;
-    using Half = FwdCfg<BX_, BY_, BZ_ / 2, THREADS_, false>;
+    using Half = FwdCfg<BX_, HY, HZ, THREADS_, false>;
+    static constexpr int RECORD_GROUP = HAXIS == 1 ? kRecordGroupY : kRecordGroup;
+    static constexpr int RECORD_ALIGN = HAXIS == 1 ? kRecordAlignY : kRecordAlign;
+    static constexpr bool DOUBLE_Q16 = Q16 && BX == 32 && BY * BZ == 32 * 64;
+    static constexpr float T1 = DOUBLE_Q16 ? (HAXIS == 1 ? kBrickT1Y : 22.f) : 18.f;
+    static constexpr float T2 = DOUBLE_Q16 ? (HAXIS == 1 ? kBrickT2Y : 48.f) : 40.f;
     static constexpr int LDS_BRICK = MIXED && FALLBACK_BYTES > BRICK_BYTES ? FALLBACK_BYTES : BRICK_BYTES;
     static constexpr int ROW_ROOM = (LDS_BUDGET - LDS_BRICK - QUEUE_BYTES - 48) / (20 * 4);
     static constexpr int CHUNK = ROW_ROOM >= 32 ? 32 : ROW_ROOM;
@@ -518,8 +525,8 @@
             n_sub = 1;
             if (C::MIXED) {
                 f32_brick = stale || (known ? la_f32 : (p.fallback && p.fallback[brick_id] != 0));
-                const int z0 = (brick_id % nbz) * C::BZ;
-                n_sub = f32_brick && p.D.z - z0 > C::HZ ? 2 : 1;
+                const int a0 = C::HAXIS == 1 ? ((brick_id / nbz) % nby) * C::BY : (brick_id % nbz) * C::BZ;
+                n_sub = f32_brick && (C::HAXIS == 1 ? p.D.y : p.D.z) - a0 > C::HLEN ? 2 : 1;
             }
         }
         const bool last_part = sub + 1 >= n_sub;
@@ -552,8 +559,9 @@
         DDRR_PROF(PROF_CLAIM);
         Box box = cfg_brick_box<C>(p.D, nby, nbz, brick_id);
         if (C::MIXED && f32_brick) {
-            box.lo[2] += sub * C::HZ;
-            box.hi[2] = box.lo[2] + C::HZ < box.hi[2] ? box.lo[2] + C::HZ : box.hi[2];
+            constexpr int A = C::HAXIS;
+            box.lo[A] += sub * C::HLEN;
+            box.hi[A] = box.lo[A] + C::HLEN < box.hi[A] ? box.lo[A] + C::HLEN : box.hi[A];
         }
         const BoxF cells = boxf(box);
         StepGeom SG;
@@ -593,7 +601,7 @@
                 const PoseGrid pg = pose_grid(p.source + (long)(b0 + tid) * 3,
                                               p.target + (long)(b0 + tid) * N * 3, det_h, det_w);
                 PixBox pb = project_brick_grid(pg, det_h, det_w, cells, p.shift);
-                if (GROUPED && kRecordAlign > 1 && !(p.dbg & 1024)) pb = align_pixbox_rows(pb, det_w, kRecordAlign);
+                if (GROUPED && C::RECORD_ALIGN > 1 && !(p.dbg & 1024)) pb = align_pixbox_rows(pb, det_w, C::RECORD_ALIGN);
                 rows[tid] = fwd_row(brick_row(pg, pb, cells, p.shift, p.eps, 0.f));
             }
             if (tid == 0) counter[0] = 0;
@@ -659,13 +667,13 @@
                     if constexpr (SUB) hit = hit && ((p.pix_mask[pix >> 5] >> (pix & 31)) & 1u) != 0u;
                     float n_grp = hit ? n_est : 0.f;
                     if (GROUPED) {
-                        if constexpr (kRecordGroup >= 2)
+                        if constexpr (C::RECORD_GROUP >= 2)
                             n_grp = fmaxf(n_grp, __builtin_bit_cast(float, __builtin_amdgcn_update_dpp(
                                 0, __builtin_bit_cast(int, n_grp), 0xB1, 0xf, 0xf, true)));
-                        if constexpr (kRecordGroup >= 4)
+                        if constexpr (C::RECORD_GROUP >= 4)
                             n_grp = fmaxf(n_grp, __builtin_bit_cast(float, __builtin_amdgcn_update_dpp(
                                 0, __builtin_bit_cast(int, n_grp), 0x4E, 0xf, 0xf, true)));
-                        if constexpr (kRecordGroup >= 8)
+                        if constexpr (C::RECORD_GROUP >= 8)
                             n_grp = fmaxf(n_grp, __builtin_bit_cast(float, __builtin_amdgcn_update_dpp(
                                 0, __builtin_bit_cast(int, n_grp), 0x141, 0xf, 0xf, true)));
                     }
@@ -787,8 +795,9 @@
         } else if (C::MIXED && half_of >= 0) {
             if constexpr (C::MIXED) {
                 Box nbox = cfg_brick_box<C>(p.D, nby, nbz, half_of);
-                nbox.lo[2] += half_sub * C::HZ;
-                nbox.hi[2] = nbox.lo[2] + C::HZ < nbox.hi[2] ? nbox.lo[2] + C::HZ : nbox.hi[2];
+                constexpr int A = C::HAXIS;
+                nbox.lo[A] += half_sub * C::HLEN;
+                nbox.hi[A] = nbox.lo[A] + C::HLEN < nbox.hi[A] ? nbox.lo[A] + C::HLEN : nbox.hi[A];
                 pf.clear();
                 pf.template half<typename C::Half>(p, brick, nbox, tid_ld, true);
                 pf_kind = 2;
@@ -1050,12 +1059,14 @@
 
 using CfgF32 = FwdCfg<32, 32, 32, 1024, false>;
 using CfgQ16Z64 = FwdCfg<32, 32, 64, 1024, true>;
+using CfgQ16Y64 = FwdCfg<32, 64, 32, 1024, true>;
+static_assert(CfgQ16Z64::MIXED && CfgQ16Y64::MIXED && CfgQ16Y64::HAXIS == 1 && CfgQ16Z64::HAXIS == 2, "fp32 halves");
+static_assert(CfgQ16Y64::FALLBACK_BYTES == CfgQ16Z64::FALLBACK_BYTES, "the same image of a half");
 #if defined(DDRR_EXPERIMENTS) || defined(DDRR_BRICK_PROFILE)
 using CfgQ16x2 = FwdCfg<32, 32, 32, 512, true>;
 using CfgQ16x1 = FwdCfg<32, 32, 32, 1024, true>;
 using CfgF32Half = FwdCfg<32, 32, 16, 512, false, 0>;
 using CfgQ16X64 = FwdCfg<64, 32, 32, 1024, true>;
-using CfgQ16Y64 = FwdCfg<32, 64, 32, 1024, true>;
 using CfgF32Y64 = FwdCfg<16, 64, 32, 1024, false>;
 using CfgF32X64 = FwdCfg<64, 16, 32, 1024, false>;
 using CfgF32Z64 = FwdCfg<16, 32, 64, 1024, false>;
@@ -1087,17 +1098,24 @@
     return kWsHeaderBytes + (n32_bricks(dx, dy, dz) * 3 * (long)sizeof(float) + 255) / 256 * 256 + kFingerprintBytes;
 }
 
+template <class C>
+static long packed_bytes(int dx, int dy, int dz) {
+    return (long)((dx + C::BX - 1) / C::BX) * ((dy + C::BY - 1) / C::BY) * ((dz + C::BZ - 1) / C::BZ) * C::BRICK_BYTES;
+}
+
 long brick_workspace_bytes(int dx, int dy, int dz, int brick_storage) {
     if (brick_storage == DDRR_BRICKS_F32) return 0;
     long n = ranges_bytes(dx, dy, dz);
-    if (brick_storage == DDRR_BRICKS_Q16_PACKED)
-        n += (long)((dx + CfgQ16Z64::BX - 1) / CfgQ16Z64::BX) * ((dy + CfgQ16Z64::BY - 1) / CfgQ16Z64::BY) *
-             ((dz + CfgQ16Z64::BZ - 1) / CfgQ16Z64::BZ) * CfgQ16Z64::BRICK_BYTES;
+    if (brick_storage == DDRR_BRICKS_Q16_PACKED) n += packed_bytes<CfgQ16Z64>(dx, dy, dz);
+    if (brick_storage == DDRR_BRICKS_Q16_PACKED_Y) n += packed_bytes<CfgQ16Y64>(dx, dy, dz);
     return n;
 }
 
 template <class C, bool PRE = false>
-static int launch_variant(const BrickLaunch &l, const BrickArgs &p, int dev, int n_cu) {
+static int launch_variant(const BrickLaunch &l, const BrickArgs &args, int dev, int n_cu) {
+    BrickArgs p = args;
+    p.t1 = g_brick_t1 * (C::T1 / 18.f);
+    p.t2 = g_brick_t2 * (C::T2 / 40.f);
     if (p.pix_mask)
         return l.aux ? launch_cfg<true, C, PRE, true>(p, dev, n_cu, l.out, l.aux, l.st)
                      : launch_cfg<false, C, PRE, true>(p, dev, n_cu, l.out, l.aux, l.st);
@@ -1105,8 +1123,14 @@
                  : launch_cfg<false, C, PRE, false>(p, dev, n_cu, l.out, l.aux, l.st);
 }
 
+template <class C>
+static int launch_q16(const BrickLaunch &l, const BrickArgs &p, int dev, int n_cu) {
+    return l.B <= 8 ? launch_variant<C, true>(l, p, dev, n_cu) : launch_variant<C>(l, p, dev, n_cu);
+}
+
 int launch_fwd_bricks(const BrickLaunch &l, const FwdStorage &s) {
     int variant = s.variant, ranges_valid = s.ranges_valid;
+    bool y_long = s.y_long != 0, packed_ok = s.packed != 0;
     const bool vec_ok = (l.dz & 3) == 0 && (reinterpret_cast<uintptr_t>(l.volume) & 15) == 0;
     const bool quads_ok = l.dz >= 4 && (long)l.dx * l.dy * l.dz >= 4 && (reinterpret_cast<uintptr_t>(l.volume) & 3) == 0;
     bool few_f32 = variant == DDRR_BRICKS_F32 && l.B < 8;
@@ -1116,6 +1140,8 @@
         variant = g_brick_variant;
         if (variant != last_variant) ranges_valid = 0;
         last_variant = variant;
+        y_long = false;
+        if (!(variant == DDRR_BRICKS_Q16 || variant == 5) && !(variant == 6 && s.y_long)) packed_ok = false;
         few_f32 = false;
     }
 #endif
@@ -1133,7 +1159,7 @@
     p.ranges = ws ? ws + kWsHeaderBytes / sizeof(float) : nullptr;
     p.fallback = ws ? reinterpret_cast<const int *>(p.ranges + 2 * n32_bricks(l.dx, l.dy, l.dz)) : nullptr;
     p.ranges_valid = ranges_valid;
-    p.packed = s.packed && ws ? reinterpret_cast<const unsigned char *>(ws) + ranges_bytes(l.dx, l.dy, l.dz)
+    p.packed = packed_ok && ws ? reinterpret_cast<const unsigned char *>(ws) + ranges_bytes(l.dx, l.dy, l.dz)
                               : nullptr;
     p.fingerprint = ws ? reinterpret_cast<const unsigned *>(reinterpret_cast<const unsigned char *>(ws) +
                                                             ranges_bytes(l.dx, l.dy, l.dz) - kFingerprintBytes)
@@ -1145,18 +1171,13 @@
     p.split_t = g_brick_split_t;
     p.split_s = g_brick_split_s;
 #endif
-    if (variant == DDRR_BRICKS_Q16 || variant == 5) {
-        p.t1 = g_brick_t1 * (22.f / 18.f);
-        p.t2 = g_brick_t2 * (48.f / 40.f);
-    }
     int dev = 0, n_cu = 0;
     if (int rc = brick_launch_resources(l, p, dev, n_cu, false)) return rc;
     int rc = 0;
     switch (variant) {
         case DDRR_BRICKS_F32: rc = launch_variant<CfgF32>(l, p, dev, n_cu); break;
         case DDRR_BRICKS_Q16:
-            rc = l.B <= 8 ? launch_variant<CfgQ16Z64, true>(l, p, dev, n_cu)
-                          : launch_variant<CfgQ16Z64>(l, p, dev, n_cu);
+            rc = y_long ? launch_q16<CfgQ16Y64>(l, p, dev, n_cu) : launch_q16<CfgQ16Z64>(l, p, dev, n_cu);
             break;
 #if defined(DDRR_EXPERIMENTS) || defined(DDRR_BRICK_PROFILE)
         case 2: rc = launch_variant<CfgQ16x1>(l, p, dev, n_cu); break;
diff --git a/diffdrr_amd/drr.py b/diffdrr_amd/drr.py
--- a/diffdrr_amd/drr.py
+++ b/diffdrr_amd/drr.py
@@ -59,10 +59,19 @@
             self.renderer = Trilinear(voxel_shift, **renderer_kwargs)
         else:
             raise ValueError(f"renderer must be 'siddon' or 'trilinear', not {renderer}")
+        if isinstance(self.renderer, Siddon):
+            self.renderer.view_axis = self._view_axis()
         self.compile_renderer = compile_renderer
         self.reshape = reshape
         self.patch_size = patch_size
         self.checkpoint_gradients = checkpoint_gradients
+
+    def _view_axis(self):
+        with torch.no_grad():
+            ends = torch.tensor([[[0.0, 0.0, 0.0], [0.0, 0.0, 1.0]]])
+            ends = self.affine_inverse(self.detector.reorient(ends))
+            d = (ends[0, 1] - ends[0, 0]).abs()
+        return "xyz"[int(torch.argmax(d))]
 
     @property
     def affine(self):
@@ -270,7 +279,7 @@
 
     def _render_euler_inference(self, rot, xyz, convention, degrees):
         from .pose import _AXIS, _check_convention
-        from .renderers import _brick_storage
+        from .renderers import _brick_axis, _brick_storage
 
         r, det = self.renderer, self.detector
         B = rot.shape[0]
@@ -293,7 +302,8 @@
                 clear_launch_ws=launch_ws)
             ops.siddon_forward_bricks(self.density, source, target, img, cfg["det"],
                                       voxel_shift=cfg["voxel_shift"], eps=cfg["eps"],
-                                      storage=_brick_storage(self.density, cfg, B), out=out, launch_ws=launch_ws,
+                                      storage=_brick_storage(self.density, cfg, B),
+                                      axis=_brick_axis(self.density, cfg, B), out=out, launch_ws=launch_ws,
                                       cleared=True, pixel_mask=det.subsample_mask())
         if det.n_subsample is not None:
             return _ScatteredGrid(out.unsqueeze(1))
diff --git a/diffdrr_amd/ops.py b/diffdrr_amd/ops.py
--- a/diffdrr_amd/ops.py
+++ b/diffdrr_amd/ops.py
@@ -253,12 +253,15 @@
     return torch.cat([p03, blk[:, 4].reshape(1, -1)])[:, :R].reshape(5, B, N)
 
 
-_BRICK_STORAGE = {"f32": _lib.BRICKS_F32, "q16": _lib.BRICKS_Q16, "q16p": _lib.BRICKS_Q16_PACKED}
+_BRICK_STORAGE = {"f32": _lib.BRICKS_F32, "q16": _lib.BRICKS_Q16, "q16p": _lib.BRICKS_Q16_PACKED,
+                  "q16y": _lib.BRICKS_Q16_Y, "q16py": _lib.BRICKS_Q16_PACKED_Y}
+_Y_TWIN = {"q16": "q16y", "q16p": "q16py"}
 _range_cache = {}
+_launches = 0
 
 
 class _Workspace:
-    __slots__ = ("ref", "buf", "built_version", "built_ptr", "churn", "event", "stream")
+    __slots__ = ("ref", "buf", "built_version", "built_ptr", "churn", "event", "stream", "used")
 
     def __init__(self, ref, buf):
         self.ref, self.buf = ref, buf
@@ -266,6 +269,7 @@
         self.built_ptr = None
         self.churn = 0
         self.event = self.stream = None
+        self.used = 0
 
 
 def _workspace_entry(volume, storage):
@@ -273,6 +277,11 @@
     if ent is not None and ent.ref() is volume and ent.buf.device == volume.device:
         return ent
     return None
+
+
+def _used_entry(volume, storage):
+    ents = [e for e in (_workspace_entry(volume, s) for s in (storage, _Y_TWIN.get(storage))) if e is not None]
+    return max(ents, key=lambda e: e.used) if ents else None
 
 
 def brick_workspace(volume, storage="q16"):
@@ -312,26 +321,26 @@
 
 
 def invalidate_brick_workspace(volume):
-    for storage in ("q16", "q16p"):
+    for storage in ("q16", "q16p", "q16y", "q16py"):
         ent = _workspace_entry(volume, storage)
         if ent is not None:
             ent.built_version = ent.built_ptr = None
 
 
 def brick_workspace_stale(volume, storage):
-    ent = _workspace_entry(volume, storage)
+    ent = _used_entry(volume, storage)
     if ent is None or ent.built_version is None:
         return None
     return int(ent.buf[2:3].view(torch.int32).item())
 
 
 def workspace_churn(volume, storage):
-    ent = _workspace_entry(volume, storage)
+    ent = _used_entry(volume, storage)
     return ent.churn if ent is not None else 0
 
 
 def brick_fallbacks(volume, storage):
-    ent = _workspace_entry(volume, storage)
+    ent = _used_entry(volume, storage)
     if ent is None or ent.built_version is None:
         return None
     head = ent.buf[:2].view(torch.int32).tolist()
@@ -352,12 +361,16 @@
 
 def siddon_forward_bricks(volume, source, target, img, det, *, voxel_shift=0.5, eps=1e-8,
                           want_aux=False, record_vmax=0.0, storage="f32", want_image=True,
-                          aux=None, out=None, launch_ws=None, cleared=False, pixel_mask=None):
+                          aux=None, out=None, launch_ws=None, cleared=False, pixel_mask=None, axis="z"):
     r = _rays(volume, source, target, img)
     B, N = r.B, r.N
     H, W = _grid(det, N, source)
     if storage != "f32" and not brick_storage_applies(volume):
         storage = "f32"
+    if axis not in ("y", "z"):
+        raise ValueError(f"axis must be 'y' or 'z', not {axis!r}")
+    if axis == "y" and volume.device.type == "cuda":
+        storage = _Y_TWIN.get(storage, storage)
     need_out = want_image or not want_aux
     if out is not None and (not need_out or out.shape != (B, N) or out.dtype != torch.float32
                             or not out.is_contiguous() or out.device != volume.device):
@@ -388,8 +401,12 @@
         _ptr(out), _ptr(aux), float(record_vmax) if packed else 0.0,
         _BRICK_STORAGE[storage], _ptr(ranges), int(valid) | (_lib.BRICKS_CLEARED if cleared else 0),
         launch_ws.data_ptr(), *(() if pixel_mask is None else (pixel_mask.data_ptr(),)))
-    if storage != "f32" and not valid:
-        brick_workspace_commit(volume, storage)
+    if storage != "f32":
+        global _launches
+        _launches += 1
+        _workspace_entry(volume, storage).used = _launches
+        if not valid:
+            brick_workspace_commit(volume, storage)
     return out, aux
 
 
diff --git a/diffdrr_amd/registration.py b/diffdrr_amd/registration.py
--- a/diffdrr_amd/registration.py
+++ b/diffdrr_amd/registration.py
@@ -251,7 +251,7 @@
 
     def _render(self):
         from . import ops
-        from .renderers import _brick_storage
+        from .renderers import _brick_axis, _brick_storage
 
         drr, reg = self.reg.drr, self.reg
         r, det = drr.renderer, drr.detector
@@ -265,6 +265,7 @@
                                                           clear_launch_ws=launch_ws)
         ops.siddon_forward_bricks(drr.density, source, target, img, cfg["det"], voxel_shift=cfg["voxel_shift"],
                                   eps=cfg["eps"], want_aux=True, storage=_brick_storage(drr.density, cfg, self.B),
+                                  axis=_brick_axis(drr.density, cfg, self.B),
                                   want_image=False, aux=self._aux, launch_ws=launch_ws, cleared=True)
         return dict(aux=self._aux, source=source, Mw=Mw, Ainv=Ainv, P=P, rot=rot, xyz=xyz, axes=self.axes,
                     reorient34=reorient34), dict(eps=cfg["eps"], with_img_path=not cfg["stop_gradients"])
diff --git a/diffdrr_amd/renderers.py b/diffdrr_amd/renderers.py
--- a/diffdrr_amd/renderers.py
+++ b/diffdrr_amd/renderers.py
@@ -94,6 +94,30 @@
     return storage
 
 
+VIEW_AXIS_AUTO = True
+VIEW_AXIS_MIN_POSES = 16
+
+
+def _brick_axis(volume, cfg, poses=None):
+    dev = volume.device
+    if dev.type != "cuda" or volume.dim() != 3:
+        return "z"
+    if dev not in _cu_count:
+        _cu_count[dev] = torch.cuda.get_device_properties(dev).multi_processor_count
+    return _resolve_brick_axis(cfg.get("brick_axis", "z"), cfg.get("view_axis"), volume.shape, _cu_count[dev], poses)
+
+
+def _resolve_brick_axis(brick_axis, view_axis, shape, n_cu, poses=None):
+    if brick_axis in ("y", "z"):
+        return brick_axis
+    if brick_axis != "auto":
+        raise ValueError(f"Siddon.brick_axis must be 'auto', 'y' or 'z', not {brick_axis!r}")
+    if view_axis != "y" or not VIEW_AXIS_AUTO or (poses is not None and int(poses) < VIEW_AXIS_MIN_POSES):
+        return "z"
+    dx, dy, dz = shape
+    return "y" if (-(-dx // 32)) * (-(-dy // 64)) * (-(-dz // 32)) >= 4 * n_cu else "z"
+
+
 class _SiddonFn(torch.autograd.Function):
 
     @staticmethod
@@ -108,7 +132,7 @@
             out, aux = ops.siddon_forward_bricks(
                 volume, source, target, img, cfg["det"], voxel_shift=cfg["voxel_shift"],
                 eps=cfg["eps"], want_aux=want_aux, record_vmax=_record_vmax(volume, want_aux, cfg),
-                storage=_brick_storage(volume, cfg, source.shape[0]))
+                storage=_brick_storage(volume, cfg, source.shape[0]), axis=_brick_axis(volume, cfg, source.shape[0]))
         else:
             out, aux, _ = ops.siddon_forward(
                 volume, source, target, img, voxel_shift=cfg["voxel_shift"], eps=cfg["eps"],
@@ -349,7 +373,8 @@
             out, aux = ops.siddon_forward_bricks(
                 volume, source, target, img, cfg["det"], voxel_shift=cfg["voxel_shift"],
                 eps=cfg["eps"], want_aux=want_aux, record_vmax=_record_vmax(volume, want_aux, cfg),
-                storage=_brick_storage(volume, cfg, source.shape[0]), pixel_mask=cfg.get("pixel_mask"))
+                storage=_brick_storage(volume, cfg, source.shape[0]), axis=_brick_axis(volume, cfg, source.shape[0]),
+                pixel_mask=cfg.get("pixel_mask"))
         else:
             out, aux, _ = ops.siddon_forward(
                 volume, source, target, img, voxel_shift=cfg["voxel_shift"], eps=cfg["eps"],
@@ -395,7 +420,7 @@
                                                           clear_launch_ws=launch_ws if some else None)
         ops.siddon_forward_bricks(
             volume, source, target, img, cfg["det"], voxel_shift=cfg["voxel_shift"], eps=cfg["eps"],
-            want_aux=True, storage=_brick_storage(volume, cfg, B), want_image=False, aux=aux,
+            want_aux=True, storage=_brick_storage(volume, cfg, B), axis=_brick_axis(volume, cfg, B), want_image=False, aux=aux,
             launch_ws=launch_ws, cleared=some)
         ncc, stats, _, total = ops.siddon_ncc_forward(aux, img, fixed, ncc_eps, want_sum=True) if reduce_sum \
             else (*ops.siddon_ncc_forward(aux, img, fixed, ncc_eps), None)
@@ -429,7 +454,8 @@
                                                           clear=aux, clear_launch_ws=launch_ws)
         out, _ = ops.siddon_forward_bricks(
             volume, source, target, img, cfg["det"], voxel_shift=cfg["voxel_shift"], eps=cfg["eps"],
-            want_aux=True, storage=_brick_storage(volume, cfg, B), aux=aux, launch_ws=launch_ws, cleared=True)
+            want_aux=True, storage=_brick_storage(volume, cfg, B), axis=_brick_axis(volume, cfg, B), aux=aux,
+            launch_ws=launch_ws, cleared=True)
         ctx.axes, ctx.cfg = axes, cfg
         ctx.save_for_backward(rot, xyz, reorient34, P, Ainv, Mw, source, aux)
         return out
@@ -527,6 +553,8 @@
         self.grid_path = "bricks"
         self.packed_record = False
         self.brick_storage = "q16p"
+        self.brick_axis = "auto"
+        self.view_axis = None
         self.static_volume = False
         self.channels_on_bricks = True
         self.channel_words = True
@@ -553,6 +581,7 @@
                 "det": self.detector_shape if det == "unchecked" else det, "tile": self.tile,
                 "path": self.grid_path,
                 "packed_record": self.packed_record, "storage": self.brick_storage,
+                "brick_axis": self.brick_axis, "view_axis": self.view_axis,
                 "static_volume": self.static_volume,
                 "channels_on_bricks": self.channels_on_bricks, "channel_words": self.channel_words}
 
diff --git a/include/diffdrr_hip.h b/include/diffdrr_hip.h
--- a/include/diffdrr_hip.h
+++ b/include/diffdrr_hip.h
@@ -36,6 +36,8 @@
 #define DDRR_BRICKS_F32 0
 #define DDRR_BRICKS_Q16 1
 #define DDRR_BRICKS_Q16_PACKED 2
+#define DDRR_BRICKS_Q16_Y 3
+#define DDRR_BRICKS_Q16_PACKED_Y 4
 #define DDRR_BRICKS_CLEARED 2
 long ddrr_brick_workspace_bytes(int dx, int dy, int dz, int brick_storage);
 long ddrr_brick_launch_workspace_bytes(int dx, int dy, int dz);
```

Measured after the change: 23470 DRRs/s (median of 6 runs). +4.2%, better.
